# svip-lab/impersonator

Measured on AMD Instinct MI355X. Metric: frames/sec (256x256 motion-imitation, batch=8), higher is better.
Workload: dtype bf16x3; 1 GPU; Imitator inference 256x256 batch=8, random-init ImpersonatorGenerator + synthetic SMPL, 1 source; frames=1024, batch_per_gpu=8, image_size=256, parallelism=frame-sharded replicas x1, grid_sample_align_corners=False, lanes=2, batches_per_launch_sequence=4, frames_per_launch=32, precision=bf16x3, precision_policy=auto

## Files before the change

impersonator_amd/csrc/conv.h:

```cpp
#pragma once
#include <vector>

#include "common.h"

namespace lwg {

constexpr int kConvBM = 128;
constexpr int kConvBK = 32;

struct ConvPhase {
    int KH, KW;
    int ntaps;
    int Kpad;
    long w_off;
    int oy0, ox0;
    int iy0, ix0;
};

inline void split_bf16_groups(const float *src, size_t n, float *dst_opaque)
{
    __bf16 *d = reinterpret_cast<__bf16 *>(dst_opaque);
    for (size_t g = 0; g < n; g += 32)
        for (int e = 0; e < 32; ++e) {
            const float v = src[g + e];
            const __bf16 hi = (__bf16)v;
            d[2 * g + e] = hi;
            d[2 * g + 32 + e] = (__bf16)(v - (float)hi);
        }
}

struct ConvArgs {
    const float *x; int ldx;
    int N, H, W, Cin, cin_log2;
    const float *w;
    const float *w_split;
    int precision;
    const float *zeros;
    float *y; int ldy;
    int Ho, Wo, Cout;
    int Hm, Wm, stride, pad, os;
    int dil;
    float2 *partials;
    int mtiles;
    int nphase;
    int fuse_phases;
    int natural_order;
    int tap_inner;
    int raw_in, raw_from;
    const float2 *in_ss; int in_ss_ld;
    unsigned long long *trace;
    int general;
    const float *bias;
    int ksplit;
    float *kpart;
    size_t kpart_stride;
    ConvPhase ph[4];
};

int conv_trace_set(void *device_buffer, size_t bytes);
int conv_trace_launch(int idx, long long *v10);

enum { kIgemmReg64 = 0, kIgemmReg128 = 1, kIgemmSmallCin = 2, kIgemmDma64 = 3, kIgemmDma128 = 4, kIgemmBf16x3_64 = 5,
       kIgemmBf16x3_128 = 6, kDirectStemBf16x3 = 7, kHaloBf16x3_128 = 8, kHaloBf16x3_64 = 9, kIgemmDma32 = 10, kIgemmVariants = 11 };
extern const char *const kIgemmVariantNames[kIgemmVariants];
int launch_conv_igemm(const ConvArgs &a, int bn, hipStream_t st, int *variant = nullptr);
int check_conv_igemm(const ConvArgs &a, int bn);
bool conv_raw_input_supported(const ConvArgs &a, int bn);

constexpr int kStemKRow = 48;
constexpr int kStemWPitch = 7 * kStemKRow * 2 + 16;
constexpr int kStemWBytes = 2 * 64 * kStemWPitch;
struct StemArgs {
    const float *x; int N, H, W;
    const void *w;
    float *y;
    float2 *partials;
    int dbg;
};
bool stem_bf16x3_supported(int H, int W, int cin, int cin_pad, int cout, int k, int stride, int pad);
void stem_pack_weights(const float *w_oihw, int cin, std::vector<unsigned char> &out);
int launch_stem_bf16x3(const StemArgs &a, hipStream_t st, int max_workgroups = 0);

int launch_in_finalize(const float2 *partials, int nphase, int mtiles, int N, int C, const float *gamma,
                       const float *beta, float eps, float2 *scale_shift, hipStream_t st);

struct ApplyArgs {
    const float *raw; int C;
    int N, H, W;
    const float2 *scale_shift;
    int relu;
    float *dst; int ld_dst;
    const float *res; int ld_res;
    int split;
    int nwarp;
    const float *warp_src[2];
    int warp_n[2];
    const float *warp_T[2];
    int align_corners;
};
int launch_apply(const ApplyArgs &a, hipStream_t st, int lanes = 0);

int launch_unsplit(float *buf, size_t n, hipStream_t st);

struct HeadsArgs {
    const float *x; int N, H, W;
    const float2 *scale_shift;
    const float *wh;
    float *color, *mask;
    const float *bg; int bg_bs;
    float *pred;
};
int launch_heads(const HeadsArgs &a, hipStream_t st);
size_t heads_bf16x3_frag_bytes();
int launch_heads_pack(const float *wh, void *wfrag, hipStream_t st);
int launch_heads_bf16x3(const HeadsArgs &a, const void *wfrag, hipStream_t st, int bands = 0);

}
```

impersonator_amd/csrc/conv.hip:

```cpp
#include <type_traits>

#include "conv.h"
#include "split.h"
#include "sample.h"

namespace lwg {
namespace {

typedef float f32x16 __attribute__((ext_vector_type(16)));
typedef float f32x4 __attribute__((ext_vector_type(4)));
#pragma clang diagnostic ignored "-Winline-asm"

constexpr int BM = kConvBM;
constexpr int BK = kConvBK;
constexpr int LDK = BK + 4;

template <int BN, int WM, int WN, bool WIDE = false, int NWAVES = 4, int BMT = BM, int TC2 = 0>
__device__ __forceinline__ void igemm_epilogue(const ConvArgs &a, const ConvPhase &ph, int phase, f32x16 (&acc)[WM][WN],
                                               float *smem, int tid, int lane, int wave_m, int wave_n, int img, int rem0, int n0,
                                               int mtile, int sub_stride = 0)
{
    unsigned ones = ~0u;
    asm volatile("" : "+s"(ones));
    lane = (int)__builtin_amdgcn_mbcnt_hi(ones, __builtin_amdgcn_mbcnt_lo(ones, 0u));
// ... 398 lines not shown
        }
        amask[j] = m;
    }
    const float *xin = a.x + (size_t)img * a.H * a.W * a.ldx;
    const float *wsrc[B_ROWS];
#pragma unroll
    for (int j = 0; j < B_ROWS; ++j) {
        const int row = (wave * B_ROWS + j) * 8 + lr;
        wsrc[j] = a.w + ph.w_off + (size_t)(n0 + row) * ph.Kpad + (ls ^ ((row >> 1) & 7)) * 4;
    }

    const unsigned lds_base = (unsigned)(uintptr_t)(__attribute__((address_space(3))) float *)smem;
    auto dma16 = [&](const float *gsrc, unsigned lds_byte) {
        asm volatile("s_mov_b32 m0, %1\n\t"
                     "s_nop 0\n\t"
                     "global_load_lds_dwordx4 %0, off"
                     :
                     : "v"(gsrc), "s"(lds_byte)
                     : "memory", "m0");
    };
    const unsigned wave_a = __builtin_amdgcn_readfirstlane(lds_base + (unsigned)(wave * 4 * 8 * BK * 4));
    const unsigned wave_b = __builtin_amdgcn_readfirstlane(lds_base + (unsigned)((BM * BK + wave * B_ROWS * 8 * BK) * 4));
    int s_tap = 0, s_kh = 0, s_kw = 0, s_ci0 = 0;
    auto dma_piece = [&](int p, int kt, int slot) {
        const unsigned slot_byte = (unsigned)(slot * STAGE * 4);
        if (p < 4) {
            const unsigned sa = wave_a + slot_byte + (unsigned)(p * 8 * BK * 4);
            const int toff = (s_kh * a.W + s_kw) * a.dil * a.ldx + s_ci0;
            const float *src = ((amask[p] >> s_tap) & 1u) ? xin + (aoff[p] + toff) : a.zeros;
            dma16(src, sa);
        } else {
            const unsigned sb = wave_b + slot_byte + (unsigned)((p - 4) * 8 * BK * 4);
            dma16(wsrc[p - 4] + kt * BK, sb);
        }
        if (p == LPS - 1) {
            s_ci0 += BK;
            if (s_ci0 == a.Cin) {
                s_ci0 = 0;
                ++s_tap;
                if (++s_kw == ph.KW) { s_kw = 0; ++s_kh; }
            }
        }
    };

    f32x16 acc[WM][WN];
#pragma unroll
    for (int i = 0; i < WM; ++i)
#pragma unroll
        for (int j = 0; j < WN; ++j)
#pragma unroll
            for (int r = 0; r < 16; ++r) acc[i][j][r] = 0.f;

    const int frow = lane & 31;
    const int fsw = (frow >> 1) & 7;
    const int a_row = (wave_m * 32 * WM + frow) * BK;
    const int b_row = BM * BK + (wave_n * 32 * WN + frow) * BK;
    int fcol[BK / 8];
#pragma unroll
    for (int k8 = 0; k8 < BK / 8; ++k8) fcol[k8] = (((2 * k8 + (lane >> 5)) ^ fsw) * 4);

    auto stage_body = [&](int kt, int slot, auto do_dma) {
        const float *As = smem + slot * STAGE + a_row;
        const float *Bs = smem + slot * STAGE + b_row;
        int slot2 = slot + (NS - 1);
        if (slot2 >= NS) slot2 -= NS;
        float4 af[WM], bf[WN];
#pragma unroll
        for (int i = 0; i < WM; ++i) af[i] = *reinterpret_cast<const float4 *>(As + i * 32 * BK + fcol[0]);
#pragma unroll
        for (int j = 0; j < WN; ++j) bf[j] = *reinterpret_cast<const float4 *>(Bs + j * 32 * BK + fcol[0]);
#pragma unroll
        for (int k8 = 0; k8 < BK / 8; ++k8) {
            float4 an[WM], bn4[WN];
            if (k8 + 1 < BK / 8 && !(DBG & 8)) {
#pragma unroll
                for (int i = 0; i < WM; ++i) an[i] = *reinterpret_cast<const float4 *>(As + i * 32 * BK + fcol[k8 + 1]);
#pragma unroll
                for (int j = 0; j < WN; ++j) bn4[j] = *reinterpret_cast<const float4 *>(Bs + j * 32 * BK + fcol[k8 + 1]);
            }
#pragma unroll
            for (int i = 0; i < WM; ++i)
#pragma unroll
                for (int j = 0; j < WN; ++j) {
                    acc[i][j] = __builtin_amdgcn_mfma_f32_32x32x2f32(af[i].x, bf[j].x, acc[i][j], 0, 0, 0);
                    acc[i][j] = __builtin_amdgcn_mfma_f32_32x32x2f32(af[i].y, bf[j].y, acc[i][j], 0, 0, 0);
                    acc[i][j] = __builtin_amdgcn_mfma_f32_32x32x2f32(af[i].z, bf[j].z, acc[i][j], 0, 0, 0);
                    acc[i][j] = __builtin_amdgcn_mfma_f32_32x32x2f32(af[i].w, bf[j].w, acc[i][j], 0, 0, 0);
                    constexpr int CHAINS = (BK / 8) * WM * WN;
                    const int piece = k8 * (WM * WN) + i * WN + j;
                    if (decltype(do_dma)::value && !(DBG & 1)) {
#pragma unroll
                        for (int pp = piece; pp < LPS; ++pp) {
                            if (pp != piece && piece != CHAINS - 1) break;
                            __builtin_amdgcn_sched_barrier(0);
                            dma_piece(pp, kt + (NS - 1), slot2);
                            __builtin_amdgcn_sched_barrier(0);
                        }
                    }
                }
            if (k8 + 1 < BK / 8 && !(DBG & 8)) {
#pragma unroll
                for (int i = 0; i < WM; ++i) af[i] = an[i];
#pragma unroll
                for (int j = 0; j < WN; ++j) bf[j] = bn4[j];
            }
        }
        if (decltype(do_dma)::value) {
            asm volatile("s_waitcnt vmcnt(%0)" ::"n"((NS - 2) * LPS) : "memory");
        } else {
            asm volatile("s_waitcnt vmcnt(0)" ::: "memory");
        }
        if (!(DBG & 4)) __builtin_amdgcn_s_barrier();
        asm volatile("" ::: "memory");
    };
    using yes = std::integral_constant<bool, true>;
    using no = std::integral_constant<bool, false>;
    static_assert(LPS <= 2 * (BK / 8) * WM * WN, "not enough MFMA chains to hide the DMA pieces of a stage");

    const int nk = ph.Kpad / BK;
#pragma unroll
    for (int st = 0; st < NS - 1; ++st)
        if (st < nk) {
#pragma unroll
            for (int p = 0; p < LPS; ++p) dma_piece(p, st, st);
        }
    if (nk >= NS - 1) {
        asm volatile("s_waitcnt vmcnt(%0)" ::"n"((NS - 2) * LPS) : "memory");
    } else {
        asm volatile("s_waitcnt vmcnt(0)" ::: "memory");
    }
    __builtin_amdgcn_s_barrier();
    asm volatile("" ::: "memory");

    int slot = 0, kt = 0;
    for (; kt + (NS - 1) < nk; ++kt) {
        stage_body(kt, slot, yes{});
        if (++slot == NS) slot = 0;
    }
    for (; kt < nk; ++kt) {
        stage_body(kt, slot, no{});
        if (++slot == NS) slot = 0;
    }
    igemm_epilogue<BN, WM, WN, true>(a, ph, pz, acc, smem, tid, lane, wave_m, wave_n, img, rem0, n0, blockIdx.x);
    __syncthreads();
    }
}

template <int BN, int WM, int WN, int DBG = 0, int NS = 3>
__global__ __launch_bounds__(256) void conv_igemm_dma_f32(const ConvArgs a)
{
    igemm_dma_body<BN, WM, WN, DBG, NS>(a);
}

template <int BN, int WM, int WN, int NS = 3, int DBG = 0, int BMT = BM>
__global__ __launch_bounds__(64 * (BMT / (32 * WM)) * (BN / (32 * WN))) void conv_igemm_bf16x3(const ConvArgs a)
{
    constexpr int WAVES_N = BN / (32 * WN), WAVES_M = BMT / (32 * WM), NW = WAVES_M * WAVES_N;
    static_assert((NW == 4 || NW == 8) && NS >= 3, "wave layout");
    constexpr int A_CH = (DBG & 1024) ? 1 : BMT / 8 / NW, B_CH = BN / 8 / NW;
    constexpr int LPS = A_CH + B_CH;
    constexpr int STAGE = (BMT + BN) * BK;
    constexpr int TILES = WM * WN;
    constexpr int Q = 6 * TILES;
    static_assert(Q >= LPS, "at most one DMA piece per MFMA");
    constexpr int QB = Q * 3 / 4;
    constexpr int ISSUED = (QB * LPS) / Q;

    extern __shared__ __attribute__((aligned(16))) float smem[];
    const int tid = threadIdx.x, lane = tid & 63;
    const int wave = __builtin_amdgcn_readfirstlane(tid >> 6);
    const int wave_m = wave / WAVES_N, wave_n = wave % WAVES_N;
    int bx = blockIdx.x;
    const int by = blockIdx.y;
    if (!(DBG & 64) && !a.natural_order && (gridDim.x & 7) == 0) bx = (blockIdx.x & 7) * (gridDim.x >> 3) + (blockIdx.x >> 3);
    const int m0 = bx * BMT, n0 = by * BN;
    const int hw_m = a.Hm * a.Wm, img = __builtin_amdgcn_readfirstlane(m0 / hw_m), rem0 = m0 - img * hw_m;
    const unsigned lds_base = (unsigned)(uintptr_t)(__attribute__((address_space(3))) float *)smem;
    auto uniform_ptr = [](const void *p) {
        const unsigned long long v = (unsigned long long)p;
        const unsigned lo = __builtin_amdgcn_readfirstlane((unsigned)v);
        const unsigned hi = __builtin_amdgcn_readfirstlane((unsigned)(v >> 32));
        return reinterpret_cast<const char *>(((unsigned long long)hi << 32) | lo);
    };
    auto dma16 = [&](unsigned voff, const char *sbase, unsigned lds_byte) {
        asm volatile("s_mov_b32 m0, %2\n\t"
                     "s_nop 0\n\t"
                     "global_load_lds_dwordx4 %0, %1"
                     :
                     : "v"(voff), "s"(sbase), "s"(lds_byte)
                     : "memory", "m0");
    };
    using yes = std::integral_constant<bool, true>;
    using no = std::integral_constant<bool, false>;
    unsigned long long tr_a = 0, tr_b = 0, tr_c = 0, tr_wait = 0, tr_bar = 0, tr_t0 = 0, tr_loop0 = 0, tr_loop1 = 0;
    unsigned long long tr_d0 = 0, tr_d1 = 0, tr_d2 = 0, tr_d3 = 0, tr_dma = 0, tr_rt0 = 0;
    unsigned tr_stages = 0;
    if (DBG & 512) {
        tr_t0 = __builtin_amdgcn_s_memtime();
        tr_rt0 = __builtin_amdgcn_s_memrealtime();
    }

    const int pz0 = a.fuse_phases ? 0 : a.nphase - 1 - (int)blockIdx.z;
    const int pz1 = a.fuse_phases ? a.nphase : pz0 + 1;
    for (int pz = pz0; pz < pz1; ++pz) {
    const ConvPhase ph = a.ph[pz];

    const int lr = lane >> 3, ls = lane & 7;
    int aoff[A_CH];
    unsigned amask[A_CH];
#pragma unroll
    for (int j = 0; j < A_CH; ++j) {
        const int row = (wave * A_CH + j) * 8 + lr;
        const int rem = rem0 + row;
        const int hm = rem / a.Wm, wm = rem - hm * a.Wm;
        const int hi0 = hm * a.stride - a.pad, wi0 = wm * a.stride - a.pad;
        aoff[j] = (hi0 * a.W + wi0) * a.ldx + (ls ^ ((row >> 1) & 7)) * 4;
        unsigned m = 0;
        for (int t = 0, kh = 0, kw = 0; t < ph.ntaps; ++t) {
            const bool ok = (unsigned)(hi0 + kh * a.dil) < (unsigned)a.H && (unsigned)(wi0 + kw * a.dil) < (unsigned)a.W;
            m |= (unsigned)ok << t;
            if (++kw == ph.KW) { kw = 0; ++kh; }
        }
        amask[j] = m;
    }
    const float *xin = a.x + (size_t)img * a.H * a.W * a.ldx;
    const char *x_base = uniform_ptr(xin);
    const char *w_base = uniform_ptr(a.w_split + ph.w_off);
    const unsigned zoff_b = (unsigned)((const char *)a.zeros - (const char *)xin);
    unsigned wvoff[B_CH], cur[A_CH];
#pragma unroll
    for (int j = 0; j < B_CH; ++j) {
        const int row = (wave * B_CH + j) * 8 + lr;
        wvoff[j] = (unsigned)(((n0 + row) * ph.Kpad + (ls ^ ((row >> 1) & 7)) * 4) * 4);
    }
    int s_tap = 0, s_kh = 0, s_kw = 0;
    unsigned s_ci_b = 0, s_w_b = 0;
    auto retap = [&]() {
        const int tapoff = (s_kh * a.W + s_kw) * a.dil * a.ldx;
#pragma unroll
        for (int p = 0; p < A_CH; ++p) cur[p] = ((amask[p] >> s_tap) & 1u) ? (unsigned)((aoff[p] + tapoff) * 4) : zoff_b;
    };
    retap();
    const unsigned wave_a = __builtin_amdgcn_readfirstlane(lds_base + (unsigned)(wave * A_CH * 8 * BK * 4));
    const unsigned wave_b = __builtin_amdgcn_readfirstlane(lds_base + (unsigned)((BMT * BK + wave * B_CH * 8 * BK) * 4));
    auto dma_piece = [&](int p, int kt, int slot) {
        const unsigned slot_byte = (unsigned)(slot * STAGE * 4);
        if (p < A_CH) {
            dma16(cur[p], x_base + s_ci_b, wave_a + slot_byte + (unsigned)(p * 8 * BK * 4));
        } else {
            dma16(wvoff[p - A_CH], w_base + __builtin_amdgcn_readfirstlane(s_w_b), wave_b + slot_byte + (unsigned)((p - A_CH) * 8 * BK * 4));
        }
        if (p == LPS - 1) {
            if (a.tap_inner) {
                ++s_tap;
                if (++s_kw == ph.KW) { s_kw = 0; ++s_kh; }
                if (s_tap == ph.ntaps) { s_tap = 0; s_kh = 0; s_kw = 0; s_ci_b += BK * 4; }
                s_w_b = (unsigned)(s_tap * a.Cin) * 4u + s_ci_b;
                retap();
            } else {
                s_w_b += BK * 4;
                s_ci_b += BK * 4;
                if (s_ci_b == (unsigned)a.Cin * 4) {
                    asm volatile("; next tap" ::: "memory");
                    s_ci_b = 0;
                    ++s_tap;
                    if (++s_kw == ph.KW) { s_kw = 0; ++s_kh; }
                    retap();
                }
            }
        }
    };

    f32x16 acc[WM][WN];
#pragma unroll
    for (int i = 0; i < WM; ++i)
#pragma unroll
        for (int j = 0; j < WN; ++j)
#pragma unroll
            for (int r = 0; r < 16; ++r) acc[i][j][r] = 0.f;

    const int frow = lane & 31, fsw = (frow >> 1) & 7;
    const int a_row = (wave_m * 32 * WM + frow) * BK;
    const int b_row = BMT * BK + (wave_n * 32 * WN + frow) * BK;
    int fcol[4];
#pragma unroll
    for (int c = 0; c < 4; ++c) fcol[c] = (((2 * c + (lane >> 5)) ^ fsw) * 4);
    struct Frags { float4 ah[WM], al[WM], bh[WN], bl[WN]; };
    auto load_frags = [&](int slot, int kb, Frags &f) {
        const float *As = smem + slot * STAGE + a_row;
        const float *Bs = smem + slot * STAGE + b_row;
        const int ch = fcol[kb], cl = fcol[2 + kb];
#pragma unroll
        for (int i = 0; i < WM; ++i) {
            f.ah[i] = *reinterpret_cast<const float4 *>(As + i * 32 * BK + ch);
            f.al[i] = *reinterpret_cast<const float4 *>(As + i * 32 * BK + cl);
        }
#pragma unroll
        for (int j = 0; j < WN; ++j) {
            f.bh[j] = *reinterpret_cast<const float4 *>(Bs + j * 32 * BK + ch);
            f.bl[j] = *reinterpret_cast<const float4 *>(Bs + j * 32 * BK + cl);
        }
    };
    auto load_one = [&](int slot, int kb, Frags &f, int idx) {
        const float *As = smem + slot * STAGE + a_row;
        const float *Bs = smem + slot * STAGE + b_row;
        const int ch = fcol[kb], cl = fcol[2 + kb];
        if (idx < WM) f.al[idx] = *reinterpret_cast<const float4 *>(As + idx * 32 * BK + cl);
        else if (idx < WM + WN) f.bh[idx - WM] = *reinterpret_cast<const float4 *>(Bs + (idx - WM) * 32 * BK + ch);
        else if (idx < 2 * WM + WN) f.ah[idx - WM - WN] = *reinterpret_cast<const float4 *>(As + (idx - WM - WN) * 32 * BK + ch);
        else f.bl[idx - 2 * WM - WN] = *reinterpret_cast<const float4 *>(Bs + (idx - 2 * WM - WN) * 32 * BK + cl);
    };
    constexpr int NL = 2 * (WM + WN);
    constexpr int RPM = (NL + (Q - QB) - 1) / (Q - QB);
    Frags fr;

    auto stage_body = [&](int kt, auto slot_c, auto do_dma) {
        constexpr int slot = decltype(slot_c)::value;
        constexpr int slot1 = (slot + 1) % NS, slot2 = (slot + NS - 1) % NS;
        Frags f1, nx;
        if (DBG & 256) load_frags(slot, 1, f1);
#pragma unroll
        for (int q = 0; q < Q; ++q) {
            const int kb = q / (3 * TILES), r = q % (3 * TILES);
            const int t = r / TILES, i = (r / WN) % WM, j = r % WN;
            if (q == QB) {
                __builtin_amdgcn_sched_barrier(0);
                if (DBG & 512) {
                    if (tr_stages) {
                        tr_wait += tr_b - tr_a; tr_bar += tr_c - tr_b;
                        tr_dma += (tr_d1 - tr_d0) + (tr_d3 - tr_d2);
                    }
                    ++tr_stages;
                    tr_a = __builtin_amdgcn_s_memtime();
                }
                if (decltype(do_dma)::value) {
                    asm volatile("s_waitcnt vmcnt(%0) lgkmcnt(0)" ::"n"((NS - 3) * LPS + ISSUED) : "memory");
                } else {
                    asm volatile("s_waitcnt vmcnt(0) lgkmcnt(0)" ::: "memory");
                }
                if (DBG & 512) tr_b = __builtin_amdgcn_s_memtime();
                if (!(DBG & 4)) __builtin_amdgcn_s_barrier();
                if (DBG & 512) tr_c = __builtin_amdgcn_s_memtime();
                asm volatile("" ::: "memory");
                if (DBG & 256) {
                    load_frags(slot1, 0, nx);
                    __builtin_amdgcn_sched_barrier(0);
                }
            }
            const Frags &f = kb == 0 ? fr : f1;
            const float4 a4 = t == 0 ? f.al[i] : f.ah[i];
            const float4 b4 = t == 1 ? f.bl[j] : f.bh[j];
            acc[i][j] = __builtin_amdgcn_mfma_f32_32x32x16_bf16(__builtin_bit_cast(bf16x8_t, a4),
                                                                __builtin_bit_cast(bf16x8_t, b4), acc[i][j], 0, 0, 0);
            if (!(DBG & 8) && !(DBG & 256)) {
                if (q < NL) {
                    load_one(slot, 1, f1, q);
                    __builtin_amdgcn_sched_group_barrier(0x008, 1, 0);
                    __builtin_amdgcn_sched_group_barrier(0x100, 1, 0);
                } else if (q >= QB && RPM * (q - QB) < NL) {
#pragma unroll
                    for (int r2 = 0; r2 < RPM; ++r2)
                        if (RPM * (q - QB) + r2 < NL) load_one(slot1, 0, nx, RPM * (q - QB) + r2);
                    __builtin_amdgcn_sched_group_barrier(0x008, 1, 0);
                    __builtin_amdgcn_sched_group_barrier(0x100, RPM, 0);
                }
            }
            if (decltype(do_dma)::value && !(DBG & 1)) {
                const int pc = ((q + 1) * LPS) / Q;
                const int pb = (q * LPS) / Q;
                if (pc != pb) {
                    __builtin_amdgcn_sched_barrier(0);
                    if ((DBG & 512) && pb == 0) tr_d0 = __builtin_amdgcn_s_memtime();
                    if ((DBG & 512) && pb == A_CH) tr_d2 = __builtin_amdgcn_s_memtime();
                    dma_piece(pb, kt + (NS - 1), slot2);
                    if ((DBG & 512) && pb == 0) tr_d1 = __builtin_amdgcn_s_memtime();
                    if ((DBG & 512) && pb == A_CH) tr_d3 = __builtin_amdgcn_s_memtime();
                    __builtin_amdgcn_sched_barrier(0);
                }
            }
        }
        if (!(DBG & 8)) fr = nx;
    };

    const int nk = ph.Kpad / BK;
#pragma unroll
    for (int st = 0; st < NS - 1; ++st)
        if (st < nk) {
#pragma unroll
            for (int p = 0; p < LPS; ++p) dma_piece(p, st, st);
        }
    if (nk >= NS - 1) {
        asm volatile("s_waitcnt vmcnt(%0)" ::"n"((NS - 2) * LPS) : "memory");
    } else {
        asm volatile("s_waitcnt vmcnt(0)" ::: "memory");
    }
    __builtin_amdgcn_s_barrier();
    asm volatile("" ::: "memory");
    load_frags(0, 0, fr);

    if (DBG & 512) tr_loop0 = __builtin_amdgcn_s_memtime();
    int kt = 0, slot = 0;
    static_assert(NS >= 3 && NS <= 5, "ring depth");
    for (; kt + 2 * (NS - 1) < nk; kt += NS) {
        stage_body(kt, std::integral_constant<int, 0>{}, yes{});
        stage_body(kt + 1, std::integral_constant<int, 1>{}, yes{});
        stage_body(kt + 2, std::integral_constant<int, 2>{}, yes{});
        if constexpr (NS >= 4) stage_body(kt + 3, std::integral_constant<int, 3>{}, yes{});
        if constexpr (NS >= 5) stage_body(kt + 4, std::integral_constant<int, 4>{}, yes{});
    }
    auto run_stage = [&](int k, int sl, auto do_dma) {
        if (sl == 0) stage_body(k, std::integral_constant<int, 0>{}, do_dma);
        else if (sl == 1) stage_body(k, std::integral_constant<int, 1>{}, do_dma);
        else if (NS == 3 || sl == 2) stage_body(k, std::integral_constant<int, 2>{}, do_dma);
        else if (NS == 4 || sl == 3) stage_body(k, std::integral_constant<int, (NS > 3 ? 3 : 2)>{}, do_dma);
        else stage_body(k, std::integral_constant<int, NS - 1>{}, do_dma);
    };
    for (; kt + (NS - 1) < nk; ++kt) {
        run_stage(kt, slot, yes{});
        if (++slot == NS) slot = 0;
    }
    for (; kt < nk; ++kt) {
        run_stage(kt, slot, no{});
        if (++slot == NS) slot = 0;
    }

    if (DBG & 512) {
        asm volatile("s_waitcnt lgkmcnt(0)" ::: "memory");
        tr_wait += tr_b - tr_a;
        tr_bar += tr_c - tr_b;
        tr_loop1 = __builtin_amdgcn_s_memtime();
    }
    if (!(DBG & 32)) igemm_epilogue<BN, WM, WN, !(DBG & 128), NW, BMT>(a, ph, pz, acc, smem, tid, lane, wave_m, wave_n, img, rem0, n0, bx);
    if ((DBG & 512) && a.trace && lane == 0) {
        const unsigned long long tr_end = __builtin_amdgcn_s_memtime();
        unsigned long long *o = a.trace + ((((size_t)blockIdx.z * gridDim.y + blockIdx.y) * gridDim.x + blockIdx.x) * NW + wave) * 8;
        const unsigned long long tr_rt1 = __builtin_amdgcn_s_memrealtime();
        unsigned hwid, xcc;
        asm volatile("s_getreg_b32 %0, hwreg(HW_REG_HW_ID)" : "=s"(hwid));
        asm volatile("s_getreg_b32 %0, hwreg(HW_REG_XCC_ID)" : "=s"(xcc));
        o[0] = tr_t0; o[1] = tr_loop0; o[2] = tr_loop1; o[3] = tr_end; o[4] = tr_wait; o[5] = tr_bar;
        o[6] = (unsigned long long)tr_stages | (tr_dma << 16) | ((tr_rt1 - tr_rt0) << 44);
        o[7] = ((unsigned long long)xcc << 32) | hwid;
    }
    if (DBG & 32) {
        float keep = 0.f;
#pragma unroll
        for (int i = 0; i < WM; ++i)
#pragma unroll
            for (int j = 0; j < WN; ++j)
#pragma unroll
                for (int r = 0; r < 16; ++r) keep += acc[i][j][r];
        if (keep == 123.456f) a.y[0] = 1.f;
    }
    __syncthreads();
    }
}

template <int NHW, int B_CH, int Q, int QB, int NS, int HT = 7>
struct HaloSched {
    static constexpr int nh(int t) { return t < HT ? NHW / HT + (t < NHW % HT ? 1 : 0) : 0; }
    static constexpr int tap_of(int k) { int t = 0; while (hstart(t + 1) <= k) ++t; return t; }
    static constexpr bool dma_at(int t, int q) { for (int p = 0; p < lps(t); ++p) if (pos(t, p) == q) return true; return false; }
    static constexpr int nfree(int t, int q0) { int n = 0; for (int q = q0; q < QB; ++q) n += dma_at(t, q) ? 0 : 1; return n; }
    static constexpr int conv_first(int nconv, int nslot, int slot, int piece) { return conv_range(nconv, nslot, slot, piece) / 16; }
    static constexpr int conv_last(int nconv, int nslot, int slot, int piece) { return conv_range(nconv, nslot, slot, piece) % 16; }
    static constexpr int conv_range(int nconv, int nslot, int slot, int piece) {
        if (nconv == 1) {
            if (piece != 0) return 0;
            if (nslot >= 7)
                return slot == 0 ? 0 * 16 + 1 : slot == 3 ? 1 * 16 + 3 : slot == 4 ? 3 * 16 + 5 : slot == 5 ? 5 * 16 + 7 : slot == 6 ? 7 * 16 + 8 : 0;
            return slot == 0 ? 0 * 16 + 1 : slot == 2 ? 1 * 16 + 4 : slot == 3 ? 4 * 16 + 6 : slot == 4 ? 6 * 16 + 8 : 0;
        }
        if (nslot >= 8) {
            if (slot >= 8 || (slot & 1) != piece) return 0;
            return (slot >> 1) == 0 ? 0 * 16 + 1 : (slot >> 1) == 1 ? 1 * 16 + 3 : (slot >> 1) == 2 ? 3 * 16 + 5 : 5 * 16 + 8;
        }
        if (slot == 0) return 0 * 16 + 1;
        if (slot < 2 || slot >= 6 || (slot & 1) != piece) return 0;
        return slot < 4 ? 1 * 16 + 4 : 4 * 16 + 8;
    }
    static constexpr int free_index(int t, int q0, int q) {
        if (q < q0 || q >= QB || dma_at(t, q)) return -1;
        int n = 0;
        for (int u = q0; u < q; ++u) n += dma_at(t, u) ? 0 : 1;
        return n;
    }
    static constexpr int hstart(int t) { int n = 0; for (int u = 0; u < t; ++u) n += nh(u); return n; }
    static constexpr int lps(int t) { return nh(t) + B_CH; }
    static constexpr int pos(int t, int p) { return (p + 1) * Q / lps(t) - 1; }
    static constexpr int issued(int t) { int n = 0; for (int p = 0; p < lps(t); ++p) n += pos(t, p) < QB ? 1 : 0; return n; }
    static constexpr int nwait(int t) { int n = issued(t); for (int d = 1; d <= NS - 3; ++d) n += lps((t + 9 - d) % 9); return n; }
};

struct HaloCT {
    static constexpr int phase(int t) { return t == 0 ? 0 : t < 3 ? 1 : t < 5 ? 2 : 3; }
    static constexpr int tap(int t) { return t == 0 ? 0 : t < 3 ? t - 1 : t < 5 ? t - 3 : t - 5; }
    static constexpr int dy(int t) { return (t == 4 || t == 7 || t == 8) ? 1 : 0; }
    static constexpr int dx(int t) { return (t == 2 || t == 6 || t == 8) ? 1 : 0; }
};

template <int BN, int WM, int WN, int NWAVES, int BMT, int TC>
__device__ __forceinline__ void halo_epilogue(const ConvArgs &a, const ConvPhase &ph, int phase, f32x4 (&acc)[2 * WM][2 * WN], float *smem,
                                              int wave_m, int wave_n, int img, int h0, int w0, int n0, int part0, int sub_stride)
{
    unsigned ones = ~0u;
    asm volatile("" : "+s"(ones));
    const int lane = (int)__builtin_amdgcn_mbcnt_hi(ones, __builtin_amdgcn_mbcnt_lo(ones, 0u));
    const int tid = (wave_m * (BN / (32 * WN)) + wave_n) * 64 + lane;
    const int col = lane & 15, rsel = 4 * (lane >> 4);
    constexpr int TP = 36;
    float *stage = smem + (tid >> 6) * 32 * TP;
    const int rrow = lane >> 3, rcol = (lane & 7) * 4;
#pragma unroll
    for (int i = 0; i < WM; ++i)
#pragma unroll
        for (int j = 0; j < WN; ++j) {
#pragma unroll
            for (int h = 0; h < 2; ++h)
#pragma unroll
                for (int g = 0; g < 2; ++g)
#pragma unroll
                    for (int r = 0; r < 4; ++r) stage[(16 * h + rsel + r) * TP + 16 * g + col] = acc[2 * i + h][2 * j + g][r];
#pragma unroll
            for (int q = 0; q < 4; ++q) {
                const int row = q * 8 + rrow;
                const float4 v = *reinterpret_cast<const float4 *>(stage + row * TP + rcol);
                const int trow = wave_m * 32 * WM + i * 32 + row;
                const int hm = h0 + trow / TC, wm = w0 + trow % TC;
                const size_t opix = ((size_t)img * a.Ho + hm * a.os + ph.oy0) * a.Wo + wm * a.os + ph.ox0;
                *reinterpret_cast<float4 *>(a.y + opix * a.ldy + n0 + wave_n * 32 * WN + j * 32 + rcol) = v;
            }
        }
    if (!a.partials) return;
    float2 *red = reinterpret_cast<float2 *>(smem + NWAVES * 32 * TP);
    auto lane_xor = [&](float v, int m) {
        return __builtin_bit_cast(float, __builtin_amdgcn_ds_bpermute((lane ^ m) << 2, __builtin_bit_cast(int, v)));
    };
#pragma unroll
    for (int i = 0; i < WM; ++i)
#pragma unroll
        for (int j = 0; j < WN; ++j)
#pragma unroll
            for (int g = 0; g < 2; ++g) {
                float s = 0.f;
#pragma unroll
                for (int h = 0; h < 2; ++h)
#pragma unroll
                    for (int r = 0; r < 4; ++r) s += acc[2 * i + h][2 * j + g][r];
                s += lane_xor(s, 16);
                s += lane_xor(s, 32);
                const float mu = s * (1.f / 32.f);
                float q = 0.f;
#pragma unroll
                for (int h = 0; h < 2; ++h)
#pragma unroll
                    for (int r = 0; r < 4; ++r) {
                        const float d = acc[2 * i + h][2 * j + g][r] - mu;
                        q += d * d;
                    }
                q += lane_xor(q, 16);
                q += lane_xor(q, 32);
                if (lane < 16) red[(wave_m * WM + i) * BN + wave_n * 32 * WN + j * 32 + 16 * g + col] = make_float2(mu, q);
            }
    __syncthreads();
    if (tid < BN * (BMT / BM)) {
        constexpr int RT = BM / 32;
        const int sub = tid / BN, ch = tid - sub * BN;
        float mean = 0.f;
#pragma unroll
        for (int w = 0; w < RT; ++w) mean += red[(sub * RT + w) * BN + ch].x;
        mean *= 1.f / RT;
        float m2 = 0.f;
#pragma unroll
        for (int w = 0; w < RT; ++w) {
            const float2 p = red[(sub * RT + w) * BN + ch];
            const float d = p.x - mean;
            m2 += p.y + 32.f * d * d;
        }
        a.partials[((size_t)phase * a.mtiles + (size_t)part0 + (size_t)sub * sub_stride) * a.Cout + n0 + ch] = make_float2(mean, m2);
    }
}

constexpr int halo_min_waves(int bn, int ct) { return ct ? (bn == 128 ? 1 : 2) : bn == 128 ? 2 : 3; }

template <int BN, int WM, int WN, int NS, int TC, int BMT = BM, int CT = 0, bool RAW = false>
__global__ __launch_bounds__(64 * (BMT / (32 * WM)) * (BN / (32 * WN))) __attribute__((amdgpu_waves_per_eu(halo_min_waves(BN, CT))))
void conv3x3_halo_bf16x3(const ConvArgs a)
{
    constexpr int NPH = CT ? 4 : 1, PADL = CT ? 0 : 1;
    constexpr int WAVES_N = BN / (32 * WN), WAVES_M = BMT / (32 * WM), NW = WAVES_M * WAVES_N;
    static_assert((NW == 4 || NW == 8) && (NS == 3 || NS == 4) && BMT % TC == 0 && TC % 32 == 0, "layout");
    constexpr int TR = BMT / TC, HC = TC + 2 - (CT ? 1 : 0), HR = TR + 2 - (CT ? 1 : 0), HP = HR * HC;
    constexpr int NCH = (HP + 7) / 8;
    constexpr int NHW = (NCH + NW - 1) / NW;
    constexpr int HALO = NCH * 8 * BK;
    constexpr int B_CH = BN / 8 / NW, BSTAGE = BN * BK, BOFF = 2 * HALO;
    static_assert(B_CH >= 1, "a weight chunk per wave");
    constexpr int TILES = WM * WN, Q = 6 * TILES, QB = Q * 3 / 4, NL = 2 * (WM + WN);
    constexpr int RPM = (NL + 2 * (Q - QB) - 1) / (2 * (Q - QB));
    constexpr int HT = RAW ? 6 : 7;
    using S = HaloSched<NHW, B_CH, Q, QB, NS, HT>;
    static_assert(S::hstart(9) == NHW && Q >= NHW / HT + 1 + B_CH, "halo pieces fit their taps, one piece per MFMA at most");
    static_assert(!RAW || (NW % 2 == 0 && S::tap_of(NHW - 1) + 3 <= 8), "RAW: chunk parity per wave, conversions end ahead of the barrier of tap 8");
    constexpr int DUMMY = BOFF + NS * BSTAGE;
    constexpr int SSOFF = DUMMY + 8 * BK;

    extern __shared__ __attribute__((aligned(16))) float smem[];
    const int tid = threadIdx.x, lane = tid & 63;
// ... 165 lines not shown
        int nxt_a[WM];
        [[maybe_unused]] const bool raw_next = RAW && sl + 1 < nslices && (sl + 1) * BK >= a.raw_from;
        [[maybe_unused]] const unsigned live_bits = raw_next ? inside : 0u;
        if constexpr (RAW) {
            if (T == S::tap_of(0) + 3) load_ss(sl + 1 < nslices ? sl + 1 : 0);
        }
#pragma unroll
        for (int q = 0; q < Q; ++q) {
            const int t = q / (2 * TILES), r = q % (2 * TILES);
            if (q == QB) {
                __builtin_amdgcn_sched_barrier(0);
                if (ISSUE) {
                    asm volatile("s_waitcnt vmcnt(%0) lgkmcnt(0)" ::"n"(S::nwait(T)) : "memory");
                } else {
                    asm volatile("s_waitcnt vmcnt(0) lgkmcnt(0)" ::: "memory");
                }
                __builtin_amdgcn_s_barrier();
                asm volatile("" ::: "memory");
#pragma unroll
                for (int ii = 0; ii < WM; ++ii) nxt_a[ii] = a_addr(ii, TN, hs_next);
            }
            constexpr int PP = CT ? HaloCT::phase(T) : 0;
            auto mfma_and_read = [&](int e) {
                const int u = 2 * r + e, i = u / WN2, j = u % WN2, g = 2 * q + e;
                const float4 a4 = t == 0 ? fr.a[i] : f1.a[i];
                const float4 b4 = t == 1 ? f1.b[j] : fr.b[j];
                acc[PP][i][j] = __builtin_amdgcn_mfma_f32_16x16x32_bf16(__builtin_bit_cast(bf16x8_t, a4),
                                                                        __builtin_bit_cast(bf16x8_t, b4), acc[PP][i][j], 0, 0, 0);
                if (g < NL) {
                    load_one(cur_a, slot, false, f1, g);
                    __builtin_amdgcn_sched_group_barrier(0x008, 1, 0);
                    __builtin_amdgcn_sched_group_barrier(0x100, 1, 0);
                } else if (g >= 2 * QB && RPM * (g - 2 * QB) < NL) {
#pragma unroll
                    for (int r2 = 0; r2 < RPM; ++r2)
                        if (RPM * (g - 2 * QB) + r2 < NL) load_one(nxt_a, slot1, true, nx, RPM * (g - 2 * QB) + r2);
                    __builtin_amdgcn_sched_group_barrier(0x008, 1, 0);
                    __builtin_amdgcn_sched_group_barrier(0x100, RPM, 0);
                }
            };
            mfma_and_read(0);
            if constexpr (!RAW) mfma_and_read(1);
            if constexpr (RAW) {
                constexpr int NCONV = T >= 3 ? S::nh(T - 3) : 0, K0 = T >= 3 ? S::hstart(T - 3) : 0;
                constexpr int Q0 = QB - NL >= 10 ? NL : 0;
                constexpr int NF = S::nfree(T, Q0);
                static_assert(NCONV <= 2 && NF >= (NCONV == 2 ? 6 : 5), "conversion steps fit ahead of the barrier");
                const int fi = S::free_index(T, Q0, q);
                if (NCONV > 0 && fi >= 0) {
                    const int a0 = S::conv_first(NCONV, NF, fi, 0), a1 = S::conv_last(NCONV, NF, fi, 0);
                    const int b0 = S::conv_first(NCONV, NF, fi, 1), b1 = S::conv_last(NCONV, NF, fi, 1);
                    if (a1 > a0 || b1 > b0) {
                        __builtin_amdgcn_sched_barrier(0);
#pragma unroll
                        for (int m = 0; m < 8; ++m)
                            if (m >= a0 && m < a1) convert_step(K0, cvA, hs ^ 1, m, (live_bits >> K0) & 1u);
#pragma unroll
                        for (int m = 0; m < 8; ++m)
                            if (m >= b0 && m < b1) convert_step(K0 + 1, cvB, hs ^ 1, m, (live_bits >> (K0 + 1)) & 1u);
                        __builtin_amdgcn_sched_barrier(0);
                    }
                }
                mfma_and_read(1);
            }
            if (ISSUE) {
#pragma unroll
                for (int p = 0; p < S::lps(T); ++p)
                    if (q == S::pos(T, p)) {
                        __builtin_amdgcn_sched_barrier(0);
                        if (p < S::nh(T)) halo_piece(S::hstart(T) + p, sl_halo, hs ^ 1);
                        else weight_piece(p - S::nh(T), IT, is, slot2);
                        __builtin_amdgcn_sched_barrier(0);
                    }
            }
        }
        fr = nx;
#pragma unroll
        for (int ii = 0; ii < WM; ++ii) cur_a[ii] = nxt_a[ii];
    };

    if constexpr (RAW) {
        const float2 *ss = a.in_ss + (size_t)img * a.in_ss_ld;
        const int nraw = a.Cin - a.raw_from;
        for (int i2 = tid; i2 < nraw; i2 += NW * 64) reinterpret_cast<float2 *>(smem + SSOFF)[i2] = ss[i2];
        asm volatile("s_waitcnt vmcnt(0)" ::: "memory");
    }
#pragma unroll
    for (int j = 0; j < NHW; ++j) halo_piece(j, 0, 0);
#pragma unroll
    for (int st = 0; st < NS - 1; ++st)
#pragma unroll
        for (int jb = 0; jb < B_CH; ++jb) weight_piece(jb, st, 0, st);
    asm volatile("s_waitcnt vmcnt(%0)" ::"n"((NS - 2) * B_CH) : "memory");
    if constexpr (RAW) {
        if (a.raw_from == 0) {
            asm volatile("s_waitcnt lgkmcnt(0)" ::: "memory");
            __builtin_amdgcn_s_barrier();
            asm volatile("" ::: "memory");
            load_ss(0);
#pragma unroll
            for (int j = 0; j < NHW; ++j)
#pragma unroll
                for (int step = 0; step < 8; ++step) convert_step(j, cvA, 0, step, (inside >> j) & 1u);
            asm volatile("s_waitcnt lgkmcnt(0)" ::: "memory");
        }
    }
    __builtin_amdgcn_s_barrier();
    asm volatile("" ::: "memory");
#pragma unroll
    for (int ii = 0; ii < WM; ++ii) cur_a[ii] = a_addr(ii, 0, 0);
#pragma unroll
    for (int idx = 0; idx < NL; ++idx) load_one(cur_a, 0, true, fr, idx);

    using yes = std::integral_constant<bool, true>;
    using no = std::integral_constant<bool, false>;
    if (a.trace) tr_loop0 = __builtin_amdgcn_s_memtime();
    int slot = 0;
    auto bump = [&]() { slot = slot + 1 == NS ? 0 : slot + 1; };
#define LWG_HALO_STAGE(T, ISS) stage_body(std::integral_constant<int, T>{}, ISS{}, sl, slot); bump();
    for (int sl = 0; sl + 1 < nslices; ++sl) {
        LWG_HALO_STAGE(0, yes) LWG_HALO_STAGE(1, yes) LWG_HALO_STAGE(2, yes) LWG_HALO_STAGE(3, yes) LWG_HALO_STAGE(4, yes)
        LWG_HALO_STAGE(5, yes) LWG_HALO_STAGE(6, yes) LWG_HALO_STAGE(7, yes) LWG_HALO_STAGE(8, yes)
    }
    {
        const int sl = nslices - 1;
        LWG_HALO_STAGE(0, yes) LWG_HALO_STAGE(1, yes) LWG_HALO_STAGE(2, yes) LWG_HALO_STAGE(3, yes) LWG_HALO_STAGE(4, yes)
        LWG_HALO_STAGE(5, yes)
        if constexpr (NS == 3) { LWG_HALO_STAGE(6, yes) } else { LWG_HALO_STAGE(6, no) }
        LWG_HALO_STAGE(7, no) LWG_HALO_STAGE(8, no)
    }
#undef LWG_HALO_STAGE

    if (a.trace) tr_loop1 = __builtin_amdgcn_s_memtime();
    __syncthreads();
    const int part0 = img * (tiles_x * (a.Hm / 4)) + (h0 / 4) * tiles_x + (w0 / TC);
#pragma unroll
    for (int pp = 0; pp < NPH; ++pp) {
        if (pp) __syncthreads();
        halo_epilogue<BN, WM, WN, NW, BMT, TC>(a, a.ph[pp], pp, acc[pp], smem, wave_m, wave_n, img, h0, w0, n0, part0, tiles_x);
    }
    if (a.trace && lane == 0) {
        const unsigned long long tr_end = __builtin_amdgcn_s_memtime(), tr_rt1 = __builtin_amdgcn_s_memrealtime();
        unsigned long long *o = a.trace + (((size_t)blockIdx.y * gridDim.x + blockIdx.x) * NW + wave) * 8;
        o[0] = tr_t0; o[1] = tr_loop0; o[2] = tr_loop1; o[3] = tr_end; o[4] = 0; o[5] = 0;
        o[6] = (unsigned long long)(9 * nslices) | ((tr_rt1 - tr_rt0) << 44);
        o[7] = 0;
    }
}

constexpr int FIN_CH = 16, FIN_SL = 16;
__global__ __launch_bounds__(256) void in_finalize_kernel(const float2 *__restrict__ partials, int nphase, int mtiles,
                                                          int tiles_per_img, int C, const float *__restrict__ gamma,
                                                          const float *__restrict__ beta, float eps,
                                                          float2 *__restrict__ scale_shift)
{
    __shared__ double sh[3][FIN_SL][FIN_CH];
    const int cl = threadIdx.x & (FIN_CH - 1);
    const int c = blockIdx.x * FIN_CH + cl;
    const int slice = threadIdx.x / FIN_CH;
    const int n = blockIdx.y;
    double sm = 0., sq = 0., m2 = 0.;
    if (c < C) {
        for (int p = 0; p < nphase; ++p) {
            const float2 *base = partials + ((size_t)p * mtiles + (size_t)n * tiles_per_img) * C + c;
#pragma unroll 4
            for (int t = slice; t < tiles_per_img; t += FIN_SL) {
                const float2 v = base[(size_t)t * C];
                sm += v.x;
                sq += (double)v.x * v.x;
                m2 += v.y;
            }
        }
    }
    sh[0][slice][cl] = sm;
    sh[1][slice][cl] = sq;
    sh[2][slice][cl] = m2;
    __syncthreads();
    if (slice == 0 && c < C) {
        sm = sq = m2 = 0.;
#pragma unroll
        for (int k = 0; k < FIN_SL; ++k) {
            sm += sh[0][k][cl];
            sq += sh[1][k][cl];
            m2 += sh[2][k][cl];
        }
        const double cnt = (double)nphase * tiles_per_img;
        const double mean = sm / cnt;
        double between = sq - cnt * mean * mean;
        if (between < 0.) between = 0.;
        const double var = (m2 + BM * between) / (cnt * BM);
        const double inv = 1.0 / sqrt(var + (double)eps);
        const float sc = (float)(gamma[c] * inv);
        scale_shift[(size_t)n * C + c] = make_float2(sc, (float)(beta[c] - mean * gamma[c] * inv));
    }
}

__device__ __forceinline__ float4 ld4(const float *p) { return *reinterpret_cast<const float4 *>(p); }
__device__ __forceinline__ void fma4(float4 &acc, const float4 v, float w)
{
    acc.x += v.x * w; acc.y += v.y * w; acc.z += v.z * w; acc.w += v.w * w;
}

__global__ __launch_bounds__(256) void apply_kernel(const ApplyArgs a)
{
    const int c4n = a.C >> 2;
    const long i = (long)blockIdx.x * blockDim.x + threadIdx.x;
    const long total = (long)a.N * a.H * a.W * c4n;
    if (i >= total) return;
    const long pix = i / c4n;
    const int c = (int)(i - pix * c4n) * 4;
    const int hw = a.H * a.W;
    const int n = (int)(pix / hw);
    const int pn = (int)(pix - (long)n * hw);

    const float4 v = ld4(a.raw + pix * a.C + c);
    const float4 s01 = ld4(reinterpret_cast<const float *>(a.scale_shift + (size_t)n * a.C + c));
    const float4 s23 = ld4(reinterpret_cast<const float *>(a.scale_shift + (size_t)n * a.C + c + 2));
    float4 y;
    y.x = v.x * s01.x + s01.y;
    y.y = v.y * s01.z + s01.w;
    y.z = v.z * s23.x + s23.y;
    y.w = v.w * s23.z + s23.w;
    if (a.relu) {
        y.x = fmaxf(y.x, 0.f); y.y = fmaxf(y.y, 0.f); y.z = fmaxf(y.z, 0.f); y.w = fmaxf(y.w, 0.f);
    }
    const int soff = (c >> 5) * 32 + ((c & 31) >> 1);
    if (a.res) {
        float4 r;
        if (a.split) {
            const bf16x4_t h = *reinterpret_cast<const bf16x4_t *>(a.res + pix * a.ld_res + soff);
            const bf16x4_t l = *reinterpret_cast<const bf16x4_t *>(a.res + pix * a.ld_res + soff + 16);
            r = make_float4((float)h[0] + (float)l[0], (float)h[1] + (float)l[1], (float)h[2] + (float)l[2],
                            (float)h[3] + (float)l[3]);
        } else {
            r = ld4(a.res + pix * a.ld_res + c);
        }
        y.x += r.x; y.y += r.y; y.z += r.z; y.w += r.w;
    }
    for (int k = 0; k < a.nwarp; ++k) {
        const float2 g = *reinterpret_cast<const float2 *>(a.warp_T[k] + pix * 2);
        const GridTaps t = grid_taps(g.x, g.y, a.W, a.H, a.align_corners);
        const float *src = a.warp_src[k] + (size_t)(a.warp_n[k] > 1 ? n : 0) * hw * a.C + c;
        float4 wsum = make_float4(0.f, 0.f, 0.f, 0.f);
        if (t.vnw) fma4(wsum, ld4(src + (size_t)(t.y0 * a.W + t.x0) * a.C), t.wnw);
        if (t.vne) fma4(wsum, ld4(src + (size_t)(t.y0 * a.W + t.x0 + 1) * a.C), t.wne);
        if (t.vsw) fma4(wsum, ld4(src + (size_t)((t.y0 + 1) * a.W + t.x0) * a.C), t.wsw);
        if (t.vse) fma4(wsum, ld4(src + (size_t)((t.y0 + 1) * a.W + t.x0 + 1) * a.C), t.wse);
        y.x += wsum.x; y.y += wsum.y; y.z += wsum.z; y.w += wsum.w;
    }
    (void)pn;
    if (a.split) {
        bf16x4_t h, l;
        h[0] = (__bf16)y.x; h[1] = (__bf16)y.y; h[2] = (__bf16)y.z; h[3] = (__bf16)y.w;
        l[0] = (__bf16)(y.x - (float)h[0]); l[1] = (__bf16)(y.y - (float)h[1]);
        l[2] = (__bf16)(y.z - (float)h[2]); l[3] = (__bf16)(y.w - (float)h[3]);
        *reinterpret_cast<bf16x4_t *>(a.dst + pix * a.ld_dst + soff) = h;
        *reinterpret_cast<bf16x4_t *>(a.dst + pix * a.ld_dst + soff + 16) = l;
    } else {
        *reinterpret_cast<float4 *>(a.dst + pix * a.ld_dst + c) = y;
    }
}

__global__ __launch_bounds__(256) void apply8_kernel(const ApplyArgs a)
{
    const int c8n = a.C >> 3;
    const long i = (long)blockIdx.x * blockDim.x + threadIdx.x;
    const long total = (long)a.N * a.H * a.W * c8n;
    if (i >= total) return;
    const long pix = i / c8n;
    const int c = (int)(i - pix * c8n) * 8;
    const int hw = a.H * a.W;
    const int n = (int)(pix / hw);

    const float4 v0 = ld4(a.raw + pix * a.C + c), v1 = ld4(a.raw + pix * a.C + c + 4);
    const float *ssp = reinterpret_cast<const float *>(a.scale_shift + (size_t)n * a.C + c);
    const float4 s0 = ld4(ssp), s1 = ld4(ssp + 4), s2 = ld4(ssp + 8), s3 = ld4(ssp + 12);
    float y[8];
    y[0] = v0.x * s0.x + s0.y; y[1] = v0.y * s0.z + s0.w; y[2] = v0.z * s1.x + s1.y; y[3] = v0.w * s1.z + s1.w;
    y[4] = v1.x * s2.x + s2.y; y[5] = v1.y * s2.z + s2.w; y[6] = v1.z * s3.x + s3.y; y[7] = v1.w * s3.z + s3.w;
    if (a.relu) {
#pragma unroll
        for (int k = 0; k < 8; ++k) y[k] = fmaxf(y[k], 0.f);
    }
    const int soff = (c >> 5) * 32 + ((c & 31) >> 1);
    if (a.res) {
        const bf16x8_t h = *reinterpret_cast<const bf16x8_t *>(a.res + pix * a.ld_res + soff);
        const bf16x8_t l = *reinterpret_cast<const bf16x8_t *>(a.res + pix * a.ld_res + soff + 16);
#pragma unroll
        for (int k = 0; k < 8; ++k) y[k] += (float)h[k] + (float)l[k];
    }
    for (int k = 0; k < a.nwarp; ++k) {
        const float2 g = *reinterpret_cast<const float2 *>(a.warp_T[k] + pix * 2);
        const GridTaps t = grid_taps(g.x, g.y, a.W, a.H, a.align_corners);
        const float *src = a.warp_src[k] + (size_t)(a.warp_n[k] > 1 ? n : 0) * hw * a.C + c;
        float4 w0 = make_float4(0.f, 0.f, 0.f, 0.f), w1 = w0;
        if (t.vnw) { const float *q = src + (size_t)(t.y0 * a.W + t.x0) * a.C; fma4(w0, ld4(q), t.wnw); fma4(w1, ld4(q + 4), t.wnw); }
        if (t.vne) { const float *q = src + (size_t)(t.y0 * a.W + t.x0 + 1) * a.C; fma4(w0, ld4(q), t.wne); fma4(w1, ld4(q + 4), t.wne); }
        if (t.vsw) { const float *q = src + (size_t)((t.y0 + 1) * a.W + t.x0) * a.C; fma4(w0, ld4(q), t.wsw); fma4(w1, ld4(q + 4), t.wsw); }
        if (t.vse) { const float *q = src + (size_t)((t.y0 + 1) * a.W + t.x0 + 1) * a.C; fma4(w0, ld4(q), t.wse); fma4(w1, ld4(q + 4), t.wse); }
        y[0] += w0.x; y[1] += w0.y; y[2] += w0.z; y[3] += w0.w; y[4] += w1.x; y[5] += w1.y; y[6] += w1.z; y[7] += w1.w;
    }
    bf16x8_t h, l;
#pragma unroll
    for (int k = 0; k < 8; ++k) {
        h[k] = (__bf16)y[k];
        l[k] = (__bf16)(y[k] - (float)h[k]);
    }
    *reinterpret_cast<bf16x8_t *>(a.dst + pix * a.ld_dst + soff) = h;
    *reinterpret_cast<bf16x8_t *>(a.dst + pix * a.ld_dst + soff + 16) = l;
}

__global__ __launch_bounds__(256) void unsplit_kernel(float *buf, size_t ngroups)
{
    const size_t g = (size_t)blockIdx.x * blockDim.x + threadIdx.x;
    if (g >= ngroups) return;
    float4 raw[8];
#pragma unroll
    for (int i = 0; i < 8; ++i) raw[i] = ld4(buf + g * 32 + i * 4);
#pragma unroll
    for (int i = 0; i < 4; ++i) {
        const bf16x8_t h = __builtin_bit_cast(bf16x8_t, raw[i]);
        const bf16x8_t l = __builtin_bit_cast(bf16x8_t, raw[4 + i]);
        float4 o0 = make_float4((float)h[0] + (float)l[0], (float)h[1] + (float)l[1], (float)h[2] + (float)l[2],
                                (float)h[3] + (float)l[3]);
        float4 o1 = make_float4((float)h[4] + (float)l[4], (float)h[5] + (float)l[5], (float)h[6] + (float)l[6],
                                (float)h[7] + (float)l[7]);
        *reinterpret_cast<float4 *>(buf + g * 32 + i * 8) = o0;
        *reinterpret_cast<float4 *>(buf + g * 32 + i * 8 + 4) = o1;
    }
}

constexpr int HT = 32, HH = HT + 6;
constexpr int HCH = 8;
constexpr int HPITCH = HCH + 4;
constexpr int HEADS_W = 49 * HCH * 4;
constexpr int HEADS_LDS = (HH * HH * HPITCH + HEADS_W) * (int)sizeof(float);

__global__ __launch_bounds__(256) void heads_kernel(const HeadsArgs a)
{
    extern __shared__ __attribute__((aligned(16))) float halo[];
    const int tid = threadIdx.x;
    const int tx = tid & 31, tg = tid >> 5;
    const int n = blockIdx.z;
    const int y0 = blockIdx.y * HT, x0 = blockIdx.x * HT;
    const float *xin = a.x + (size_t)n * a.H * a.W * 64;
    const float2 *ss = a.scale_shift + (size_t)n * 64;

    float acc[4][4];
#pragma unroll
    for (int r = 0; r < 4; ++r)
#pragma unroll
        for (int o = 0; o < 4; ++o) acc[r][o] = 0.f;

    for (int chunk = 0; chunk < 64 / HCH; ++chunk) {
        __syncthreads();
        for (int i = tid; i < HH * HH * (HCH / 4); i += 256) {
            const int pix = i / (HCH / 4), half = i % (HCH / 4);
            const int hy = pix / HH, hx = pix - hy * HH;
            const int gy = y0 - 3 + hy, gx = x0 - 3 + hx;
            float4 v = make_float4(0.f, 0.f, 0.f, 0.f);
            if ((unsigned)gy < (unsigned)a.H && (unsigned)gx < (unsigned)a.W) {
                const int c = chunk * HCH + half * 4;
                v = ld4(xin + ((size_t)gy * a.W + gx) * 64 + c);
                const float4 s01 = ld4(reinterpret_cast<const float *>(ss + c));
                const float4 s23 = ld4(reinterpret_cast<const float *>(ss + c + 2));
                v.x = fmaxf(v.x * s01.x + s01.y, 0.f);
                v.y = fmaxf(v.y * s01.z + s01.w, 0.f);
                v.z = fmaxf(v.z * s23.x + s23.y, 0.f);
                v.w = fmaxf(v.w * s23.z + s23.w, 0.f);
            }
            *reinterpret_cast<float4 *>(halo + pix * HPITCH + half * 4) = v;
        }
        float *wl = halo + HH * HH * HPITCH;
        for (int i = tid; i < 49 * HCH; i += 256) {
            const int t = i / HCH, c = i % HCH;
            *reinterpret_cast<float4 *>(wl + i * 4) = ld4(a.wh + ((size_t)t * 64 + chunk * HCH + c) * 4);
        }
        __syncthreads();
        for (int kx = 0; kx < 7; ++kx)
            for (int q = 0; q < HCH / 4; ++q) {
                float4 hv[10], wq[7][4];
#pragma unroll
                for (int hr = 0; hr < 10; ++hr) hv[hr] = ld4(halo + ((tg * 4 + hr) * HH + tx + kx) * HPITCH + q * 4);
#pragma unroll
                for (int ky = 0; ky < 7; ++ky) {
                    const float *wp = wl + ((ky * 7 + kx) * HCH + q * 4) * 4;
#pragma unroll
                    for (int ci = 0; ci < 4; ++ci) wq[ky][ci] = ld4(wp + ci * 4);
                }
                __builtin_amdgcn_sched_barrier(0);
#pragma unroll
                for (int ky = 0; ky < 7; ++ky)
#pragma unroll
                    for (int r = 0; r < 4; ++r) {
                        const float4 v = hv[r + ky];
                        const float vv[4] = {v.x, v.y, v.z, v.w};
#pragma unroll
                        for (int ci = 0; ci < 4; ++ci) {
                            const float4 w = wq[ky][ci];
                            acc[r][0] = fmaf(vv[ci], w.x, acc[r][0]);
                            acc[r][1] = fmaf(vv[ci], w.y, acc[r][1]);
                            acc[r][2] = fmaf(vv[ci], w.z, acc[r][2]);
                            acc[r][3] = fmaf(vv[ci], w.w, acc[r][3]);
                        }
                    }
            }
    }
    const int ox = x0 + tx;
    if (ox >= a.W) return;
    const size_t hw = (size_t)a.H * a.W;
#pragma unroll
    for (int r = 0; r < 4; ++r) {
        const int oy = y0 + tg * 4 + r;
        if (oy >= a.H) break;
        const size_t p = (size_t)oy * a.W + ox;
        const float col[3] = {tanhf(acc[r][0]), tanhf(acc[r][1]), tanhf(acc[r][2])};
        const float m = 1.f / (1.f + expf(-acc[r][3]));
#pragma unroll
        for (int c = 0; c < 3; ++c) {
            if (a.color) a.color[((size_t)n * 3 + c) * hw + p] = col[c];
            if (a.pred) {
                const float b = a.bg[((size_t)(a.bg_bs > 1 ? n : 0) * 3 + c) * hw + p];
                a.pred[((size_t)n * 3 + c) * hw + p] = m * b + (1.f - m) * col[c];
            }
        }
        if (a.mask) a.mask[(size_t)n * hw + p] = m;
    }
}

}

const char *const kIgemmVariantNames[kIgemmVariants] = {
    "conv_igemm_f32<64, 1, 2, false, 0>", "conv_igemm_f32<128, 2, 2, false, 0>", "conv_igemm_f32<64, 1, 2, true, 0>",
    "conv_igemm_dma_f32<64, 1, 2, 0, 3>", "conv_igemm_dma_f32<128, 2, 2, 0, 3>",
    "conv_igemm_bf16x3<64, 1, 2, 3, 0>", "conv_igemm_bf16x3<128, 2, 2", "stem_bf16x3_kernel",
    "conv3x3_halo_bf16x3<128, 2, 2", "conv3x3_halo_bf16x3<64, 1, 2", "conv_igemm_dma_f32<32, 1, 1, 0, 3>"};

constexpr int kTraceMaxLaunches = 4096;
struct TraceLaunch { size_t offset; int gx, gy, gz, waves, stages, cin, cout, hm, n; };
struct TraceState {
    void *buf = nullptr; size_t bytes = 0, used = 0; int n = 0;
    TraceLaunch launch[kTraceMaxLaunches];
};
static TraceState g_trace;

int conv_trace_set(void *device_buffer, size_t bytes)
{
    g_trace.buf = device_buffer; g_trace.bytes = device_buffer ? bytes : 0; g_trace.used = 0; g_trace.n = 0;
    return LWG_OK;
}
int conv_trace_launch(int idx, long long *v)
{
    if (idx < 0 || idx >= g_trace.n) return LWG_ERR_INVALID_ARG;
    const TraceLaunch &L = g_trace.launch[idx];
    v[0] = (long long)L.offset; v[1] = L.gx; v[2] = L.gy; v[3] = L.gz; v[4] = L.waves; v[5] = L.stages; v[6] = L.cin; v[7] = L.cout;
    v[8] = L.hm; v[9] = L.n;
    return LWG_OK;
}

static unsigned long long *trace_block(const ConvArgs &a, dim3 grid, int waves, int stages)
{
    if (!g_trace.buf) return nullptr;
    const size_t need = (size_t)grid.x * grid.y * grid.z * waves * 8 * sizeof(unsigned long long);
    if (g_trace.used + need > g_trace.bytes || g_trace.n >= kTraceMaxLaunches) return nullptr;
    unsigned long long *p = reinterpret_cast<unsigned long long *>(static_cast<char *>(g_trace.buf) + g_trace.used);
    TraceLaunch &L = g_trace.launch[g_trace.n++];
    L.offset = g_trace.used; L.gx = grid.x; L.gy = grid.y; L.gz = grid.z; L.waves = waves; L.stages = stages; L.cin = a.Cin;
    L.cout = a.Cout; L.hm = a.Hm; L.n = a.N;
    g_trace.used += need;
    return p;
}

struct ConvKernel { void (*fn)(ConvArgs); int block; size_t lds_cap; int variant; const char *label; };

constexpr int kRawMaxChannels = 512;
constexpr size_t reg_lds(int bn) { return (size_t)2 * (BM + bn) * LDK * sizeof(float); }
constexpr size_t ring_lds(int ns, int bn, int bmt = BM) { return (size_t)ns * (bmt + bn) * BK * sizeof(float); }
constexpr size_t halo_lds(int hp, int ns, int bn) { return ((size_t)2 * ((hp + 7) / 8) * 8 * BK + (size_t)ns * bn * BK) * sizeof(float); }
constexpr int halo3x3_px(int bmt) { return (bmt / 32 + 2) * (32 + 2); }
constexpr int kHaloCTPx = (4 + 1) * (32 + 1);
constexpr size_t raw_lds(int channels) { return (size_t)8 * BK * sizeof(float) + (size_t)channels * sizeof(float2); }

enum ConvKernelId {
    kF32_64, kF32_128, kF32_Small, kGen_64, kGen_128, kGen_Small, kGenX3_64, kGenX3_128, kGenX3_Small,
    kDma_32, kDma_64, kDma_128,
    kRing_64, kRing_128_3, kRing_128_4, kRing_128_Traced, kRing_128_Tall,
    kHalo_64, kHalo_128, kHalo_Tall, kHaloRaw_64, kHaloRaw_128, kHaloRaw_Tall,
    kHaloCT_64, kHaloCT_128, kHaloCTRaw_64, kHaloCTRaw_128,
#ifdef LWG_EXPERIMENTS
    kRing_128_X, kRing_128_5,
#endif
    kConvKernels
};
static const ConvKernel kConvKernelTable[kConvKernels] = {
    {&conv_igemm_f32<64, 1, 2, false>, 256, reg_lds(64), kIgemmReg64, "conv_igemm_f32"},
    {&conv_igemm_f32<128, 2, 2, false>, 256, reg_lds(128), kIgemmReg128, "conv_igemm_f32"},
    {&conv_igemm_f32<64, 1, 2, true>, 256, reg_lds(64), kIgemmSmallCin, "conv_igemm_f32"},
    {&conv_igemm_f32<64, 1, 2, false, 0, true>, 256, reg_lds(64), kIgemmReg64, "conv_igemm_f32 (general)"},
    {&conv_igemm_f32<128, 2, 2, false, 0, true>, 256, reg_lds(128), kIgemmReg128, "conv_igemm_f32 (general)"},
    {&conv_igemm_f32<64, 1, 2, true, 0, true>, 256, reg_lds(64), kIgemmSmallCin, "conv_igemm_f32 (general)"},
    {&conv_igemm_f32<64, 1, 2, false, 0, true, true>, 256, reg_lds(64), kIgemmReg64, "conv_igemm_f32 (general)"},
    {&conv_igemm_f32<128, 2, 2, false, 0, true, true>, 256, reg_lds(128), kIgemmReg128, "conv_igemm_f32 (general)"},
    {&conv_igemm_f32<64, 1, 2, true, 0, true, true>, 256, reg_lds(64), kIgemmSmallCin, "conv_igemm_f32 (general)"},
    {&conv_igemm_dma_f32<32, 1, 1>, 256, ring_lds(3, 32), kIgemmDma32, "conv_igemm_dma_f32"},
    {&conv_igemm_dma_f32<64, 1, 2>, 256, ring_lds(3, 64), kIgemmDma64, "conv_igemm_dma_f32"},
    {&conv_igemm_dma_f32<128, 2, 2>, 256, ring_lds(3, 128), kIgemmDma128, "conv_igemm_dma_f32"},
    {&conv_igemm_bf16x3<64, 1, 2>, 256, ring_lds(3, 64), kIgemmBf16x3_64, "conv_igemm_bf16x3"},
    {&conv_igemm_bf16x3<128, 2, 2>, 256, ring_lds(3, 128), kIgemmBf16x3_128, "conv_igemm_bf16x3"},
    {&conv_igemm_bf16x3<128, 2, 2, 4>, 256, ring_lds(4, 128), kIgemmBf16x3_128, "conv_igemm_bf16x3"},
    {&conv_igemm_bf16x3<128, 2, 2, 4, 512>, 256, ring_lds(4, 128), kIgemmBf16x3_128, "conv_igemm_bf16x3 (traced)"},
    {&conv_igemm_bf16x3<128, 2, 2, 3, 0, 256>, 512, ring_lds(3, 128, 256), kIgemmBf16x3_128, "conv_igemm_bf16x3 (256-row tiles)"},
    {&conv3x3_halo_bf16x3<64, 1, 2, 3, 32>, 256, halo_lds(halo3x3_px(128), 3, 64), kHaloBf16x3_64, "conv3x3_halo_bf16x3"},
    {&conv3x3_halo_bf16x3<128, 2, 2, 4, 32>, 256, halo_lds(halo3x3_px(128), 4, 128), kHaloBf16x3_128, "conv3x3_halo_bf16x3"},
    {&conv3x3_halo_bf16x3<128, 2, 2, 4, 32, 256>, 512, halo_lds(halo3x3_px(256), 4, 128), kHaloBf16x3_128, "conv3x3_halo_bf16x3"},
    {&conv3x3_halo_bf16x3<64, 1, 2, 3, 32, 128, 0, true>, 256, halo_lds(halo3x3_px(128), 3, 64) + raw_lds(kRawMaxChannels),
     kHaloBf16x3_64, "conv3x3_halo_bf16x3"},
    {&conv3x3_halo_bf16x3<128, 2, 2, 4, 32, 128, 0, true>, 256, halo_lds(halo3x3_px(128), 4, 128) + raw_lds(kRawMaxChannels),
     kHaloBf16x3_128, "conv3x3_halo_bf16x3"},
    {&conv3x3_halo_bf16x3<128, 2, 2, 4, 32, 256, 0, true>, 512, halo_lds(halo3x3_px(256), 4, 128) + raw_lds(kRawMaxChannels),
     kHaloBf16x3_128, "conv3x3_halo_bf16x3"},
    {&conv3x3_halo_bf16x3<64, 1, 2, 3, 32, 128, 1>, 256, halo_lds(kHaloCTPx, 3, 64), kHaloBf16x3_64, "conv3x3_halo_bf16x3 (transposed)"},
    {&conv3x3_halo_bf16x3<128, 2, 2, 4, 32, 128, 1>, 256, halo_lds(kHaloCTPx, 4, 128), kHaloBf16x3_128, "conv3x3_halo_bf16x3 (transposed)"},
    {&conv3x3_halo_bf16x3<64, 1, 2, 3, 32, 128, 1, true>, 256, kLdsPerCu, kHaloBf16x3_64, "conv3x3_halo_bf16x3 (transposed)"},
    {&conv3x3_halo_bf16x3<128, 2, 2, 4, 32, 128, 1, true>, 256, kLdsPerCu, kHaloBf16x3_128, "conv3x3_halo_bf16x3 (transposed)"},
#ifdef LWG_EXPERIMENTS
    {&conv_igemm_bf16x3<128, 2, 2, 4, 1024>, 256, ring_lds(4, 128), kIgemmBf16x3_128, "conv_igemm_bf16x3"},
    {&conv_igemm_bf16x3<128, 2, 2, 5>, 256, ring_lds(5, 128), kIgemmBf16x3_128, "conv_igemm_bf16x3"},
#endif
};

static bool halo3x3_shape(const ConvArgs &a)
{
    const ConvPhase &p0 = a.ph[0];
    return a.nphase == 1 && p0.KH == 3 && p0.KW == 3 && a.stride == 1 && a.pad == 1 && a.dil == 1 && a.os == 1 && a.H == a.Hm &&
           a.W == a.Wm && p0.Kpad == 9 * a.Cin && a.Wm % 32 == 0 && a.Hm % 4 == 0;
}
static bool haloCT_shape(const ConvArgs &a)
{
    return a.nphase == 4 && a.os == 2 && a.stride == 1 && a.pad == 0 && a.dil == 1 && a.H == a.Hm && a.W == a.Wm && a.Wm % 32 == 0 &&
           a.Hm % 4 == 0 && a.Cout % 64 == 0 && a.ph[0].KH == 1 && a.ph[0].KW == 1 && a.ph[1].KH == 1 && a.ph[1].KW == 2 &&
           a.ph[2].KH == 2 && a.ph[2].KW == 1 && a.ph[3].KH == 2 && a.ph[3].KW == 2 && a.ph[0].Kpad == a.Cin &&
           a.ph[1].Kpad == 2 * a.Cin && a.ph[2].Kpad == 2 * a.Cin && a.ph[3].Kpad == 4 * a.Cin;
}

struct ConvSwitches {
    bool halo, halo_tall, ct_wide, ring3, ring_tall, fused_apply;
    char ring_exp;
};
static const ConvSwitches &conv_switches()
{
    static const ConvSwitches sw = [] {
        auto first = [](const char *name) { const char *v = getenv(name); return v ? v[0] : '\0'; };
        return ConvSwitches{first("LWG_HALO") != '0',
                            first("LWG_HALO_TALL") != '0',
                            first("LWG_CT_WIDE") != '0',
                            first("LWG_RING") == '3',
                            first("LWG_RING_TALL") != '0',
                            first("LWG_FUSED_APPLY") != '0',
                            first("LWG_RING")};
    }();
    return sw;
}

static bool raw_input_route(const ConvArgs &a, int bn, const ConvSwitches &sw)
{
    if (!sw.halo || !sw.fused_apply) return false;
    if (a.precision != 1 || a.general || !a.w_split || (a.ldx & 31) || (a.Cin & 31) || a.Cin < 32 || (bn != 64 && bn != 128)) return false;
    if (a.raw_from < 0 || (a.raw_from & 31) || a.raw_from >= a.Cin || a.Cin - a.raw_from > kRawMaxChannels) return false;
    return halo3x3_shape(a) || haloCT_shape(a);
}
bool conv_raw_input_supported(const ConvArgs &a, int bn) { return raw_input_route(a, bn, conv_switches()); }

struct ConvLaunch { const ConvKernel *k; dim3 grid; size_t lds; int trace_waves, trace_stages; };

static int plan_conv_igemm(const ConvArgs &a, int bn, int ncu, const ConvSwitches &sw, bool tracing, size_t trace_free, ConvLaunch *out)
{
    const bool bn32_ok = bn == 32 && a.precision == 0 && !a.general && a.Cin >= BK && a.zeros;
    if (a.Cout % bn != 0 || (bn != 64 && bn != 128 && !bn32_ok))
        LWG_FAIL(LWG_ERR_UNSUPPORTED, "conv: Cout=%d not a multiple of the %d-channel tile", a.Cout, bn);
    if (!a.general && ((a.Hm * a.Wm) % BM != 0 || a.mtiles * BM != a.N * a.Hm * a.Wm))
        LWG_FAIL(LWG_ERR_UNSUPPORTED, "conv: %dx%d output grid per image is not a multiple of %d pixels", a.Hm, a.Wm, BM);
    if (a.general && (a.partials || a.fuse_phases || (a.precision != 0 && a.precision != 1) ||
                      a.mtiles != ceil_div((long)a.N * a.Hm * a.Wm, BM)))
        LWG_FAIL(LWG_ERR_INVALID_ARG, "conv: general mode is unfused, without statistics, mtiles = ceil(M/128)");
    if (a.ksplit > 1 && (!a.general || !a.kpart || a.kpart_stride < (size_t)a.N * a.Ho * a.Wo * a.ldy))
        LWG_FAIL(LWG_ERR_INVALID_ARG, "conv: a reduction split needs the general mode and a partial buffer of ksplit outputs");
    if (a.dil < 1) LWG_FAIL(LWG_ERR_INVALID_ARG, "conv: dilation must be >= 1");
    if ((1 << a.cin_log2) != a.Cin || a.Cin < 4 || (a.ldx & 3))
        LWG_FAIL(LWG_ERR_UNSUPPORTED, "conv: Cin=%d must be a power of two >= 4 with a 16-byte aligned pixel stride", a.Cin);
    int max_taps = 0;
    for (int p = 0; p < a.nphase; ++p) {
        if (a.ph[p].Kpad % BK != 0 || a.ph[p].Kpad < a.ph[p].ntaps * a.Cin)
            LWG_FAIL(LWG_ERR_UNSUPPORTED, "conv: bad padded K=%d for %d taps x %d channels", a.ph[p].Kpad, a.ph[p].ntaps, a.Cin);
        if (a.ph[p].ntaps > max_taps) max_taps = a.ph[p].ntaps;
    }
    if (a.precision == 1 && a.tap_inner)
        for (int p = 0; p < a.nphase; ++p)
            if (a.ph[p].Kpad != a.ph[p].ntaps * a.Cin)
                LWG_FAIL(LWG_ERR_UNSUPPORTED, "conv: taps-innermost walk needs K=%d == %d taps x %d channels", a.ph[p].Kpad,
                         a.ph[p].ntaps, a.Cin);
    if (a.raw_in && (!a.in_ss || !raw_input_route(a, bn, sw)))
        LWG_FAIL(LWG_ERR_UNSUPPORTED, "conv: raw (un-normalised) input is only taken by the halo-resident bf16x3 kernels");

    const bool small_cin = a.Cin < BK;
    const dim3 grid(a.mtiles, a.Cout / bn, a.fuse_phases ? 1 : a.nphase * (a.ksplit > 1 ? a.ksplit : 1));
    const int tile = small_cin ? 2 : (bn == 128 ? 1 : 0);
    auto choose = [&](int id, dim3 g, size_t lds, int trace_waves = 0, int trace_stages = 0) -> int {
        *out = ConvLaunch{&kConvKernelTable[id], g, lds, trace_waves, trace_stages};
        if (lds > out->k->lds_cap) LWG_FAIL(LWG_ERR_STATE, "conv: %s asks for %zu bytes of LDS, opted in to %zu", out->k->label, lds, out->k->lds_cap);
        return LWG_OK;
    };
    if (a.general) {
        if (small_cin && bn != 64) LWG_FAIL(LWG_ERR_UNSUPPORTED, "conv: Cin=%d < %d is only built for the 64-channel tile", a.Cin, BK);
        if (max_taps > 64) LWG_FAIL(LWG_ERR_UNSUPPORTED, "conv: more than 64 taps");
        return choose((a.precision == 1 ? kGenX3_64 : kGen_64) + tile, grid, reg_lds(bn));
    }
    if (a.precision == 1) {
        if (small_cin || !a.w_split || !a.zeros || (a.ldx & 31) || (a.Cin & 31))
            LWG_FAIL(LWG_ERR_UNSUPPORTED, "conv: the bf16x3 path needs split weights and Cin, pixel stride multiples of 32");
        const char *x_end = reinterpret_cast<const char *>(a.x + (size_t)a.N * a.H * a.W * a.ldx);
        const char *z = reinterpret_cast<const char *>(a.zeros);
        if (z < x_end || (size_t)(z - reinterpret_cast<const char *>(a.x)) + (size_t)a.Cin * 4 > 0xffffffffull)
            LWG_FAIL(LWG_ERR_UNSUPPORTED, "conv: the bf16x3 path needs its zero run behind the input tensor, within 4 GiB");
        for (int p = 0; p < a.nphase; ++p)
            if ((size_t)a.Cout * a.ph[p].Kpad * 4 > 0xffffffffull)
                LWG_FAIL(LWG_ERR_UNSUPPORTED, "conv: weight matrix too large for 32-bit lane offsets");
        if (max_taps > 32) LWG_FAIL(LWG_ERR_UNSUPPORTED, "conv: more than 32 taps on the bf16x3 path");
        const size_t raw_bytes = a.raw_in ? raw_lds(a.Cin - a.raw_from) : 0;
        if (sw.halo && halo3x3_shape(a)) {
            const bool tall = bn == 128 && a.Hm % 8 == 0 && (long)(a.mtiles / 2) * (a.Cout / 128) >= ncu && sw.halo_tall;
            const int bmt = tall ? 256 : BM;
            return choose((a.raw_in ? kHaloRaw_64 : kHalo_64) + (tall ? 2 : bn == 128 ? 1 : 0), dim3(grid.x / (bmt / BM), grid.y, 1),
                          halo_lds(halo3x3_px(bmt), bn == 128 ? 4 : 3, bn) + raw_bytes, bmt / 32, 9 * a.Cin / BK);
        }
        if (sw.halo && haloCT_shape(a)) {
            const bool wide = a.Cout % 128 == 0 && (long)a.mtiles * (a.Cout / 128) >= ncu && sw.ct_wide;
            const int cbn = wide ? 128 : 64;
            return choose((a.raw_in ? kHaloCTRaw_64 : kHaloCT_64) + wide, dim3(a.mtiles, a.Cout / cbn, 1),
                          halo_lds(kHaloCTPx, wide ? 4 : 3, cbn) + raw_bytes, 4, -(int)(9 * a.Cin / BK));
        }
        if (bn == 64) return choose(kRing_64, grid, ring_lds(3, 64));
        if (tracing && !sw.ring3 && (size_t)grid.x * grid.y * grid.z * 4 * 8 * sizeof(unsigned long long) <= trace_free)
            return choose(kRing_128_Traced, grid, ring_lds(4, 128), 4, a.ph[0].Kpad / BK);
        if (!a.fuse_phases && a.nphase == 1 && (a.mtiles & 1) == 0 && (a.Hm * a.Wm) % 256 == 0 && !tracing &&
            (long)(a.mtiles / 2) * (a.Cout / 128) >= ncu && sw.ring_tall)
            return choose(kRing_128_Tall, dim3(grid.x / 2, grid.y, 1), ring_lds(3, 128, 256));
#ifdef LWG_EXPERIMENTS
        if (sw.ring_exp == 'x') return choose(kRing_128_X, grid, ring_lds(4, 128));
        if (sw.ring_exp == '5') return choose(kRing_128_5, grid, ring_lds(5, 128));
#endif
        return sw.ring3 ? choose(kRing_128_3, grid, ring_lds(3, 128)) : choose(kRing_128_4, grid, ring_lds(4, 128));
    }
    if (small_cin && bn != 64) LWG_FAIL(LWG_ERR_UNSUPPORTED, "conv: Cin=%d < %d is only built for the 64-channel tile", a.Cin, BK);
    const bool use_dma = !small_cin && a.zeros && max_taps <= 32 && (bn <= 64 || (long)grid.x * grid.y * grid.z <= ncu);
    if (a.fuse_phases && !use_dma) LWG_FAIL(LWG_ERR_UNSUPPORTED, "conv: fused phases need the DMA-fed kernel (Cin >= 32, 64-channel tile)");
    if (use_dma) return choose(bn == 32 ? kDma_32 : bn == 64 ? kDma_64 : kDma_128, grid, ring_lds(3, bn));
    if (bn != 64 && bn != 128) LWG_FAIL(LWG_ERR_UNSUPPORTED, "conv: the register-staged fp32 kernel has 64- and 128-channel tiles, not %d", bn);
    return choose(kF32_64 + tile, grid, reg_lds(bn));
}

int check_conv_igemm(const ConvArgs &a, int bn)
{
    ConvLaunch L;
    return plan_conv_igemm(a, bn, device_cu_count(), conv_switches(), false, 0, &L);
}

int launch_conv_igemm(const ConvArgs &a_in, int bn, hipStream_t st, int *variant)
{
    ConvArgs a = a_in;
    a.trace = nullptr;
    ConvLaunch L;
    const size_t trace_free = g_trace.n < kTraceMaxLaunches ? g_trace.bytes - g_trace.used : 0;
    const int rc = plan_conv_igemm(a, bn, device_cu_count(), conv_switches(), g_trace.buf != nullptr, trace_free, &L);
    if (rc != LWG_OK) return rc;
    static DeviceOnce opted_in;
    if (!opted_in.done()) {
        for (const ConvKernel &k : kConvKernelTable)
            LWG_HIP(hipFuncSetAttribute(reinterpret_cast<const void *>(k.fn), hipFuncAttributeMaxDynamicSharedMemorySize, (int)k.lds_cap));
        opted_in.mark();
    }
    if (L.trace_waves) a.trace = trace_block(a, L.grid, L.trace_waves, L.trace_stages);
    L.k->fn<<<L.grid, L.k->block, L.lds, st>>>(a);
    if (variant) *variant = L.k->variant;
    LWG_LAUNCH_CHECK(L.k->label);
    return LWG_OK;
}

#ifdef LWG_IGEMM_BENCH
static void launch_capped(void (*kern)(ConvArgs), const ConvArgs &a, int bn, int block, size_t lds, hipStream_t st, int bmt = BM)
{
    (void)hipFuncSetAttribute(reinterpret_cast<const void *>(kern), hipFuncAttributeMaxDynamicSharedMemorySize, (int)lds);
    kern<<<dim3(a.mtiles / (bmt / BM), a.Cout / bn, a.nphase), block, lds, st>>>(a);
}
template <int DBG>
static void launch_dbg(const ConvArgs &a, int bn, hipStream_t st)
{
    launch_capped(bn == 64 ? &conv_igemm_f32<64, 1, 2, false, DBG> : &conv_igemm_f32<128, 2, 2, false, DBG>, a, bn, 256, reg_lds(bn), st);
}
template <int DBG, int NS = 3>
static void launch_dma_dbg(const ConvArgs &a, int bn, hipStream_t st)
{
    launch_capped(bn == 64 ? &conv_igemm_dma_f32<64, 1, 2, DBG, NS> : &conv_igemm_dma_f32<128, 2, 2, DBG, NS>, a, bn, 256, ring_lds(NS, bn), st);
}
template <int NS, int DBG>
static void launch_k_dbg(const ConvArgs &a, int bn, hipStream_t st)
{
    launch_capped(bn == 64 ? &conv_igemm_bf16x3<64, 1, 2, NS, DBG> : &conv_igemm_bf16x3<128, 2, 2, NS, DBG>, a, bn, 256, ring_lds(NS, bn), st);
}
template <int BN, int WM, int WN, int DBG>
static void launch_w_dbg(const ConvArgs &a, hipStream_t st)
{
    launch_capped(&conv_igemm_bf16x3<BN, WM, WN, 3, DBG>, a, BN, 64 * (BM / (32 * WM)) * (BN / (32 * WN)), ring_lds(3, BN), st);
}
int launch_conv_igemm_dbg(const ConvArgs &a, int bn, int dbg, hipStream_t st)
{
    switch (dbg) {
        case 821: if (bn == 128) launch_w_dbg<128, 2, 1, 0>(a, st); else launch_w_dbg<64, 1, 1, 0>(a, st); break;
        case 812: if (bn == 128) launch_w_dbg<128, 1, 2, 0>(a, st); else launch_w_dbg<64, 1, 1, 0>(a, st); break;
        case 831: if (bn == 128) launch_w_dbg<128, 2, 1, 1>(a, st); else launch_w_dbg<64, 1, 1, 1>(a, st); break;
        case 856:
            if (bn != 64 || (a.mtiles & 1) || (a.Hm * a.Wm) % 256 != 0) return LWG_ERR_INVALID_ARG;
            launch_capped(&conv_igemm_bf16x3<64, 2, 2, 3, 0, 256>, a, 64, 256, ring_lds(3, 64, 256), st, 256);
            break;
        case 300: {
            ConvArgs b = a;
            b.precision = 1;
            return launch_conv_igemm(b, bn, st, nullptr);
        }
        case 200: launch_k_dbg<3, 0>(a, bn, st); break;
        case 201: launch_k_dbg<3, 1>(a, bn, st); break;
        case 204: launch_k_dbg<3, 4>(a, bn, st); break;
        case 213: launch_k_dbg<3, 13>(a, bn, st); break;
        case 240: launch_k_dbg<4, 0>(a, bn, st); break;
        case 241: launch_k_dbg<4, 1>(a, bn, st); break;
        case 245: launch_k_dbg<4, 13>(a, bn, st); break;
        case 1240: launch_k_dbg<4, 1024>(a, bn, st); break;
        case 232: launch_k_dbg<3, 32>(a, bn, st); break;
        case 264: launch_k_dbg<3, 64>(a, bn, st); break;
        case 328: launch_k_dbg<3, 128>(a, bn, st); break;
        case 456: launch_k_dbg<3, 256>(a, bn, st); break;
        case 0: launch_dbg<0>(a, bn, st); break;
        case 1: launch_dbg<1>(a, bn, st); break;
        case 3: launch_dbg<3>(a, bn, st); break;
        case 7: launch_dbg<7>(a, bn, st); break;
        case 15: launch_dbg<15>(a, bn, st); break;
        case 16: launch_dbg<16>(a, bn, st); break;
        case 4: launch_dbg<4>(a, bn, st); break;
        case 100: launch_dma_dbg<0>(a, bn, st); break;
        case 116: launch_dma_dbg<16>(a, bn, st); break;
        case 101: launch_dma_dbg<1>(a, bn, st); break;
        case 104: launch_dma_dbg<4>(a, bn, st); break;
        case 140: launch_dma_dbg<0, 4>(a, bn, st); break;
        default: return LWG_ERR_INVALID_ARG;
    }
    return LWG_OK;
}
#endif

int launch_in_finalize(const float2 *partials, int nphase, int mtiles, int N, int C, const float *gamma,
                       const float *beta, float eps, float2 *scale_shift, hipStream_t st)
{
    if (mtiles % N != 0) LWG_FAIL(LWG_ERR_UNSUPPORTED, "in_finalize: %d tiles do not split over %d images", mtiles, N);
    const dim3 grid(ceil_div(C, FIN_CH), N);
    in_finalize_kernel<<<grid, 256, 0, st>>>(partials, nphase, mtiles, mtiles / N, C, gamma, beta, eps, scale_shift);
    LWG_LAUNCH_CHECK("in_finalize_kernel");
    return LWG_OK;
}

int launch_apply(const ApplyArgs &a, hipStream_t st, int lanes)
{
    if (lanes != 0 && lanes != 4 && lanes != 8) LWG_FAIL(LWG_ERR_INVALID_ARG, "apply: lanes=%d (0: the launcher's choice, 4, 8)", lanes);
    if (lanes == 8 && !a.split) LWG_FAIL(LWG_ERR_UNSUPPORTED, "apply: eight channels per thread is the split-bf16 kernel");
    if ((a.C & 3) || (a.ld_dst & 3) || (a.res && (a.ld_res & 3)))
        LWG_FAIL(LWG_ERR_UNSUPPORTED, "apply: channel counts/strides must be multiples of 4 (C=%d)", a.C);
    if (a.split && ((a.C & 31) || (a.ld_dst & 31) || ((uintptr_t)a.dst & 127) ||
                    (a.res && ((a.ld_res & 31) || ((uintptr_t)a.res & 127)))))
        LWG_FAIL(LWG_ERR_UNSUPPORTED, "apply: split-bf16 buffers need 32-channel granularity (C=%d)", a.C);
    static const char *a8_env = getenv("LWG_APPLY8");
    if (lanes == 8 || (lanes == 0 && a.split && !(a8_env && a8_env[0] == '0'))) {
        const long total8 = (long)a.N * a.H * a.W * (a.C >> 3);
        apply8_kernel<<<ceil_div(total8, 256), 256, 0, st>>>(a);
        LWG_LAUNCH_CHECK("apply8_kernel");
        return LWG_OK;
    }
    const long total = (long)a.N * a.H * a.W * (a.C >> 2);
    apply_kernel<<<ceil_div(total, 256), 256, 0, st>>>(a);
    LWG_LAUNCH_CHECK("apply_kernel");
    return LWG_OK;
}

int launch_unsplit(float *buf, size_t n, hipStream_t st)
{
    if (n % 32) LWG_FAIL(LWG_ERR_INVALID_ARG, "unsplit: %zu floats is not a whole number of 32-value groups", n);
    if (!n) return LWG_OK;
    unsplit_kernel<<<(unsigned)ceil_div((long)(n / 32), 256), 256, 0, st>>>(buf, n / 32);
    LWG_LAUNCH_CHECK("unsplit_kernel");
    return LWG_OK;
}

int launch_heads(const HeadsArgs &a, hipStream_t st)
{
    if (a.pred && !a.bg) LWG_FAIL(LWG_ERR_INVALID_ARG, "heads: pred requested without a background image");
    static DeviceOnce opt_in;
    const int rc = opt_in_lds(reinterpret_cast<const void *>(&heads_kernel), HEADS_LDS, opt_in);
    if (rc != LWG_OK) return rc;
    const dim3 grid(ceil_div(a.W, HT), ceil_div(a.H, HT), a.N);
    heads_kernel<<<grid, 256, HEADS_LDS, st>>>(a);
    LWG_LAUNCH_CHECK("heads_kernel");
    return LWG_OK;
}

}
```

impersonator_amd/csrc/direct.hip:

```cpp
#include <type_traits>

#include "conv.h"

namespace lwg {
namespace {

typedef float f32x16 __attribute__((ext_vector_type(16)));
typedef __bf16 bf16x8_t __attribute__((ext_vector_type(8)));
typedef float f32x4 __attribute__((ext_vector_type(4)));
typedef float f32x4u __attribute__((ext_vector_type(4), aligned(4)));

constexpr int ST_COLS = 128, ST_ROWS = 2;
constexpr int ST_HW = ST_COLS + 8, ST_HH = ST_ROWS + 6;
constexpr int ST_PIX = 12;
constexpr int ST_HPLANE = ST_HH * ST_HW * ST_PIX;
constexpr int ST_WROW = kStemKRow * 2;
constexpr int ST_WPITCH = kStemWPitch;
constexpr int ST_WPLANE = 64 * ST_WPITCH;
constexpr int ST_RED = 2 * 4 * 64 * 8;
constexpr int ST_GROUPS = 2;
constexpr int ST_GLDS = 2 * ST_HPLANE + ST_RED;
constexpr int ST_LDS = 2 * ST_WPLANE + ST_GROUPS * ST_GLDS + 16;
static_assert(2 * ST_WPLANE == kStemWBytes, "host and device agree on the staged filter bank");
static_assert(ST_HPLANE % 16 == 0 && ST_LDS <= 160 * 1024, "stem tile must fit one CU's LDS");
static_assert((ST_WPITCH / 16) % 2 == 1, "odd 16-byte pitch: conflict-free weight fragment reads");

__device__ __forceinline__ void stem_group_barrier(unsigned *ctr, unsigned &target, int lane)
{
    target += 4;
    asm volatile("s_waitcnt lgkmcnt(0)" ::: "memory");
    if (lane == 0) __hip_atomic_fetch_add(ctr, 1u, __ATOMIC_RELAXED, __HIP_MEMORY_SCOPE_WORKGROUP);
    while (__hip_atomic_load(ctr, __ATOMIC_RELAXED, __HIP_MEMORY_SCOPE_WORKGROUP) < target) __builtin_amdgcn_s_sleep(1);
    asm volatile("" ::: "memory");
}

__global__ __launch_bounds__(256 * ST_GROUPS) void stem_bf16x3_kernel(const StemArgs a)
{
    extern __shared__ __attribute__((aligned(16))) unsigned char lds[];
    unsigned char *wts = lds;
    const int group = __builtin_amdgcn_readfirstlane(threadIdx.x >> 8);
    unsigned char *halo = lds + 2 * ST_WPLANE + group * ST_GLDS;
    float2 *red = reinterpret_cast<float2 *>(halo + 2 * ST_HPLANE);
    unsigned *gctr_all = reinterpret_cast<unsigned *>(lds + 2 * ST_WPLANE + ST_GROUPS * ST_GLDS);
    unsigned *gctr = gctr_all + group;
    unsigned gtarget = 0;

    const int tid = threadIdx.x & 255, lane = tid & 63;
    const int wave = __builtin_amdgcn_readfirstlane(tid >> 6);
#ifdef LWG_EXPERIMENTS
    const int dbg = a.dbg;
#else
    constexpr int dbg = 0;
#endif
    const int wrow = wave >> 1, whalf = wave & 1;

    for (int i = threadIdx.x; i < 2 * ST_WPLANE / 16; i += 256 * ST_GROUPS)
        reinterpret_cast<float4 *>(wts)[i] = reinterpret_cast<const float4 *>(a.w)[i];
    if (threadIdx.x < ST_GROUPS) gctr_all[threadIdx.x] = 0;

    const int a_base = ((wrow * ST_HW) + whalf * 64 + (lane & 31)) * ST_PIX + (lane >> 5) * 16;
    const int b_base = (lane & 31) * ST_WPITCH + (lane >> 5) * 16;

    const int tiles_x = a.W / ST_COLS, tiles_y = a.H / ST_ROWS;
    const int ntiles = a.N * tiles_y * tiles_x;
    constexpr int HE = (ST_HH * ST_HW + 255) / 256;
    float4 pre4[HE];
    float2 pre2[HE];
    auto fetch_halo = [&](int tile) {
        const int img = tile / (tiles_y * tiles_x);
        const int trem = tile - img * (tiles_y * tiles_x);
        const int ty = trem / tiles_x, tx = trem - ty * tiles_x;
        const int h0 = ty * ST_ROWS, c0 = tx * ST_COLS;
        const float *xin = a.x + (size_t)img * a.H * a.W * 8;
#pragma unroll
        for (int k = 0; k < HE; ++k) {
            const int e = tid + k * 256;
            const int hy = e / ST_HW, hx = e - hy * ST_HW;
            const int gy = h0 - 3 + hy, gx = c0 - 3 + hx;
            pre4[k] = make_float4(0.f, 0.f, 0.f, 0.f);
            pre2[k] = make_float2(0.f, 0.f);
            if (e < ST_HH * ST_HW && (unsigned)gy < (unsigned)a.H && (unsigned)gx < (unsigned)a.W) {
                const float *p = xin + ((size_t)gy * a.W + gx) * 8;
                pre4[k] = *reinterpret_cast<const float4 *>(p);
                pre2[k] = *reinterpret_cast<const float2 *>(p + 4);
            }
        }
    };
    auto store_halo = [&]() {
#pragma unroll
        for (int k = 0; k < HE; ++k) {
            const int e = tid + k * 256;
            if (e >= ST_HH * ST_HW) break;
            const float f[6] = {pre4[k].x, pre4[k].y, pre4[k].z, pre4[k].w, pre2[k].x, pre2[k].y};
            unsigned hw[3], lw[3];
#pragma unroll
            for (int c = 0; c < 3; ++c) {
                const __bf16 h0 = (__bf16)f[2 * c], h1 = (__bf16)f[2 * c + 1];
                const __bf16 l0 = (__bf16)(f[2 * c] - (float)h0), l1 = (__bf16)(f[2 * c + 1] - (float)h1);
                hw[c] = (unsigned)__builtin_bit_cast(unsigned short, h0) | ((unsigned)__builtin_bit_cast(unsigned short, h1) << 16);
                lw[c] = (unsigned)__builtin_bit_cast(unsigned short, l0) | ((unsigned)__builtin_bit_cast(unsigned short, l1) << 16);
            }
            unsigned *ph = reinterpret_cast<unsigned *>(halo + e * ST_PIX);
            unsigned *pl = reinterpret_cast<unsigned *>(halo + ST_HPLANE + e * ST_PIX);
            ph[0] = hw[0]; ph[1] = hw[1]; ph[2] = hw[2];
            pl[0] = lw[0]; pl[1] = lw[1]; pl[2] = lw[2];
        }
    };
    const int tile0 = blockIdx.x * ST_GROUPS + group, tstride = gridDim.x * ST_GROUPS;
    if (tile0 < ntiles) fetch_halo(tile0);
    __syncthreads();
    for (int tile = tile0; tile < ntiles; tile += tstride) {
        const int img = tile / (tiles_y * tiles_x);
        const int trem = tile - img * (tiles_y * tiles_x);
        const int ty = trem / tiles_x, tx = trem - ty * tiles_x;
        const int h0 = ty * ST_ROWS, c0 = tx * ST_COLS;

        if (!(dbg & 8) || tile == tile0) store_halo();
        stem_group_barrier(gctr, gtarget, lane);
        if (!(dbg & 8) && tile + tstride < ntiles) fetch_halo(tile + tstride);

        f32x16 acc[2][2];
#pragma unroll
        for (int i = 0; i < 2; ++i)
#pragma unroll
            for (int j = 0; j < 2; ++j)
#pragma unroll
                for (int r = 0; r < 16; ++r) acc[i][j][r] = 0.f;
        struct Frags { f32x4 ah[2], al[2], bh[2], bl[2]; };
        auto load_frags = [&](int n, Frags &f) {
            const int kh = n / 3, s3 = n - 3 * kh;
            const int ao = a_base + kh * ST_HW * ST_PIX + s3 * 32, bo = b_base + kh * ST_WROW + s3 * 32;
            f.al[0] = *reinterpret_cast<const f32x4u *>(halo + ST_HPLANE + ao);
            f.bh[0] = *reinterpret_cast<const f32x4 *>(wts + bo);
            f.bh[1] = *reinterpret_cast<const f32x4 *>(wts + bo + 32 * ST_WPITCH);
            f.al[1] = *reinterpret_cast<const f32x4u *>(halo + ST_HPLANE + ao + 32 * ST_PIX);
            f.ah[0] = *reinterpret_cast<const f32x4u *>(halo + ao);
            f.bl[0] = *reinterpret_cast<const f32x4 *>(wts + ST_WPLANE + bo);
            f.bl[1] = *reinterpret_cast<const f32x4 *>(wts + ST_WPLANE + bo + 32 * ST_WPITCH);
            f.ah[1] = *reinterpret_cast<const f32x4u *>(halo + ao + 32 * ST_PIX);
        };
        Frags fr[2];
        load_frags(0, fr[0]);
        if (!(dbg & 4))
#pragma unroll
        for (int n = 0; n < 21; ++n) {
            const Frags &f = fr[n & 1];
            if (n + 1 < 21) load_frags(n + 1, fr[(n + 1) & 1]);
#pragma unroll
            for (int t = 0; t < 3; ++t)
#pragma unroll
                for (int i = 0; i < 2; ++i)
#pragma unroll
                    for (int j = 0; j < 2; ++j) {
                        const f32x4 a4 = t == 0 ? f.al[i] : f.ah[i];
                        const f32x4 b4 = t == 1 ? f.bl[j] : f.bh[j];
                        acc[i][j] = __builtin_amdgcn_mfma_f32_32x32x16_bf16(
                            __builtin_bit_cast(bf16x8_t, a4), __builtin_bit_cast(bf16x8_t, b4), acc[i][j], 0, 0, 0);
                    }
            if (n + 1 < 21) {
#pragma unroll
                for (int g2 = 0; g2 < 12; ++g2) {
                    __builtin_amdgcn_sched_group_barrier(0x008, 1, 0);
                    __builtin_amdgcn_sched_group_barrier(0x100, 1, 0);
                }
            }
            __builtin_amdgcn_sched_barrier(0);
        }

        const int col = lane & 31, rsel = 4 * (lane >> 5);
        const size_t prow = ((size_t)img * a.H + h0 + wrow) * a.W + c0 + whalf * 64;
        if (!(dbg & 1)) {
#pragma unroll
            for (int i = 0; i < 2; ++i)
#pragma unroll
                for (int r = 0; r < 16; ++r) {
                    const int px = i * 32 + (r & 3) + 8 * (r >> 2) + rsel;
                    float *yo = a.y + (prow + px) * 64 + col;
                    yo[0] = acc[i][0][r];
                    yo[32] = acc[i][1][r];
                }
        }
        if (a.partials && !(dbg & 2)) {
#pragma unroll
            for (int i = 0; i < 2; ++i)
#pragma unroll
                for (int j = 0; j < 2; ++j) {
                    float s = 0.f;
#pragma unroll
                    for (int r = 0; r < 16; ++r) s += acc[i][j][r];
                    s += __shfl_xor(s, 32);
                    const float mu = s * (1.f / 32.f);
                    float q = 0.f;
#pragma unroll
                    for (int r = 0; r < 16; ++r) {
                        const float d = acc[i][j][r] - mu;
                        q += d * d;
                    }
                    q += __shfl_xor(q, 32);
                    if (lane < 32) red[(wrow * 4 + whalf * 2 + i) * 64 + j * 32 + col] = make_float2(mu, q);
                }
        }
        stem_group_barrier(gctr, gtarget, lane);
        if (a.partials && tid < 128) {
            const int row = tid >> 6, c = tid & 63;
            float mean = 0.f;
#pragma unroll
            for (int w = 0; w < 4; ++w) mean += red[(row * 4 + w) * 64 + c].x;
            mean *= 0.25f;
            float m2 = 0.f;
#pragma unroll
            for (int w = 0; w < 4; ++w) {
                const float2 pr = red[(row * 4 + w) * 64 + c];
                const float d = pr.x - mean;
                m2 += pr.y + 32.f * d * d;
            }
            const size_t mtile = (((size_t)img * a.H + h0 + row) * a.W + c0) / kConvBM;
            a.partials[mtile * 64 + c] = make_float2(mean, m2);
        }
    }
}

}

bool stem_bf16x3_supported(int H, int W, int cin, int cin_pad, int cout, int k, int stride, int pad)
{
    return cin <= 6 && cin_pad == 8 && cout == 64 && k == 7 && stride == 1 && pad == 3 && W % ST_COLS == 0 && H % ST_ROWS == 0 &&
           kConvBM == 128;
}

void stem_pack_weights(const float *w, int cin, std::vector<unsigned char> &out)
{
    out.assign(kStemWBytes, 0);
    __bf16 *hi = reinterpret_cast<__bf16 *>(out.data());
    __bf16 *lo = reinterpret_cast<__bf16 *>(out.data() + kStemWBytes / 2);
    for (int co = 0; co < 64; ++co)
        for (int kh = 0; kh < 7; ++kh)
            for (int kw = 0; kw < 7; ++kw)
                for (int ci = 0; ci < cin && ci < 6; ++ci) {
                    const float v = w[(((size_t)co * cin + ci) * 7 + kh) * 7 + kw];
                    const size_t idx = (size_t)co * (kStemWPitch / 2) + (size_t)kh * kStemKRow + (size_t)kw * 6 + ci;
                    const __bf16 h = (__bf16)v;
                    hi[idx] = h;
                    lo[idx] = (__bf16)(v - (float)h);
                }
}

int launch_stem_bf16x3(const StemArgs &a, hipStream_t st, int max_workgroups)
{
    if (!a.x || !a.w || !a.y) LWG_FAIL(LWG_ERR_INVALID_ARG, "stem: NULL argument");
    if (a.N < 1 || a.H < 1 || a.W < 1 || max_workgroups < 0) LWG_FAIL(LWG_ERR_INVALID_ARG, "stem: empty tensor or negative grid cap");
    if (a.W % ST_COLS || a.H % ST_ROWS) LWG_FAIL(LWG_ERR_UNSUPPORTED, "stem: %dx%d is not a multiple of the 2x128 tile", a.H, a.W);
    static DeviceOnce opt_in;
    const int rc = opt_in_lds(reinterpret_cast<const void *>(&stem_bf16x3_kernel), ST_LDS, opt_in);
    if (rc != LWG_OK) return rc;
    const int ncu = device_cu_count();
    const int ntiles = a.N * (a.H / ST_ROWS) * (a.W / ST_COLS);
    const int want = ceil_div(ntiles, ST_GROUPS);
    int nwg = want < ncu ? want : ncu;
    if (max_workgroups > 0 && nwg > max_workgroups) nwg = max_workgroups;
#ifdef LWG_EXPERIMENTS
    static const int dbg = getenv("LWG_STEM_DBG") ? atoi(getenv("LWG_STEM_DBG")) : 0;
    StemArgs b = a;
    b.dbg = dbg;
    stem_bf16x3_kernel<<<nwg, 256 * ST_GROUPS, ST_LDS, st>>>(b);
#else
    stem_bf16x3_kernel<<<nwg, 256 * ST_GROUPS, ST_LDS, st>>>(a);
#endif
    LWG_LAUNCH_CHECK("stem_bf16x3_kernel");
    return LWG_OK;
}

}

using namespace lwg;

int lwg_stem_forward(const float *x, int N, int H, int W, const float *w_host, int cin, int precision, float *y, float *partials,
                     int max_workgroups, lwg_stream_t stream)
{
    LWG_REQUIRE(x && w_host && y, "stem_forward: NULL argument");
    LWG_REQUIRE(N >= 1 && H >= 1 && W >= 1, "stem_forward: empty tensor (N=%d, H=%d, W=%d)", N, H, W);
    LWG_REQUIRE(cin >= 1, "stem_forward: cin=%d", cin);
    LWG_REQUIRE(precision == 0 || precision == 1, "stem_forward: precision=%d (0: fp32, 1: bf16x3)", precision);
    LWG_REQUIRE(max_workgroups >= 0, "stem_forward: max_workgroups=%d", max_workgroups);
    LWG_REQUIRE((uintptr_t)x % 16 == 0 && (uintptr_t)y % 4 == 0 && (uintptr_t)partials % 8 == 0,
                "stem_forward: x must be 16-byte aligned (y 4, partials 8)");
    if (cin > 6) LWG_FAIL(LWG_ERR_UNSUPPORTED, "stem_forward: cin=%d, the NHWC8 stem carries at most 6 channels", cin);
    if (W % ST_COLS || H % ST_ROWS)
        LWG_FAIL(LWG_ERR_UNSUPPORTED, "stem_forward: %dx%d is not a multiple of the %dx%d tile", H, W, ST_ROWS, ST_COLS);
    if ((long)N * H * W > (1l << 24)) LWG_FAIL(LWG_ERR_UNSUPPORTED, "stem_forward: more than 2^24 pixels");
    hipStream_t st = as_stream(stream);

    ConvPhase ph = {};
    ph.KH = ph.KW = 7;
    ph.ntaps = 49;
    ph.Kpad = (int)align_up((size_t)49 * 8, kConvBK);
    std::vector<unsigned char> packed;
    if (precision == 1) {
        stem_pack_weights(w_host, cin, packed);
    } else {
        packed.assign((size_t)64 * ph.Kpad * sizeof(float), 0);
        float *h = reinterpret_cast<float *>(packed.data());
        for (int co = 0; co < 64; ++co)
            for (int ci = 0; ci < cin; ++ci)
                for (int t = 0; t < 49; ++t) h[(size_t)co * ph.Kpad + (size_t)t * 8 + ci] = w_host[((size_t)co * cin + ci) * 49 + t];
    }
    void *wdev = nullptr;
    LWG_HIP(hipMalloc(&wdev, packed.size()));
    int rc = LWG_OK;
    if (hipMemcpy(wdev, packed.data(), packed.size(), hipMemcpyHostToDevice) != hipSuccess) {
        set_error("stem_forward: weight upload failed");
        rc = LWG_ERR_HIP;
    } else if (precision == 1) {
        StemArgs s = {};
        s.x = x; s.N = N; s.H = H; s.W = W;
        s.w = wdev;
        s.y = y;
        s.partials = reinterpret_cast<float2 *>(partials);
        rc = launch_stem_bf16x3(s, st, max_workgroups);
    } else {
        ConvArgs a = {};
        a.x = x; a.ldx = 8;
        a.N = N; a.H = H; a.W = W; a.Cin = 8; a.cin_log2 = 3;
        a.w = static_cast<const float *>(wdev);
        a.y = y; a.ldy = 64;
        a.Ho = a.Hm = H; a.Wo = a.Wm = W; a.Cout = 64;
        a.stride = 1; a.pad = 3; a.os = 1; a.dil = 1;
        a.partials = reinterpret_cast<float2 *>(partials);
        a.mtiles = N * H * W / kConvBM;
        a.nphase = 1;
        a.ph[0] = ph;
        rc = launch_conv_igemm(a, 64, st);
    }
    if (hipStreamSynchronize(st) != hipSuccess && rc == LWG_OK) {
        set_error("stem_forward: the stem kernel failed");
        rc = LWG_ERR_HIP;
    }
    (void)hipFree(wdev);
    return rc;
}
```

impersonator_amd/csrc/generator.hip:

```cpp
#include <cmath>
#include <cstring>
#include <string>
#include <vector>

#include <cstdlib>

#include "conv.h"

namespace lwg {
namespace {

constexpr int kNDown = 3;
constexpr float kInEps = 1e-5f;

int ilog2(int v)
{
    int l = 0;
    while ((1 << l) < v) ++l;
    return l;
}

struct Layer {
    int cin = 0, cin_pad = 0, cout = 0, k = 0, stride = 1, pad = 0;
    bool transposed = false, has_norm = true;
    float *w = nullptr;
    float *w_split = nullptr;
    void *w_stem = nullptr;
    ConvPhase ph[4];
    int nphase = 1;
    float *gamma = nullptr, *beta = nullptr;
    bool got_w = false, got_g = false, got_b = false;
    size_t w_floats = 0;
};

struct StreamNet {
    Layer enc[kNDown + 1];
    std::vector<Layer> res;
    Layer dec[kNDown], skip[kNDown];
    float *heads_w = nullptr;
    void *heads_frag = nullptr;
    bool heads_frag_stale = true;
    bool got_img = false, got_att = false;
    bool has_skip = true;
};

}
}

using namespace lwg;

struct lwg_generator {
    int src_dim, tsf_dim, cd, repeat, is, max_batch;
    StreamNet src, tsf, bg;
    int bg_dim = 0;
    int ignored_keys = 0;

    float *x0 = nullptr;
    int x0_c = 8;
    float *raw = nullptr;
    float *cat[kNDown] = {};
    float *trunk[3] = {};
    float *sk[kNDown] = {};
    float *tscale[2][kNDown] = {};
    float2 *partials = nullptr;
    float2 *ss = nullptr;
    float *zeros = nullptr;
    size_t cat_floats[kNDown] = {}, trunk_floats = 0, sk_floats[kNDown] = {};
    int trunk_out = 0;
    int precision = 1;
    bool split = false;
    bool last_split = false;

    bool profile = false;
    std::vector<hipEvent_t> ev_pool;
    size_t ev_used = 0;
    std::vector<int> ev_variant;
    double prof_flops[kIgemmVariants] = {};
    int prof_launches[kIgemmVariants] = {};
};

namespace lwg {
namespace {

int dev_alloc(float **p, size_t floats)
{
    LWG_HIP(hipMalloc(reinterpret_cast<void **>(p), floats * sizeof(float)));
    return LWG_OK;
}

constexpr size_t kZeroTail = 1024;
int act_alloc(float **p, size_t floats)
{
    LWG_HIP(hipMalloc(reinterpret_cast<void **>(p), (floats + kZeroTail) * sizeof(float)));
    LWG_HIP(hipMemset(*p + floats, 0, kZeroTail * sizeof(float)));
    return LWG_OK;
}

void init_conv(Layer &L, int cin, int cout, int k, int stride, int pad)
{
    L.cin = cin;
    L.cin_pad = cin <= 8 ? 8 : cin <= 16 ? 16 : cin <= 32 ? 32 : cin;
    L.cout = cout;
    L.k = k;
    L.stride = stride;
    L.pad = pad;
    L.transposed = false;
    L.nphase = 1;
    ConvPhase &p = L.ph[0];
    p.KH = p.KW = k;
    p.ntaps = k * k;
    p.Kpad = (int)align_up((size_t)p.ntaps * L.cin_pad, kConvBK);
    p.w_off = 0;
    p.oy0 = p.ox0 = 0;
    L.w_floats = (size_t)cout * p.Kpad;
}

void init_convT(Layer &L, int cin, int cout)
{
    L.cin = L.cin_pad = cin;
    L.cout = cout;
    L.k = 3;
    L.stride = 1;
    L.pad = 0;
    L.transposed = true;
    L.nphase = 4;
    long off = 0;
    for (int py = 0; py < 2; ++py)
        for (int px = 0; px < 2; ++px) {
            ConvPhase &p = L.ph[py * 2 + px];
            p.KH = 1 + py;
            p.KW = 1 + px;
            p.ntaps = p.KH * p.KW;
            p.Kpad = (int)align_up((size_t)p.ntaps * cin, kConvBK);
            p.w_off = off;
            p.oy0 = py;
            p.ox0 = px;
            off += (long)cout * p.Kpad;
        }
    L.w_floats = (size_t)off;
}

int alloc_layer(Layer &L)
{
    int rc = dev_alloc(&L.w, L.w_floats);
    if (rc != LWG_OK) return rc;
    LWG_HIP(hipMemset(L.w, 0, L.w_floats * sizeof(float)));
    if (L.cin_pad >= kConvBK && L.k * L.k <= 32) {
        LWG_HIP(hipMalloc(reinterpret_cast<void **>(&L.w_split), L.w_floats * sizeof(float)));
        LWG_HIP(hipMemset(L.w_split, 0, L.w_floats * sizeof(float)));
    } else if (!L.transposed && stem_bf16x3_supported(kConvBM, kConvBM, L.cin, L.cin_pad, L.cout, L.k, L.stride, L.pad)) {
        LWG_HIP(hipMalloc(&L.w_stem, kStemWBytes));
        LWG_HIP(hipMemset(L.w_stem, 0, kStemWBytes));
    }
    if (L.has_norm) {
        if ((rc = dev_alloc(&L.gamma, L.cout)) != LWG_OK) return rc;
        if ((rc = dev_alloc(&L.beta, L.cout)) != LWG_OK) return rc;
    }
    return LWG_OK;
}

void free_layer(Layer &L)
{
    if (L.w) (void)hipFree(L.w);
    if (L.w_split) (void)hipFree(L.w_split);
    if (L.w_stem) (void)hipFree(L.w_stem);
    L.w_split = nullptr;
    L.w_stem = nullptr;
    if (L.gamma) (void)hipFree(L.gamma);
    if (L.beta) (void)hipFree(L.beta);
    L.w = L.gamma = L.beta = nullptr;
}

int build_stream(StreamNet &s, int in_dim, int cd, int repeat, bool with_decoder, bool with_skip = true)
{
    s.has_skip = with_skip;
    init_conv(s.enc[0], in_dim, cd, 7, 1, 3);
    for (int i = 1; i <= kNDown; ++i) init_conv(s.enc[i], cd << (i - 1), cd << i, 3, 2, 1);
    const int ct = cd << kNDown;
    s.res.resize(2 * repeat);
    for (auto &L : s.res) init_conv(L, ct, ct, 3, 1, 1);
    int rc;
    for (int i = 0; i <= kNDown; ++i)
        if ((rc = alloc_layer(s.enc[i])) != LWG_OK) return rc;
    for (auto &L : s.res)
        if ((rc = alloc_layer(L)) != LWG_OK) return rc;
    if (with_decoder) {
        int cur = ct;
        for (int i = 0; i < kNDown; ++i) {
            init_convT(s.dec[i], cur, cur / 2);
            if ((rc = alloc_layer(s.dec[i])) != LWG_OK) return rc;
            if (with_skip) {
                init_conv(s.skip[i], cur, cur / 2, 3, 1, 1);
                if ((rc = alloc_layer(s.skip[i])) != LWG_OK) return rc;
            }
            cur /= 2;
        }
        if ((rc = dev_alloc(&s.heads_w, 49 * 64 * 4)) != LWG_OK) return rc;
        LWG_HIP(hipMemset(s.heads_w, 0, 49 * 64 * 4 * sizeof(float)));
        LWG_HIP(hipMalloc(&s.heads_frag, heads_bf16x3_frag_bytes()));
        s.heads_frag_stale = true;
    }
    return LWG_OK;
}

void free_stream(StreamNet &s)
{
    for (auto &L : s.enc) free_layer(L);
    for (auto &L : s.res) free_layer(L);
    for (auto &L : s.dec) free_layer(L);
    for (auto &L : s.skip) free_layer(L);
    if (s.heads_w) (void)hipFree(s.heads_w);
    s.heads_w = nullptr;
    if (s.heads_frag) (void)hipFree(s.heads_frag);
    s.heads_frag = nullptr;
}

int upload_matrix(Layer &L, const std::vector<float> &h)
{
    LWG_HIP(hipMemcpy(L.w, h.data(), h.size() * sizeof(float), hipMemcpyHostToDevice));
    if (L.w_split) {
        std::vector<float> sp(h.size());
        split_bf16_groups(h.data(), h.size(), sp.data());
        LWG_HIP(hipMemcpy(L.w_split, sp.data(), sp.size() * sizeof(float), hipMemcpyHostToDevice));
    }
    L.got_w = true;
    return LWG_OK;
}

int upload_conv(Layer &L, const float *w, const int64_t *shape, int ndim, const char *key)
{
    if (ndim != 4 || shape[0] != L.cout || shape[1] != L.cin || shape[2] != L.k || shape[3] != L.k)
        LWG_FAIL(LWG_ERR_INVALID_ARG, "%s: expected shape (%d,%d,%d,%d)", key, L.cout, L.cin, L.k, L.k);
    const ConvPhase &p = L.ph[0];
    std::vector<float> h((size_t)L.cout * p.Kpad, 0.f);
    for (int co = 0; co < L.cout; ++co)
        for (int ci = 0; ci < L.cin; ++ci)
            for (int t = 0; t < L.k * L.k; ++t)
                h[(size_t)co * p.Kpad + (size_t)t * L.cin_pad + ci] = w[((size_t)co * L.cin + ci) * L.k * L.k + t];
    if (L.w_stem) {
        std::vector<unsigned char> packed;
        stem_pack_weights(w, L.cin, packed);
        LWG_HIP(hipMemcpy(L.w_stem, packed.data(), packed.size(), hipMemcpyHostToDevice));
    }
    return upload_matrix(L, h);
}

int upload_convT(Layer &L, const float *w, const int64_t *shape, int ndim, const char *key)
{
    if (ndim != 4 || shape[0] != L.cin || shape[1] != L.cout || shape[2] != 3 || shape[3] != 3)
        LWG_FAIL(LWG_ERR_INVALID_ARG, "%s: expected shape (%d,%d,3,3)", key, L.cin, L.cout);
    std::vector<float> h(L.w_floats, 0.f);
    for (int py = 0; py < 2; ++py)
        for (int px = 0; px < 2; ++px) {
            const ConvPhase &p = L.ph[py * 2 + px];
            for (int ty = 0; ty < p.KH; ++ty)
                for (int tx = 0; tx < p.KW; ++tx) {
                    const int ky = py == 0 ? 1 : (ty == 0 ? 2 : 0);
                    const int kx = px == 0 ? 1 : (tx == 0 ? 2 : 0);
                    const int t = ty * p.KW + tx;
                    for (int co = 0; co < L.cout; ++co)
                        for (int ci = 0; ci < L.cin; ++ci)
                            h[(size_t)p.w_off + (size_t)co * p.Kpad + (size_t)t * L.cin + ci] =
                                w[(((size_t)ci * L.cout + co) * 3 + ky) * 3 + kx];
                }
        }
    return upload_matrix(L, h);
}

int upload_vec(float *dst, int n, bool *flag, const float *src, const int64_t *shape, int ndim, const char *key)
{
    if (ndim != 1 || shape[0] != n) LWG_FAIL(LWG_ERR_INVALID_ARG, "%s: expected shape (%d,)", key, n);
    LWG_HIP(hipMemcpy(dst, src, (size_t)n * sizeof(float), hipMemcpyHostToDevice));
    *flag = true;
    return LWG_OK;
}

int upload_head(StreamNet &s, const float *w, const int64_t *shape, int ndim, int c0, int nc, int cd, const char *key)
{
    if (ndim != 4 || shape[0] != nc || shape[1] != cd || shape[2] != 7 || shape[3] != 7)
        LWG_FAIL(LWG_ERR_INVALID_ARG, "%s: expected shape (%d,%d,7,7)", key, nc, cd);
    std::vector<float> h(49 * 64 * 4);
    LWG_HIP(hipMemcpy(h.data(), s.heads_w, h.size() * sizeof(float), hipMemcpyDeviceToHost));
    for (int c = 0; c < nc; ++c)
        for (int ci = 0; ci < cd; ++ci)
            for (int t = 0; t < 49; ++t) h[((size_t)t * 64 + ci) * 4 + c0 + c] = w[((size_t)c * cd + ci) * 49 + t];
    LWG_HIP(hipMemcpy(s.heads_w, h.data(), h.size() * sizeof(float), hipMemcpyHostToDevice));
    s.heads_frag_stale = true;
    return LWG_OK;
}

int missing_in(const StreamNet &s, bool with_decoder)
{
    int m = 0;
    auto need = [&](const Layer &L) { m += !L.got_w + (L.has_norm ? (!L.got_g + !L.got_b) : 0); };
    for (auto &L : s.enc) need(L);
    for (auto &L : s.res) need(L);
    if (with_decoder) {
        for (auto &L : s.dec) need(L);
        if (s.has_skip) {
            for (auto &L : s.skip) need(L);
            m += !s.got_att;
        }
        m += !s.got_img;
    }
    return m;
}

#ifdef LWG_EXPERIMENTS
static int g_ko_passes = 0;
static bool ko(int bit)
{
    static const int mask = getenv("LWG_KO") ? atoi(getenv("LWG_KO")) : 0;
    return (mask & bit) && g_ko_passes >= 6;
}
#else
static constexpr bool ko(int) { return false; }
#endif

int prof_begin(lwg_generator *g, hipStream_t st, hipEvent_t *e1)
{
    if (g->ev_used + 2 > g->ev_pool.size()) {
        for (int i = 0; i < 64; ++i) {
            hipEvent_t e;
            LWG_HIP(hipEventCreate(&e));
            g->ev_pool.push_back(e);
        }
    }
    LWG_HIP(hipEventRecord(g->ev_pool[g->ev_used], st));
    *e1 = g->ev_pool[g->ev_used + 1];
    g->ev_used += 2;
    return LWG_OK;
}

const float *zero_tail_of(const lwg_generator *g, const float *x)
{
    for (int l = 0; l < kNDown; ++l) {
        if (g->cat[l] && x >= g->cat[l] && x < g->cat[l] + g->cat_floats[l]) return g->cat[l] + g->cat_floats[l];
        if (g->sk[l] && x >= g->sk[l] && x < g->sk[l] + g->sk_floats[l]) return g->sk[l] + g->sk_floats[l];
    }
    for (int i = 0; i < 3; ++i)
        if (g->trunk[i] && x >= g->trunk[i] && x < g->trunk[i] + g->trunk_floats) return g->trunk[i] + g->trunk_floats;
    return nullptr;
}

int conv_args(lwg_generator *g, const Layer &L, const float *x, int ldx, int N, int H, int W, float *raw, int ld_raw, int raw_from,
              ConvArgs &a, int &bn)
{
    a = ConvArgs{};
    a.x = x;
    a.ldx = ldx;
    a.N = N;
    a.H = H;
    a.W = W;
    a.Cin = L.cin_pad;
    a.cin_log2 = ilog2(L.cin_pad);
    a.w = L.w;
    a.w_split = L.w_split;
    a.precision = (g->split && L.w_split) ? 1 : 0;
    static const bool natural = getenv("LWG_NATURAL_TILE_ORDER") != nullptr;
    a.natural_order = natural ? 1 : 0;
    static const char *k_order = getenv("LWG_K_ORDER");
    a.tap_inner = (k_order && k_order[0] == 'c') ? 0 : 1;
    a.zeros = g->zeros;
    if (a.precision == 1) {
        a.zeros = zero_tail_of(g, x);
        if (!a.zeros) LWG_FAIL(LWG_ERR_STATE, "bf16x3 conv input is not one of the handle's activation buffers");
    }
    a.y = raw;
    a.ldy = ld_raw > 0 ? ld_raw : L.cout;
    a.Cout = L.cout;
    if (raw_from >= 0) {
        a.raw_in = 1;
        a.raw_from = raw_from;
        a.in_ss = g->ss;
        a.in_ss_ld = L.cin_pad - raw_from;
    }
    a.nphase = L.nphase;
    a.dil = 1;
    for (int p = 0; p < L.nphase; ++p) a.ph[p] = L.ph[p];
    if (L.transposed) {
        a.Hm = H; a.Wm = W; a.stride = 1; a.pad = 0; a.os = 2; a.Ho = 2 * H; a.Wo = 2 * W;
    } else {
        a.Hm = (H + 2 * L.pad - L.k) / L.stride + 1;
        a.Wm = (W + 2 * L.pad - L.k) / L.stride + 1;
        a.stride = L.stride; a.pad = L.pad; a.os = 1; a.Ho = a.Hm; a.Wo = a.Wm;
    }
    a.mtiles = N * a.Hm * a.Wm / kConvBM;
    a.partials = L.has_norm ? g->partials : nullptr;
    const long tiles128 = (long)a.mtiles * (L.cout / 128) * L.nphase;
    bn = (L.cout % 128 == 0 && tiles128 >= 256) ? 128 : 64;
    static const char *bn32_env = getenv("LWG_F32_BN32");
    if (bn == 64 && a.precision == 0 && !L.transposed && L.cin_pad >= kConvBK && L.k * L.k <= 32 && L.cout % 32 == 0 &&
        (long)a.mtiles * (L.cout / 64) * L.nphase * 2 <= 256 && !(bn32_env && bn32_env[0] == '0'))
        bn = 32;
    if (L.transposed) {
        if (a.precision == 1 && L.cout % 128 == 0) {
            bn = 128;
            a.fuse_phases = 0;
        } else {
            bn = 64;
            a.fuse_phases = 1;
        }
    }
    return LWG_OK;
}

bool takes_raw_input(lwg_generator *g, const Layer &L, const float *x, int ldx, int N, int H, int W, int raw_from)
{
    if (!g->split || !L.w_split) return false;
    ConvArgs a;
    int bn = 0;
    if (conv_args(g, L, x, ldx, N, H, W, g->raw, 0, raw_from, a, bn) != LWG_OK) return false;
    return conv_raw_input_supported(a, bn);
}

int run_conv(lwg_generator *g, const Layer &L, const float *x, int ldx, int N, int H, int W, float *raw, hipStream_t st,
             int ld_raw = 0, int raw_from = -1)
{
    ConvArgs a;
    int bn = 0;
    {
        const int rc0 = conv_args(g, L, x, ldx, N, H, W, raw, ld_raw, raw_from, a, bn);
        if (rc0 != LWG_OK) return rc0;
    }

    hipEvent_t e1 = nullptr;
    if (g->profile) {
        const int rc = prof_begin(g, st, &e1);
        if (rc != LWG_OK) return rc;
    }
    int variant = 0;
    int rc;
    if (g->split && L.w_stem && ldx == 8 && stem_bf16x3_supported(H, W, L.cin, L.cin_pad, L.cout, L.k, L.stride, L.pad)) {
        StemArgs s = {};
        s.x = x; s.N = N; s.H = H; s.W = W;
        s.w = L.w_stem;
        s.y = raw;
        s.partials = a.partials;
        rc = launch_stem_bf16x3(s, st);
        variant = kDirectStemBf16x3;
    } else {
        rc = launch_conv_igemm(a, bn, st, &variant);
    }
    if (rc != LWG_OK) return rc;
    if (g->profile) {
        LWG_HIP(hipEventRecord(e1, st));
        double k_alg = 0;
        for (int p = 0; p < L.nphase; ++p) k_alg += (double)L.ph[p].ntaps * L.cin;
        g->prof_flops[variant] += 2.0 * N * a.Hm * a.Wm * (double)L.cout * k_alg;
        g->prof_launches[variant] += 1;
        g->ev_variant.push_back(variant);
    }
    if (L.has_norm && !ko(1)) {
        rc = launch_in_finalize(g->partials, L.nphase, a.mtiles, N, L.cout, L.gamma, L.beta, kInEps, g->ss, st);
        if (rc != LWG_OK) return rc;
    }
    return LWG_OK;
}

struct Warp {
    const float *src = nullptr;
    const float *T = nullptr;
    int n = 1;
};

int run_apply(lwg_generator *g, int N, int H, int W, int C, bool relu, float *dst, int ld_dst, const float *res,
              int ld_res, const Warp *warps, int nwarp, int align, hipStream_t st)
{
    ApplyArgs a = {};
    a.raw = g->raw;
    a.C = C;
    a.N = N;
    a.H = H;
    a.W = W;
    a.scale_shift = g->ss;
    a.relu = relu;
    a.dst = dst;
    a.ld_dst = ld_dst;
    a.res = res;
    a.ld_res = ld_res;
    a.nwarp = nwarp;
    for (int k = 0; k < nwarp; ++k) {
        a.warp_src[k] = warps[k].src;
        a.warp_n[k] = warps[k].n;
        a.warp_T[k] = warps[k].T;
    }
    a.align_corners = align;
    a.split = g->split ? 1 : 0;
    return launch_apply(a, st);
}

int pack_input(lwg_generator *g, const float *x, int layout, int N, int C, int cpad, hipStream_t st, const float **out)
{
    if (layout == 1) {
        if (cpad != 8) LWG_FAIL(LWG_ERR_INVALID_ARG, "layout 1 (NHWC8) needs an input of at most 8 channels, this stream has %d", C);
        *out = x;
        return LWG_OK;
    }
    if (layout != 0) LWG_FAIL(LWG_ERR_INVALID_ARG, "layout must be 0 (NCHW) or 1 (NHWC8)");
    if (cpad > g->x0_c) LWG_FAIL(LWG_ERR_STATE, "packed-input buffer holds %d channels, %d needed", g->x0_c, cpad);
    const int rc = lwg_pack_nhwc(x, N, C, g->is, g->is, cpad, g->x0, st);
    *out = g->x0;
    return rc;
}

int run_encoder(lwg_generator *g, const StreamNet &s, int lvl, const float *x, int ldx, int N, float *dst, int ld_dst,
                const Warp *warps, int nwarp, int align, hipStream_t st)
{
    const Layer &L = s.enc[lvl];
    const int Hin = lvl == 0 ? g->is : g->is >> (lvl - 1);
    int rc = (lvl == 0 && &s == &g->tsf && ko(32)) ? LWG_OK : run_conv(g, L, x, ldx, N, Hin, Hin, g->raw, st);
    if (rc != LWG_OK) return rc;
    const int Ho = g->is >> lvl;
    if (&s == &g->tsf && ko(lvl == 0 ? 2 : 4)) return LWG_OK;
    return run_apply(g, N, Ho, Ho, L.cout, true, dst, ld_dst, nullptr, 0, warps, nwarp, align, st);
}

int run_resblock(lwg_generator *g, const StreamNet &s, int i, const float *xin, float *xout, int N,
                 const Warp *warps, int nwarp, int align, hipStream_t st)
{
    const int h = g->is >> kNDown, C = g->cd << kNDown;
    int rc;
    if (takes_raw_input(g, s.res[2 * i + 1], g->trunk[2], C, N, h, h, 0)) {
        if ((rc = run_conv(g, s.res[2 * i], xin, C, N, h, h, g->trunk[2], st, C)) != LWG_OK) return rc;
        if ((rc = run_conv(g, s.res[2 * i + 1], g->trunk[2], C, N, h, h, g->raw, st, 0, 0)) != LWG_OK) return rc;
    } else {
        if ((rc = run_conv(g, s.res[2 * i], xin, C, N, h, h, g->raw, st)) != LWG_OK) return rc;
        if ((rc = run_apply(g, N, h, h, C, true, g->trunk[2], C, nullptr, 0, nullptr, 0, align, st)) != LWG_OK) return rc;
        if ((rc = run_conv(g, s.res[2 * i + 1], g->trunk[2], C, N, h, h, g->raw, st)) != LWG_OK) return rc;
    }
    if (&s == &g->tsf && ko(8)) return LWG_OK;
    return run_apply(g, N, h, h, C, false, xout, C, xin, C, warps, nwarp, align, st);
}

int check_ready(const lwg_generator *g, int bs)
{
    if (!g) LWG_FAIL(LWG_ERR_INVALID_ARG, "NULL generator handle");
    if (bs <= 0 || bs > g->max_batch) LWG_FAIL(LWG_ERR_STATE, "batch %d outside 1..max_batch=%d", bs, g->max_batch);
    const int m = missing_in(g->src, false) + missing_in(g->tsf, true);
    if (m) LWG_FAIL(LWG_ERR_STATE, "%d weight tensors have not been loaded", m);
    return LWG_OK;
}

int run_tsf(lwg_generator *g, const float *tsf_inputs, int layout, const float *const T[2],
            const float *const *feats[2], int nsets, int bs, int align, float *color, float *mask, const float *bg,
            int bg_bs, float *pred, hipStream_t st, int feats_bs = 1)
{
    const StreamNet &s = g->tsf;
    const int is = g->is, cd = g->cd;
    int rc;
    g->split = g->last_split = g->precision == 1;
    for (int k = 0; k < nsets; ++k)
        for (int l = 1; l <= kNDown; ++l)
            if ((rc = lwg_resize_flow(T[k], bs, is, is, is >> l, is >> l, g->tscale[k][l - 1], st)) != LWG_OK) return rc;

    const float *x0 = nullptr;
    if ((rc = pack_input(g, tsf_inputs, layout, bs, g->tsf_dim, s.enc[0].cin_pad, st, &x0)) != LWG_OK) return rc;

    if ((rc = run_encoder(g, s, 0, x0, s.enc[0].cin_pad, bs, g->cat[0], 2 * cd, nullptr, 0, align, st)) != LWG_OK) return rc;
    for (int l = 1; l <= kNDown; ++l) {
        Warp w[2];
        for (int k = 0; k < nsets; ++k) {
            w[k].src = feats[k][l];
            w[k].T = g->tscale[k][l - 1];
            w[k].n = feats_bs;
        }
        const float *xin = g->cat[l - 1];
        const int ldx = 2 * (cd << (l - 1));
        float *dst = l < kNDown ? g->cat[l] : g->trunk[0];
        const int ld_dst = l < kNDown ? 2 * (cd << l) : (cd << l);
        if ((rc = run_encoder(g, s, l, xin, ldx, bs, dst, ld_dst, w, nsets, align, st)) != LWG_OK) return rc;
    }
    int cur = 0;
    for (int i = 0; i < g->repeat; ++i) {
        Warp w[2];
        for (int k = 0; k < nsets; ++k) {
            w[k].src = feats[k][kNDown + 1 + i];
            w[k].T = g->tscale[k][kNDown - 1];
            w[k].n = feats_bs;
        }
        if ((rc = run_resblock(g, s, i, g->trunk[cur], g->trunk[cur ^ 1], bs, w, nsets, align, st)) != LWG_OK) return rc;
        cur ^= 1;
    }
    g->trunk_out = cur;
    const float *d = g->trunk[cur];
    int dC = cd << kNDown, dH = is >> kNDown;
    bool d_raw = false;
    for (int i = 0; i < kNDown; ++i) {
        const int lvl = kNDown - 1 - i, oC = dC / 2, oH = dH * 2;
        const bool last = i + 1 == kNDown;
        const bool skip_takes_raw = takes_raw_input(g, s.skip[i], g->cat[lvl], 2 * oC, bs, oH, oH, oC);
        if (!(last && ko(128)) &&
            (rc = run_conv(g, s.dec[i], d, dC, bs, dH, dH, skip_takes_raw ? g->cat[lvl] + oC : g->raw, st, skip_takes_raw ? 2 * oC : 0,
                           d_raw ? 0 : -1)) != LWG_OK)
            return rc;
        if (!skip_takes_raw &&
            (rc = run_apply(g, bs, oH, oH, oC, true, g->cat[lvl] + oC, 2 * oC, nullptr, 0, nullptr, 0, align, st)) != LWG_OK)
            return rc;
        const bool next_takes_raw = !last && takes_raw_input(g, s.dec[i + 1], g->sk[i], oC, bs, oH, oH, 0);
        if (!(last && ko(64)) &&
            (rc = run_conv(g, s.skip[i], g->cat[lvl], 2 * oC, bs, oH, oH, next_takes_raw ? g->sk[i] : g->raw, st, 0,
                           skip_takes_raw ? oC : -1)) != LWG_OK)
            return rc;
        if (!last) {
            if (!next_takes_raw &&
                (rc = run_apply(g, bs, oH, oH, oC, true, g->sk[i], oC, nullptr, 0, nullptr, 0, align, st)) != LWG_OK)
                return rc;
            d = g->sk[i];
            d_raw = next_takes_raw;
        }
        dC = oC;
        dH = oH;
    }
    HeadsArgs h = {};
    h.x = g->raw;
    h.N = bs;
    h.H = is;
    h.W = is;
    h.scale_shift = g->ss;
    h.wh = s.heads_w;
    h.color = color;
    h.mask = mask;
    h.bg = bg;
    h.bg_bs = bg_bs;
    h.pred = pred;
#ifdef LWG_EXPERIMENTS
    ++g_ko_passes;
#endif
    if (ko(16)) return LWG_OK;
    if (!g->split) return launch_heads(h, st);
    if (g->tsf.heads_frag_stale) {
        if ((rc = launch_heads_pack(s.heads_w, s.heads_frag, st)) != LWG_OK) return rc;
        g->tsf.heads_frag_stale = false;
    }
    return launch_heads_bf16x3(h, s.heads_frag, st);
}

}
}

extern "C" {

int lwg_generator_create(lwg_generator **out, int src_dim, int tsf_dim, int conv_dim, int repeat_num, int image_size,
                         int max_batch)
{
    LWG_REQUIRE(out, "generator_create: NULL out");
    *out = nullptr;
    LWG_REQUIRE(src_dim > 0 && src_dim <= 32 && tsf_dim > 0 && tsf_dim <= 32, "generator_create: input dims must be 1..32");
    LWG_REQUIRE(repeat_num > 0 && max_batch > 0, "generator_create: repeat_num/max_batch must be positive");
    if (conv_dim != 64)
        LWG_FAIL(LWG_ERR_UNSUPPORTED, "generator_create: conv_dim=%d (the kernels are built for the reference's 64)", conv_dim);
    const int hb = image_size >> kNDown;
    if (image_size <= 0 || (image_size & 7) || (hb * hb) % kConvBM != 0)
        LWG_FAIL(LWG_ERR_UNSUPPORTED, "generator_create: image_size=%d; (image_size/8)^2 must be a multiple of %d",
                 image_size, kConvBM);
    int ndev = 0;
    LWG_HIP(hipGetDeviceCount(&ndev));

    lwg_generator *g = new lwg_generator();
    g->src_dim = src_dim;
    g->tsf_dim = tsf_dim;
    g->cd = conv_dim;
    g->repeat = repeat_num;
    g->is = image_size;
    g->max_batch = max_batch;
    int rc = build_stream(g->src, src_dim, conv_dim, repeat_num, true);
    if (rc == LWG_OK) rc = build_stream(g->tsf, tsf_dim, conv_dim, repeat_num, true);

    const size_t B = (size_t)max_batch, P = (size_t)image_size * image_size;
    const int cd = conv_dim;
    if (rc == LWG_OK) {
        g->x0_c = g->src.enc[0].cin_pad > g->tsf.enc[0].cin_pad ? g->src.enc[0].cin_pad : g->tsf.enc[0].cin_pad;
        rc = dev_alloc(&g->x0, B * P * g->x0_c);
    }
    if (rc == LWG_OK) rc = dev_alloc(&g->raw, B * P * cd);
    for (int l = 0; l < kNDown && rc == LWG_OK; ++l) rc = act_alloc(&g->cat[l], g->cat_floats[l] = B * (P >> (2 * l)) * (size_t)(2 * (cd << l)));
    for (int i = 0; i < 3 && rc == LWG_OK; ++i) rc = act_alloc(&g->trunk[i], g->trunk_floats = B * (P >> (2 * kNDown)) * (size_t)(cd << kNDown));
    for (int i = 0; i + 1 < kNDown && rc == LWG_OK; ++i) {
        const int lvl = kNDown - 1 - i;
        rc = act_alloc(&g->sk[i], g->sk_floats[i] = B * (P >> (2 * lvl)) * (size_t)(cd << lvl));
    }
    for (int k = 0; k < 2; ++k)
        for (int l = 1; l <= kNDown && rc == LWG_OK; ++l) rc = dev_alloc(&g->tscale[k][l - 1], B * (P >> (2 * l)) * 2);
    if (rc == LWG_OK) {
        size_t need = 0;
        for (int l = 0; l <= kNDown; ++l) {
            const size_t tiles = B * (P >> (2 * l)) / kConvBM;
            const size_t c = (size_t)(cd << l);
            need = need > tiles * c ? need : tiles * c;
        }
        float *p = nullptr;
        rc = dev_alloc(&p, need * 2);
        g->partials = reinterpret_cast<float2 *>(p);
    }
    if (rc == LWG_OK) {
        float *p = nullptr;
        rc = dev_alloc(&p, B * (size_t)(cd << kNDown) * 2);
        g->ss = reinterpret_cast<float2 *>(p);
    }
    if (rc == LWG_OK) rc = dev_alloc(&g->zeros, 64);
    if (rc == LWG_OK && hipMemset(g->zeros, 0, 64 * sizeof(float)) != hipSuccess) {
        set_error("hipMemset of the zero page failed");
        rc = LWG_ERR_HIP;
    }
    if (rc != LWG_OK) {
        lwg_generator_destroy(g);
        return rc;
    }
    *out = g;
    return LWG_OK;
}

void lwg_generator_destroy(lwg_generator *g)
{
    if (!g) return;
    free_stream(g->src);
    free_stream(g->tsf);
    free_stream(g->bg);
    auto fr = [](void *p) { if (p) (void)hipFree(p); };
    fr(g->x0);
    fr(g->raw);
    for (auto p : g->cat) fr(p);
    for (auto p : g->trunk) fr(p);
    for (auto p : g->sk) fr(p);
    for (auto &k : g->tscale)
        for (auto p : k) fr(p);
    fr(g->partials);
    fr(g->ss);
    fr(g->zeros);
    for (auto e : g->ev_pool) (void)hipEventDestroy(e);
    delete g;
}

int lwg_generator_load_weight(lwg_generator *g, const char *key, const float *data_host, const int64_t *shape, int ndim)
{
    LWG_REQUIRE(g && key && data_host && shape, "load_weight: NULL argument");
    std::string k(key);
    if (k.rfind("module.", 0) == 0) k = k.substr(7);
    if (k.rfind("bg_model.", 0) == 0) {
        if (!g->bg_dim) {
            g->ignored_keys++;
            return LWG_OK;
        }
        StreamNet &b = g->bg;
        int idx = -1, sub = -1;
        char tail[32] = {0};
        const int res0 = 3 + 3 * kNDown, up0 = res0 + g->repeat, fin = up0 + 3 * kNDown;
        auto put = [&](Layer &L, bool norm, const char *what) -> int {
            if (!norm && !strcmp(what, "weight"))
                return L.transposed ? upload_convT(L, data_host, shape, ndim, key) : upload_conv(L, data_host, shape, ndim, key);
            if (norm && !strcmp(what, "weight")) return upload_vec(L.gamma, L.cout, &L.got_g, data_host, shape, ndim, key);
            if (norm && !strcmp(what, "bias")) return upload_vec(L.beta, L.cout, &L.got_b, data_host, shape, ndim, key);
            LWG_FAIL(LWG_ERR_INVALID_ARG, "load_weight: unknown key '%s'", key);
        };
        if (sscanf(k.c_str(), "bg_model.model.%d.main.%d.%31s", &idx, &sub, tail) == 3 && idx >= res0 && idx < up0) {
            const int i = idx - res0;
            if (sub == 0 || sub == 1) return put(b.res[2 * i], sub == 1, tail);
            if (sub == 3 || sub == 4) return put(b.res[2 * i + 1], sub == 4, tail);
            LWG_FAIL(LWG_ERR_INVALID_ARG, "load_weight: unknown key '%s'", key);
        }
        if (sscanf(k.c_str(), "bg_model.model.%d.%31s", &idx, tail) == 2) {
            if (idx == fin && !strcmp(tail, "weight")) {
                const int rc = upload_head(b, data_host, shape, ndim, 0, 3, g->cd, key);
                if (rc == LWG_OK) b.got_img = true;
                return rc;
            }
            if (idx >= 0 && idx < res0) return put(b.enc[idx / 3], idx % 3 == 1, tail);
            if (idx >= up0 && idx < fin) return put(b.dec[(idx - up0) / 3], (idx - up0) % 3 == 1, tail);
        }
        LWG_FAIL(LWG_ERR_INVALID_ARG, "load_weight: unknown key '%s'", key);
    }
    StreamNet *s = nullptr;
    bool is_tsf = false;
    if (k.rfind("src_model.", 0) == 0) s = &g->src;
    else if (k.rfind("tsf_model.", 0) == 0) { s = &g->tsf; is_tsf = true; }
    else LWG_FAIL(LWG_ERR_INVALID_ARG, "load_weight: unknown key '%s'", key);
    k = k.substr(10);

    int i = -1, j = -1;
    char tail[32] = {0};
    auto norm_or_conv = [&](Layer &L, int sub, const char *what) -> int {
        if (sub == 0 && !strcmp(what, "weight"))
            return L.transposed ? upload_convT(L, data_host, shape, ndim, key) : upload_conv(L, data_host, shape, ndim, key);
        if (sub == 1 && !strcmp(what, "weight")) return upload_vec(L.gamma, L.cout, &L.got_g, data_host, shape, ndim, key);
        if (sub == 1 && !strcmp(what, "bias")) return upload_vec(L.beta, L.cout, &L.got_b, data_host, shape, ndim, key);
        LWG_FAIL(LWG_ERR_INVALID_ARG, "load_weight: unknown key '%s'", key);
    };
    if (sscanf(k.c_str(), "encoders.%d.%d.%31s", &i, &j, tail) == 3 && i >= 0 && i <= kNDown)
        return norm_or_conv(s->enc[i], j, tail);
    if (sscanf(k.c_str(), "resnets.%d.main.%d.%31s", &i, &j, tail) == 3 && i >= 0 && i < g->repeat) {
        if (j == 0 || j == 1) return norm_or_conv(s->res[2 * i], j, tail);
        if (j == 3 || j == 4) return norm_or_conv(s->res[2 * i + 1], j - 3, tail);
        LWG_FAIL(LWG_ERR_INVALID_ARG, "load_weight: unknown key '%s'", key);
    }
    const bool dec = sscanf(k.c_str(), "decoders.%d.%d.%31s", &i, &j, tail) == 3;
    const bool skp = !dec && sscanf(k.c_str(), "skippers.%d.%d.%31s", &i, &j, tail) == 3;
    if ((dec || skp) && i >= 0 && i < kNDown) {
        return norm_or_conv(dec ? s->dec[i] : s->skip[i], j, tail);
    }
    if (k == "img_reg.0.weight" || k == "attetion_reg.0.weight") {
        const bool img = k[0] == 'i';
        const int rc = upload_head(*s, data_host, shape, ndim, img ? 0 : 3, img ? 3 : 1, g->cd, key);
        if (rc == LWG_OK) (img ? s->got_img : s->got_att) = true;
        return rc;
    }
    LWG_FAIL(LWG_ERR_INVALID_ARG, "load_weight: unknown key '%s'", key);
}

int lwg_generator_missing_weights(const lwg_generator *g)
{
    if (!g) return -1;
    return missing_in(g->src, false) + missing_in(g->tsf, true);
}

int lwg_generator_num_src_features(const lwg_generator *g) { return g ? kNDown + 1 + g->repeat : 0; }

int lwg_generator_src_feature_shape(const lwg_generator *g, int index, int *C, int *H, int *W)
{
    LWG_REQUIRE(g && C && H && W, "src_feature_shape: NULL argument");
    LWG_REQUIRE(index >= 0 && index < kNDown + 1 + g->repeat, "src_feature_shape: index %d out of range", index);
    const int lvl = index <= kNDown ? index : kNDown;
    *C = g->cd << lvl;
    *H = *W = g->is >> lvl;
    return LWG_OK;
}

int lwg_generator_encode_src(lwg_generator *g, const float *src_inputs_nchw, float *const *feats_nhwc,
                             lwg_stream_t stream)
{
    return lwg_generator_encode_src_n(g, src_inputs_nchw, 1, feats_nhwc, stream);
}

int lwg_generator_encode_src_n(lwg_generator *g, const float *src_inputs_nchw, int bs, float *const *feats_nhwc,
                               lwg_stream_t stream)
{
    int rc = check_ready(g, bs);
    if (rc != LWG_OK) return rc;
    LWG_REQUIRE(src_inputs_nchw && feats_nhwc, "encode_src: NULL argument");
    for (int i = 0; i < kNDown + 1 + g->repeat; ++i) LWG_REQUIRE(feats_nhwc[i], "encode_src: feats_nhwc[%d] is NULL", i);
    hipStream_t st = as_stream(stream);
    g->split = false;
    const float *x0 = nullptr;
    if ((rc = pack_input(g, src_inputs_nchw, 0, bs, g->src_dim, g->src.enc[0].cin_pad, st, &x0)) != LWG_OK) return rc;
    const float *x = x0;
    int ldx = g->src.enc[0].cin_pad;
    for (int l = 0; l <= kNDown; ++l) {
        const int C = g->cd << l;
        if ((rc = run_encoder(g, g->src, l, x, ldx, bs, feats_nhwc[l], C, nullptr, 0, 0, st)) != LWG_OK) return rc;
        x = feats_nhwc[l];
        ldx = C;
    }
    for (int i = 0; i < g->repeat; ++i) {
        float *o = feats_nhwc[kNDown + 1 + i];
        if ((rc = run_resblock(g, g->src, i, x, o, bs, nullptr, 0, 0, st)) != LWG_OK) return rc;
        x = o;
    }
    return LWG_OK;
}

int lwg_generator_decode_src(lwg_generator *g, const float *const *feats_nhwc, int bs, float *color, float *mask,
                             lwg_stream_t stream)
{
    int rc = check_ready(g, bs);
    if (rc != LWG_OK) return rc;
    LWG_REQUIRE(feats_nhwc && color && mask, "decode_src: NULL argument");
    const int miss = missing_in(g->src, true);
    if (miss) LWG_FAIL(LWG_ERR_STATE, "%d source-stream weight tensors (decoder / heads) have not been loaded", miss);
    hipStream_t st = as_stream(stream);
    const StreamNet &s = g->src;
    const int is = g->is, cd = g->cd;
    g->split = g->last_split = false;
    for (int l = 0; l < kNDown; ++l) {
        LWG_REQUIRE(feats_nhwc[l], "decode_src: feats_nhwc[%d] is NULL", l);
        const size_t C = (size_t)cd << l, P = (size_t)bs * (is >> l) * (is >> l);
        LWG_HIP(hipMemcpy2DAsync(g->cat[l], 2 * C * sizeof(float), feats_nhwc[l], C * sizeof(float), C * sizeof(float), P,
                                 hipMemcpyDeviceToDevice, st));
    }
    const float *d = feats_nhwc[kNDown + g->repeat];
    LWG_REQUIRE(d, "decode_src: the last residual feature is NULL");
    int dC = cd << kNDown, dH = is >> kNDown;
    for (int i = 0; i < kNDown; ++i) {
// ... 224 lines not shown
```

impersonator_amd/csrc/train.hip:

```cpp
#include <algorithm>
#include <cmath>
#include <cstring>
#include <string>
#include <vector>

#include "conv.h"
#include "split.h"
#include "sample.h"

namespace lwg {
namespace {

typedef float f32x16 __attribute__((ext_vector_type(16)));
constexpr float kLeaky = 0.2f;
constexpr float kEps = 1e-5f;

__device__ __forceinline__ float4 ld4(const float *p) { return *reinterpret_cast<const float4 *>(p); }

constexpr int RS_CH = 16, RS_SL = 16;
__global__ __launch_bounds__(256) void in_stats_kernel(const float *__restrict__ x, int HW, int C, float2 *__restrict__ out)
{
    __shared__ double sh[2][RS_SL][RS_CH];
    const int cl = threadIdx.x & (RS_CH - 1), c = blockIdx.x * RS_CH + cl, slice = threadIdx.x / RS_CH, n = blockIdx.y;
    const float *p = x + (size_t)n * HW * C + c;
// ... 2542 lines not shown
    for (int i = 0; i < 7; ++i) {
        if (wm + 2 * i >= HG_MT) continue;
#pragma unroll
        for (int r = 0; r < 16; ++r) {
            const int m = (wm + 2 * i) * 32 + (r & 3) + 8 * (r >> 2) + 4 * (lane >> 5);
            if (m < HG_M) o[(size_t)m * 64 + c] = acc[i][r];
        }
    }
}

__global__ __launch_bounds__(256) void heads_wgrad_reduce_kernel(const float *__restrict__ part, int S, float *__restrict__ dw)
{
    const int i = blockIdx.x * blockDim.x + threadIdx.x;
    if (i >= HG_M * 64) return;
    float s = 0.f;
    for (int k = 0; k < S; ++k) s += part[(size_t)k * HG_M * 64 + i];
    const int c = i & 63, m = i >> 6, o = m & 7, tap = m >> 3;
    const int ky = 6 - tap / 7, kx = 6 - tap % 7;
    dw[(((size_t)o * 64 + c) * 7 + ky) * 7 + kx] = s;
}

constexpr long kHeadsMaxSlices = 512;
long heads_wgrad_slices(int N, int H, int W, long *steps_per_slice)
{
    const long total = (long)N * H * ceil_div(W, HG_PX);
    long S = kHeadsMaxSlices;
    if (S > total) S = total;
    *steps_per_slice = ceil_div(total, S);
    return ceil_div(total, *steps_per_slice);
}
constexpr size_t kHeadsWFloats = 49 * 64 * 4;

}

size_t lwg_heads_workspace_bytes(int N, int H, int W)
{
    if (N < 1 || H < 1 || W < 1) return 0;
    const size_t fwd = kHeadsWFloats + (size_t)N * 64 * 2, wg = (size_t)kHeadsMaxSlices * HG_M * 64;
    return (fwd > wg ? fwd : wg) * sizeof(float);
}

int lwg_heads_forward(const float *x, int N, int H, int W, const float *w, int w_rows, float *color, float *mask, void *ws,
                      size_t ws_bytes, lwg_stream_t stream)
{
    LWG_REQUIRE(x && w && ws && (color || mask), "heads_forward: NULL argument");
    if (w_rows < 4) LWG_FAIL(LWG_ERR_INVALID_ARG, "heads_forward: the weight tensor needs >= 4 rows (3 colour + 1 mask), got %d", w_rows);
    if (ws_bytes < lwg_heads_workspace_bytes(N, H, W)) LWG_FAIL(LWG_ERR_INVALID_ARG, "heads_forward: workspace too small");
    hipStream_t st = reinterpret_cast<hipStream_t>(stream);
    float *wh = static_cast<float *>(ws);
    float2 *ss = reinterpret_cast<float2 *>(wh + kHeadsWFloats);
    heads_weight_kernel<<<ceil_div((long)kHeadsWFloats, 256), 256, 0, st>>>(w, wh);
    LWG_LAUNCH_CHECK("heads_weight_kernel");
    fill_identity_norm_kernel<<<ceil_div((long)N * 64, 256), 256, 0, st>>>(ss, N * 64);
    LWG_LAUNCH_CHECK("fill_identity_norm_kernel");
    HeadsArgs h = {};
    h.x = x; h.N = N; h.H = H; h.W = W;
    h.scale_shift = ss;
    h.wh = wh;
    h.color = color;
    h.mask = mask;
    return launch_heads(h, st);
}

size_t lwg_heads_inference_workspace_bytes(int N, int H, int W)
{
    if (N < 1 || H < 1 || W < 1) return 0;
    return kHeadsWFloats * sizeof(float) + heads_bf16x3_frag_bytes();
}

int lwg_heads_inference(const float *x, int N, int H, int W, const float *scale_shift, const float *w, int w_rows, int precision,
                        const float *bg, int bg_bs, float *color, float *mask, float *pred, int bands, void *ws, size_t ws_bytes,
                        lwg_stream_t stream)
{
    LWG_REQUIRE(x && scale_shift && w && ws && (color || mask || pred), "heads_inference: NULL argument");
    LWG_REQUIRE(N >= 1 && H >= 1 && W >= 1, "heads_inference: empty tensor (N=%d, H=%d, W=%d)", N, H, W);
    if (w_rows < 4) LWG_FAIL(LWG_ERR_INVALID_ARG, "heads_inference: the weight tensor needs >= 4 rows (3 colour + 1 mask), got %d", w_rows);
    LWG_REQUIRE(precision == 0 || precision == 1, "heads_inference: precision=%d (0: fp32, 1: bf16x3)", precision);
    LWG_REQUIRE(bands >= 0, "heads_inference: bands=%d", bands);
    LWG_REQUIRE(!pred || bg, "heads_inference: pred requested without a background image");
    LWG_REQUIRE(!bg || bg_bs == 1 || bg_bs == N, "heads_inference: bg_bs=%d, must be 1 or the batch size %d", bg_bs, N);
    LWG_REQUIRE(((uintptr_t)x | (uintptr_t)ws) % 16 == 0 && (uintptr_t)scale_shift % 8 == 0,
                "heads_inference: x and the workspace must be 16-byte aligned (scale_shift 8)");
    if ((long)N * H * W > (1l << 24)) LWG_FAIL(LWG_ERR_UNSUPPORTED, "heads_inference: more than 2^24 pixels");
    if (ws_bytes < lwg_heads_inference_workspace_bytes(N, H, W))
        LWG_FAIL(LWG_ERR_WORKSPACE, "heads_inference: workspace of %zu bytes, %zu needed", ws_bytes,
                 lwg_heads_inference_workspace_bytes(N, H, W));
    hipStream_t st = reinterpret_cast<hipStream_t>(stream);
    float *wh = static_cast<float *>(ws);
    void *wfrag = wh + kHeadsWFloats;
    heads_weight_kernel<<<ceil_div((long)kHeadsWFloats, 256), 256, 0, st>>>(w, wh);
    LWG_LAUNCH_CHECK("heads_weight_kernel");
    HeadsArgs h = {};
    h.x = x; h.N = N; h.H = H; h.W = W;
    h.scale_shift = reinterpret_cast<const float2 *>(scale_shift);
    h.wh = wh;
    h.color = color;
    h.mask = mask;
    h.bg = bg;
    h.bg_bs = bg ? bg_bs : 1;
    h.pred = pred;
    if (precision == 0) return launch_heads(h, st);
    const int rc = launch_heads_pack(wh, wfrag, st);
    if (rc != LWG_OK) return rc;
    return launch_heads_bf16x3(h, wfrag, st, bands);
}

namespace {
int norm_conv_tile(const lwg_conv2d_desc *d, int mtiles, int nphase, int *fuse)
{
    *fuse = 0;
    if (d->transposed) {
        if (d->precision == 1 && d->Cout % 128 == 0) return 128;
        *fuse = 1;
        return 64;
    }
    const long tiles128 = (long)mtiles * (d->Cout / 128) * nphase;
    int bn = (d->Cout % 128 == 0 && tiles128 >= 256) ? 128 : 64;
    static const char *bn32_env = getenv("LWG_F32_BN32");
    if (bn == 64 && d->precision == 0 && d->Cin >= kConvBK && d->k * d->k <= 32 && d->Cout % 32 == 0 &&
        (long)mtiles * (d->Cout / 64) * nphase * 2 <= 256 && !(bn32_env && bn32_env[0] == '0'))
        bn = 32;
    return bn;
}
lwg_conv2d_desc norm_conv_ws_desc(const lwg_conv2d_desc *d)
{
    lwg_conv2d_desc w = *d;
    w.precision = 1;
    return w;
}
}

size_t lwg_norm_conv_workspace_bytes(const lwg_conv2d_desc *d)
{
    if (!d) return 0;
    const lwg_conv2d_desc w = norm_conv_ws_desc(d);
    return lwg_conv2d_workspace_bytes(&w);
}

int lwg_norm_conv_forward(const lwg_conv2d_desc *d, const float *x, const float *w, int bn, const float *in_scale_shift,
                          int raw_from, float *y, float *partials, int *variant_host, void *ws, size_t ws_bytes,
                          lwg_stream_t stream)
{
    ConvGeom g;
    int rc = conv_geom(d, &g);
    if (rc != LWG_OK) return rc;
    LWG_REQUIRE(x && w && y && partials && ws, "norm_conv_forward: NULL argument");
    LWG_REQUIRE(d->precision == 0 || d->precision == 1, "norm_conv_forward: precision=%d (0: fp32, 1: bf16x3)", d->precision);
    LWG_REQUIRE(bn == 0 || bn == 32 || bn == 64 || bn == 128, "norm_conv_forward: bn=%d (0: the generator's rule, 32, 64, 128)", bn);
    LWG_REQUIRE(((uintptr_t)x | (uintptr_t)w | (uintptr_t)y) % 16 == 0 && (uintptr_t)partials % 8 == 0,
                "norm_conv_forward: x, w and y must be 16-byte aligned (partials 8)");
    LWG_REQUIRE(!in_scale_shift || (uintptr_t)in_scale_shift % 8 == 0, "norm_conv_forward: in_scale_shift must be 8-byte aligned");
    LWG_REQUIRE((uintptr_t)ws % 16 == 0 && d->pad >= 0, "norm_conv_forward: the workspace must be 16-byte aligned, pad >= 0");
    if (in_scale_shift && d->precision != 1)
        LWG_FAIL(LWG_ERR_UNSUPPORTED, "norm_conv_forward: raw input is taken by the bf16x3 halo kernels only");
    {
        const lwg_conv2d_desc wd = norm_conv_ws_desc(d);
        const size_t need = lwg_conv2d_workspace_bytes(&wd);
        if (ws_bytes < need) LWG_FAIL(LWG_ERR_WORKSPACE, "norm_conv_forward: workspace of %zu bytes, %zu needed", ws_bytes, need);
    }
    hipStream_t st = reinterpret_cast<hipStream_t>(stream);
    const SplitWs sw = carve_split(d, g, ws);
    const bool split = d->precision == 1;
    float *wm = split ? sw.w : static_cast<float *>(ws);

    ConvArgs a = base_args(x, d->Cin, d->N, d->H, d->Cin, wm, y, d->Cout);
    a.W = d->W;
    a.general = 0;
    a.tap_inner = 1;
    a.dil = 1;
    a.zeros = sw.zeros;
    a.partials = reinterpret_cast<float2 *>(partials);
    if (d->transposed) {
        a.Hm = d->H; a.Wm = d->W; a.Ho = 2 * d->H; a.Wo = 2 * d->W;
        a.stride = 1; a.pad = 0; a.os = 2;
        a.nphase = 4;
        long off = 0;
        for (int p = 0; p < 4; ++p) {
            const int py = p >> 1, px = p & 1, nt = (1 + py) * (1 + px);
            a.ph[p] = ConvPhase{1 + py, 1 + px, nt, nt * d->Cin, off, py, px, 0, 0};
            off += (long)d->Cout * nt * d->Cin;
        }
    } else {
        a.Hm = a.Ho = g.Ho; a.Wm = a.Wo = g.Wo;
        a.stride = d->stride; a.pad = d->pad; a.os = 1;
        a.nphase = 1;
        a.ph[0] = ConvPhase{d->k, d->k, d->k * d->k, (int)align_up((size_t)d->k * d->k * d->Cin, kConvBK), 0, 0, 0, 0, 0};
    }
    if (((long)d->N * a.Hm * a.Wm) % kConvBM)
        LWG_FAIL(LWG_ERR_UNSUPPORTED, "norm_conv_forward: %d x %dx%d output pixels are not whole 128-pixel tiles", d->N, a.Hm, a.Wm);
    a.mtiles = d->N * a.Hm * a.Wm / kConvBM;
    int fuse = 0;
    const int bn_rule = norm_conv_tile(d, a.mtiles, a.nphase, &fuse);
    a.fuse_phases = fuse;
    if (bn == 0) bn = bn_rule;
    if (split) {
        if (d->Cin % 32) LWG_FAIL(LWG_ERR_UNSUPPORTED, "norm_conv_forward: the bf16x3 path needs Cin %% 32 == 0, got %d", d->Cin);
        a.x = sw.x;
        a.w_split = sw.w;
        a.precision = 1;
    }
    if (in_scale_shift) {
        a.raw_in = 1;
        a.raw_from = raw_from;
        a.in_ss = reinterpret_cast<const float2 *>(in_scale_shift);
        a.in_ss_ld = d->Cin - raw_from;
    }
    if ((rc = check_conv_igemm(a, bn)) != LWG_OK) return rc;

    const size_t x_floats = (size_t)d->N * d->H * d->W * d->Cin;
    if (d->transposed) {
        if ((rc = relayout(w, wm, 2, d->Cin, d->Cout, 9, (long)g.w_floats, st, 0, split)) != LWG_OK) return rc;
    } else if ((rc = relayout(w, wm, 0, d->Cout, d->Cin, d->k * d->k, (long)g.w_floats, st, a.ph[0].Kpad, split)) != LWG_OK) {
        return rc;
    }
    if (split) {
        if ((rc = split_pack(x, sw.x, x_floats, st, sw.zeros, sw.zero_floats)) != LWG_OK) return rc;
        if (in_scale_shift)
            LWG_HIP(hipMemcpy2DAsync(sw.x + raw_from, (size_t)d->Cin * sizeof(float), x + raw_from, (size_t)d->Cin * sizeof(float),
                                     (size_t)(d->Cin - raw_from) * sizeof(float), (size_t)d->N * d->H * d->W,
                                     hipMemcpyDeviceToDevice, st));
    } else {
        LWG_HIP(hipMemsetAsync(sw.zeros, 0, sw.zero_floats * sizeof(float), st));
    }
    int variant = -1;
    if ((rc = launch_conv_igemm(a, bn, st, &variant)) != LWG_OK) return rc;
    if (variant_host) *variant_host = variant;
    return LWG_OK;
}

int lwg_norm_finalize(const float *partials, int nphase, int mtiles, int N, int C, const float *gamma, const float *beta, float eps,
                      float *scale_shift, lwg_stream_t stream)
{
    LWG_REQUIRE(partials && gamma && beta && scale_shift, "norm_finalize: NULL argument");
    LWG_REQUIRE(nphase >= 1 && nphase <= 4 && mtiles >= 1 && N >= 1 && C >= 1,
                "norm_finalize: bad sizes (nphase=%d, mtiles=%d, N=%d, C=%d)", nphase, mtiles, N, C);
    LWG_REQUIRE(eps >= 0.f, "norm_finalize: eps=%g", (double)eps);
    LWG_REQUIRE(((uintptr_t)partials | (uintptr_t)scale_shift) % 8 == 0 && ((uintptr_t)gamma | (uintptr_t)beta) % 4 == 0,
                "norm_finalize: partials and scale_shift must be 8-byte aligned");
    if (mtiles % N) LWG_FAIL(LWG_ERR_UNSUPPORTED, "norm_finalize: %d tiles do not split over %d images", mtiles, N);
    if (N > 65535) LWG_FAIL(LWG_ERR_UNSUPPORTED, "norm_finalize: N=%d above the grid's 65535", N);
    return launch_in_finalize(reinterpret_cast<const float2 *>(partials), nphase, mtiles, N, C, gamma, beta, eps,
                              reinterpret_cast<float2 *>(scale_shift), reinterpret_cast<hipStream_t>(stream));
}

int lwg_norm_apply(const float *raw, int N, int H, int W, int C, const float *scale_shift, int relu, float *dst, int ld_dst,
                   const float *res, int ld_res, int split, int nwarp, const float *warp_src0, int warp_n0, const float *warp_T0,
                   const float *warp_src1, int warp_n1, const float *warp_T1, int align_corners, int lanes, lwg_stream_t stream)
{
    LWG_REQUIRE(raw && scale_shift && dst, "norm_apply: NULL argument");
    LWG_REQUIRE(N >= 1 && H >= 1 && W >= 1 && C >= 4, "norm_apply: bad sizes (N=%d, H=%d, W=%d, C=%d)", N, H, W, C);
    LWG_REQUIRE(nwarp >= 0 && nwarp <= 2, "norm_apply: nwarp=%d (0..2)", nwarp);
    LWG_REQUIRE(lanes == 0 || lanes == 4 || lanes == 8, "norm_apply: lanes=%d (0: the launcher's choice, 4, 8)", lanes);
    LWG_REQUIRE((split == 0 || split == 1) && (relu == 0 || relu == 1) && (align_corners == 0 || align_corners == 1),
                "norm_apply: split, relu and align_corners are 0 or 1");
    LWG_REQUIRE(ld_dst >= C && (!res || ld_res >= C), "norm_apply: pixel strides below C=%d (ld_dst=%d, ld_res=%d)", C, ld_dst, ld_res);
    const float *wsrc[2] = {warp_src0, warp_src1}, *wT[2] = {warp_T0, warp_T1};
    const int wn[2] = {warp_n0, warp_n1};
    for (int k = 0; k < nwarp; ++k) {
        LWG_REQUIRE(wsrc[k] && wT[k], "norm_apply: NULL warp term %d", k);
        LWG_REQUIRE(wn[k] == 1 || wn[k] == N, "norm_apply: warp_n%d=%d, must be 1 or the batch size %d", k, wn[k], N);
        LWG_REQUIRE((uintptr_t)wsrc[k] % 16 == 0 && (uintptr_t)wT[k] % 8 == 0, "norm_apply: warp term %d is not 16 / 8-byte aligned", k);
    }
    LWG_REQUIRE(((uintptr_t)raw | (uintptr_t)scale_shift | (uintptr_t)dst | (uintptr_t)res) % 16 == 0,
                "norm_apply: raw, scale_shift, dst and res must be 16-byte aligned");
    if ((C & 3) || (ld_dst & 3) || (res && (ld_res & 3)))
        LWG_FAIL(LWG_ERR_UNSUPPORTED, "norm_apply: channel counts / strides must be multiples of 4 (C=%d)", C);
    if (split && ((C & 31) || (ld_dst & 31) || ((uintptr_t)dst & 127) || (res && ((ld_res & 31) || ((uintptr_t)res & 127)))))
        LWG_FAIL(LWG_ERR_UNSUPPORTED, "norm_apply: split-bf16 buffers need 32-channel granularity and 128-byte alignment (C=%d)", C);
    if (lanes == 8 && !split) LWG_FAIL(LWG_ERR_UNSUPPORTED, "norm_apply: eight channels per thread is the split-bf16 kernel");
    if ((long)N * H * W * (C >> 2) > (1l << 31) - 256) LWG_FAIL(LWG_ERR_UNSUPPORTED, "norm_apply: tensor too large for one launch");
    ApplyArgs a = {};
    a.raw = raw; a.C = C; a.N = N; a.H = H; a.W = W;
    a.scale_shift = reinterpret_cast<const float2 *>(scale_shift);
    a.relu = relu;
    a.dst = dst; a.ld_dst = ld_dst;
    a.res = res; a.ld_res = res ? ld_res : 0;
    a.split = split;
    a.nwarp = nwarp;
    for (int k = 0; k < nwarp; ++k) { a.warp_src[k] = wsrc[k]; a.warp_n[k] = wn[k]; a.warp_T[k] = wT[k]; }
    a.align_corners = align_corners;
    return launch_apply(a, reinterpret_cast<hipStream_t>(stream), lanes);
}

int lwg_heads_backward_weight(const float *x, const float *dy8, int N, int H, int W, float *dw, void *ws, size_t ws_bytes,
                              lwg_stream_t stream)
{
    LWG_REQUIRE(x && dy8 && dw && ws, "heads_backward_weight: NULL argument");
    if (N < 1 || H < 1 || W < 1) LWG_FAIL(LWG_ERR_INVALID_ARG, "heads_backward_weight: empty tensor");
    if (ws_bytes < lwg_heads_workspace_bytes(N, H, W)) LWG_FAIL(LWG_ERR_INVALID_ARG, "heads_backward_weight: workspace too small");
    hipStream_t st = reinterpret_cast<hipStream_t>(stream);
    long per = 0;
    const long S = heads_wgrad_slices(N, H, W, &per);
    float *part = static_cast<float *>(ws);
    wgrad_heads_kernel<<<(unsigned)S, 256, 0, st>>>(x, dy8, N, H, W, per, part);
    LWG_LAUNCH_CHECK("wgrad_heads_kernel");
    heads_wgrad_reduce_kernel<<<ceil_div((long)HG_M * 64, 256), 256, 0, st>>>(part, (int)S, dw);
    LWG_LAUNCH_CHECK("heads_wgrad_reduce_kernel");
    return LWG_OK;
}

size_t lwg_instance_norm_scratch_bytes(int N, int HW, int C)
{
    if (N < 1 || HW < 1 || C < RS_CH) return 0;
    const int S4 = C % RS4_CH == 0 ? in_bwd_slabs4(N, C, HW) : 1, S1 = in_slabs(N, C, HW);
    return (size_t)N * (S4 > S1 ? S4 : S1) * C * 2 * sizeof(double) + (size_t)N * C * 2 * sizeof(float);
}

// ... 200 lines not shown
```

Measured before the change: 4200 frames/s.

## Fuse stem instance-norm apply into the 256-row ring bf16x3 conv via raw input

Adds a RAW variant of the 256-row ring bf16x3 implicit-GEMM kernel that loads un-normalised activations, then applies the per-channel scale/shift and ReLU and splits to bf16 hi/lo in LDS ahead of each stage barrier. The generator writes the stem's raw output straight into cat[0] with its own scale/shift buffer, and enc[1] and the last skip conv consume it directly. This removes the separate apply pass and its full-resolution read/write. In exchange it adds conversion work and vmcnt waits inside the pipelined main loop, more LDS, and more complex routing.

```diff
diff --git a/impersonator_amd/csrc/conv.h b/impersonator_amd/csrc/conv.h
--- a/impersonator_amd/csrc/conv.h
+++ b/impersonator_amd/csrc/conv.h
@@ -74,6 +74,7 @@
     const float *x; int N, H, W;
     const void *w;
     float *y;
+    int ldy;
     float2 *partials;
     int dbg;
 };
@@ -82,7 +83,7 @@
 int launch_stem_bf16x3(const StemArgs &a, hipStream_t st, int max_workgroups = 0);
 
 int launch_in_finalize(const float2 *partials, int nphase, int mtiles, int N, int C, const float *gamma,
-                       const float *beta, float eps, float2 *scale_shift, hipStream_t st);
+                       const float *beta, float eps, float2 *scale_shift, hipStream_t st, int ss_ld = 0);
 
 struct ApplyArgs {
     const float *raw; int C;
diff --git a/impersonator_amd/csrc/conv.hip b/impersonator_amd/csrc/conv.hip
--- a/impersonator_amd/csrc/conv.hip
+++ b/impersonator_amd/csrc/conv.hip
@@ -574,8 +574,8 @@
     igemm_dma_body<BN, WM, WN, DBG, NS>(a);
 }
 
-template <int BN, int WM, int WN, int NS = 3, int DBG = 0, int BMT = BM>
-__global__ __launch_bounds__(64 * (BMT / (32 * WM)) * (BN / (32 * WN))) void conv_igemm_bf16x3(const ConvArgs a)
+template <int BN, int WM, int WN, int NS, int DBG, int BMT, bool RAW>
+__device__ __forceinline__ void ring_bf16x3_body(const ConvArgs &a)
 {
     constexpr int WAVES_N = BN / (32 * WN), WAVES_M = BMT / (32 * WM), NW = WAVES_M * WAVES_N;
     static_assert((NW == 4 || NW == 8) && NS >= 3, "wave layout");
@@ -657,6 +657,8 @@
     }
     int s_tap = 0, s_kh = 0, s_kw = 0;
     unsigned s_ci_b = 0, s_w_b = 0;
+    [[maybe_unused]] int tap_new = 0, tap_now = 0;
+    [[maybe_unused]] unsigned ci_new = 0, ci_now = 0;
     auto retap = [&]() {
         const int tapoff = (s_kh * a.W + s_kw) * a.dil * a.ldx;
 #pragma unroll
@@ -667,6 +669,12 @@
     const unsigned wave_b = __builtin_amdgcn_readfirstlane(lds_base + (unsigned)((BMT * BK + wave * B_CH * 8 * BK) * 4));
     auto dma_piece = [&](int p, int kt, int slot) {
         const unsigned slot_byte = (unsigned)(slot * STAGE * 4);
+        if constexpr (RAW) {
+            if (p == 0) {
+                tap_new = s_tap;
+                ci_new = s_ci_b;
+            }
+        }
         if (p < A_CH) {
             dma16(cur[p], x_base + s_ci_b, wave_a + slot_byte + (unsigned)(p * 8 * BK * 4));
         } else {
@@ -701,12 +709,20 @@
 #pragma unroll
             for (int r = 0; r < 16; ++r) acc[i][j][r] = 0.f;
 
-    const int frow = lane & 31, fsw = (frow >> 1) & 7;
-    const int a_row = (wave_m * 32 * WM + frow) * BK;
-    const int b_row = BMT * BK + (wave_n * 32 * WN + frow) * BK;
-    int fcol[4];
-#pragma unroll
-    for (int c = 0; c < 4; ++c) fcol[c] = (((2 * c + (lane >> 5)) ^ fsw) * 4);
+    int a_row, b_row, fcol[4];
+    auto frag_geometry = [&](int l) {
+        const int frow = l & 31, fsw = (frow >> 1) & 7;
+        a_row = (wave_m * 32 * WM + frow) * BK;
+        b_row = BMT * BK + (wave_n * 32 * WN + frow) * BK;
+#pragma unroll
+        for (int c = 0; c < 4; ++c) fcol[c] = (((2 * c + (l >> 5)) ^ fsw) * 4);
+    };
+    frag_geometry(lane);
+    [[maybe_unused]] auto opaque_lane = [&]() {
+        int l = lane;
+        asm volatile("" : "+v"(l));
+        return l;
+    };
     struct Frags { float4 ah[WM], al[WM], bh[WN], bl[WN]; };
     auto load_frags = [&](int slot, int kb, Frags &f) {
         const float *As = smem + slot * STAGE + a_row;
@@ -736,10 +752,59 @@
     constexpr int RPM = (NL + (Q - QB) - 1) / (Q - QB);
     Frags fr;
 
+    static_assert(!RAW || (A_CH % 2 == 0 && NS == 3 && !(DBG & 1024)), "RAW: chunk parity per piece, one stage ahead");
+    constexpr int DUMMY = NS * STAGE;
+    constexpr int SSOFF = DUMMY + 8 * BK;
+    struct Conv { float4 v; uint2 h, l; };
+    [[maybe_unused]] Conv cv;
+    struct CvStage { int rd, hi; float4 sa, sb; };
+    [[maybe_unused]] auto cv_stage = [&](unsigned ci_b) {
+        const int l = opaque_lane(), lr2 = l >> 4, g = (l ^ lr2) & 7;
+        const float *q = reinterpret_cast<const float *>(reinterpret_cast<const char *>(smem + SSOFF) + (ci_b << 1) + g * 32);
+        return CvStage{l << 4, ((l >> 3) << 7) + ((((g >> 1) ^ lr2) & 7) << 4) + ((g & 1) << 3), *reinterpret_cast<const float4 *>(q),
+                       *reinterpret_cast<const float4 *>(q + 4)};
+    };
+    [[maybe_unused]] auto wait_vm = [](int n) {
+        switch (n) {
+#define LWG_WAIT_VM(N) case N: asm volatile("s_waitcnt vmcnt(" #N ")" ::: "memory"); break;
+            LWG_WAIT_VM(1) LWG_WAIT_VM(2) LWG_WAIT_VM(3) LWG_WAIT_VM(4) LWG_WAIT_VM(5) LWG_WAIT_VM(6) LWG_WAIT_VM(7) LWG_WAIT_VM(8)
+            LWG_WAIT_VM(9) LWG_WAIT_VM(10) LWG_WAIT_VM(11) LWG_WAIT_VM(12) LWG_WAIT_VM(13) LWG_WAIT_VM(14) LWG_WAIT_VM(15)
+#undef LWG_WAIT_VM
+            default: asm volatile("s_waitcnt vmcnt(0)" ::: "memory"); break;
+        }
+    };
+    [[maybe_unused]] auto convert_step = [&](const CvStage &ca, int p, int slot, int step, int nyoung, int tap) {
+        const int par64 = (p & 1) << 6;
+        const int chunk = (slot * STAGE + (wave * A_CH + p) * 8 * BK) * 4;
+        char *base = reinterpret_cast<char *>(smem);
+        if (step == 0) {
+            if (nyoung >= 0) wait_vm(nyoung);
+            cv.v = *reinterpret_cast<const float4 *>(base + chunk + (ca.rd ^ par64));
+        } else if (step == 1) {
+            cv.v.x = fmaxf(fmaf(cv.v.x, ca.sa.x, ca.sa.y), 0.f);
+            cv.v.y = fmaxf(fmaf(cv.v.y, ca.sa.z, ca.sa.w), 0.f);
+            cv.v.z = fmaxf(fmaf(cv.v.z, ca.sb.x, ca.sb.y), 0.f);
+            cv.v.w = fmaxf(fmaf(cv.v.w, ca.sb.z, ca.sb.w), 0.f);
+        } else if (step == 2) {
+            split_pair(cv.v.x, cv.v.y, cv.h.x, cv.l.x);
+            split_pair(cv.v.z, cv.v.w, cv.h.y, cv.l.y);
+        } else {
+            const bool live = (amask[p] >> tap) & 1u;
+            const int hi_at = live ? chunk + (ca.hi ^ par64) : DUMMY * 4 + ca.rd;
+            *reinterpret_cast<uint2 *>(base + hi_at) = cv.h;
+            *reinterpret_cast<uint2 *>(base + (live ? hi_at ^ 64 : hi_at + 8)) = cv.l;
+        }
+    };
+    constexpr int NSTEP = 4 * A_CH, QC0 = QB - NSTEP;
+    static_assert(!RAW || QC0 >= 0, "RAW: the conversion of a stage's chunks fits ahead of the stage barrier");
+    [[maybe_unused]] const int nk_raw = ph.Kpad / BK;
+
     auto stage_body = [&](int kt, auto slot_c, auto do_dma) {
         constexpr int slot = decltype(slot_c)::value;
         constexpr int slot1 = (slot + 1) % NS, slot2 = (slot + NS - 1) % NS;
         Frags f1, nx;
+        [[maybe_unused]] CvStage ca = {};
+        if constexpr (RAW) frag_geometry(opaque_lane());
         if (DBG & 256) load_frags(slot, 1, f1);
 #pragma unroll
         for (int q = 0; q < Q; ++q) {
@@ -800,21 +865,62 @@
                     __builtin_amdgcn_sched_barrier(0);
                 }
             }
+            if constexpr (RAW) {
+                if (q >= QC0 && q < QB && (decltype(do_dma)::value || kt + 1 < nk_raw)) {
+                    const int cp = (q - QC0) / 4, issued = decltype(do_dma)::value ? ((q + 1) * LPS) / Q : 0;
+                    __builtin_amdgcn_sched_barrier(0);
+                    if (q == QC0) ca = cv_stage(ci_now);
+                    convert_step(ca, cp, slot1, (q - QC0) % 4, (A_CH - 1 - cp) + B_CH + issued, tap_now);
+                    __builtin_amdgcn_sched_barrier(0);
+                }
+            }
         }
         if (!(DBG & 8)) fr = nx;
+        if constexpr (RAW) {
+            tap_now = tap_new;
+            ci_now = ci_new;
+        }
     };
 
     const int nk = ph.Kpad / BK;
+    if constexpr (RAW) {
+        const float2 *ss = a.in_ss + (size_t)img * a.in_ss_ld;
+        for (int i2 = tid; i2 < a.Cin; i2 += NW * 64) reinterpret_cast<float2 *>(smem + SSOFF)[i2] = ss[i2];
+        asm volatile("s_waitcnt vmcnt(0)" ::: "memory");
+    }
+    [[maybe_unused]] int tap_first = 0;
+    [[maybe_unused]] unsigned ci_first = 0;
 #pragma unroll
     for (int st = 0; st < NS - 1; ++st)
         if (st < nk) {
 #pragma unroll
             for (int p = 0; p < LPS; ++p) dma_piece(p, st, st);
+            if constexpr (RAW) {
+                if (st == 0) {
+                    tap_first = tap_new;
+                    ci_first = ci_new;
+                }
+            }
         }
     if (nk >= NS - 1) {
         asm volatile("s_waitcnt vmcnt(%0)" ::"n"((NS - 2) * LPS) : "memory");
     } else {
         asm volatile("s_waitcnt vmcnt(0)" ::: "memory");
+    }
+    if constexpr (RAW) {
+        asm volatile("s_waitcnt lgkmcnt(0)" ::: "memory");
+        __builtin_amdgcn_s_barrier();
+        asm volatile("" ::: "memory");
+        const CvStage ca = cv_stage(ci_first);
+#pragma unroll
+        for (int p = 0; p < A_CH; ++p) {
+#pragma unroll
+            for (int step = 0; step < 4; ++step) convert_step(ca, p, 0, step, -1, tap_first);
+            __builtin_amdgcn_sched_barrier(0);
+        }
+        asm volatile("s_waitcnt lgkmcnt(0)" ::: "memory");
+        tap_now = tap_new;
+        ci_now = ci_new;
     }
     __builtin_amdgcn_s_barrier();
     asm volatile("" ::: "memory");
@@ -876,6 +982,18 @@
     }
     __syncthreads();
     }
+}
+
+template <int BN, int WM, int WN, int NS = 3, int DBG = 0, int BMT = BM>
+__global__ __launch_bounds__(64 * (BMT / (32 * WM)) * (BN / (32 * WN))) void conv_igemm_bf16x3(const ConvArgs a)
+{
+    ring_bf16x3_body<BN, WM, WN, NS, DBG, BMT, false>(a);
+}
+
+template <int BN, int WM, int WN, int NS = 3, int BMT = 256>
+__global__ __launch_bounds__(64 * (BMT / (32 * WM)) * (BN / (32 * WN))) void conv_igemm_bf16x3_raw(const ConvArgs a)
+{
+    ring_bf16x3_body<BN, WM, WN, NS, 0, BMT, true>(a);
 }
 
 template <int NHW, int B_CH, int Q, int QB, int NS, int HT = 7>
@@ -1347,7 +1465,7 @@
 __global__ __launch_bounds__(256) void in_finalize_kernel(const float2 *__restrict__ partials, int nphase, int mtiles,
                                                           int tiles_per_img, int C, const float *__restrict__ gamma,
                                                           const float *__restrict__ beta, float eps,
-                                                          float2 *__restrict__ scale_shift)
+                                                          float2 *__restrict__ scale_shift, int ss_ld)
 {
     __shared__ double sh[3][FIN_SL][FIN_CH];
     const int cl = threadIdx.x & (FIN_CH - 1);
@@ -1386,7 +1504,7 @@
         const double var = (m2 + BM * between) / (cnt * BM);
         const double inv = 1.0 / sqrt(var + (double)eps);
         const float sc = (float)(gamma[c] * inv);
-        scale_shift[(size_t)n * C + c] = make_float2(sc, (float)(beta[c] - mean * gamma[c] * inv));
+        scale_shift[(size_t)n * ss_ld + c] = make_float2(sc, (float)(beta[c] - mean * gamma[c] * inv));
     }
 }
 
@@ -1675,11 +1793,14 @@
 constexpr int halo3x3_px(int bmt) { return (bmt / 32 + 2) * (32 + 2); }
 constexpr int kHaloCTPx = (4 + 1) * (32 + 1);
 constexpr size_t raw_lds(int channels) { return (size_t)8 * BK * sizeof(float) + (size_t)channels * sizeof(float2); }
+constexpr int kRingRawMaxChannels = 128;
+constexpr int kRingRawMinPixels = 128 * 128;
+constexpr size_t ring_raw_lds(int channels) { return (size_t)8 * BK * sizeof(float) + (size_t)channels * sizeof(float2); }
 
 enum ConvKernelId {
     kF32_64, kF32_128, kF32_Small, kGen_64, kGen_128, kGen_Small, kGenX3_64, kGenX3_128, kGenX3_Small,
     kDma_32, kDma_64, kDma_128,
-    kRing_64, kRing_128_3, kRing_128_4, kRing_128_Traced, kRing_128_Tall,
+    kRing_64, kRing_128_3, kRing_128_4, kRing_128_Traced, kRing_128_Tall, kRingRaw_128_Tall,
     kHalo_64, kHalo_128, kHalo_Tall, kHaloRaw_64, kHaloRaw_128, kHaloRaw_Tall,
     kHaloCT_64, kHaloCT_128, kHaloCTRaw_64, kHaloCTRaw_128,
 #ifdef LWG_EXPERIMENTS
@@ -1705,6 +1826,8 @@
     {&conv_igemm_bf16x3<128, 2, 2, 4>, 256, ring_lds(4, 128), kIgemmBf16x3_128, "conv_igemm_bf16x3"},
     {&conv_igemm_bf16x3<128, 2, 2, 4, 512>, 256, ring_lds(4, 128), kIgemmBf16x3_128, "conv_igemm_bf16x3 (traced)"},
     {&conv_igemm_bf16x3<128, 2, 2, 3, 0, 256>, 512, ring_lds(3, 128, 256), kIgemmBf16x3_128, "conv_igemm_bf16x3 (256-row tiles)"},
+    {&conv_igemm_bf16x3_raw<128, 2, 2>, 512, ring_lds(3, 128, 256) + ring_raw_lds(kRingRawMaxChannels), kIgemmBf16x3_128,
+     "conv_igemm_bf16x3_raw (256-row tiles)"},
     {&conv3x3_halo_bf16x3<64, 1, 2, 3, 32>, 256, halo_lds(halo3x3_px(128), 3, 64), kHaloBf16x3_64, "conv3x3_halo_bf16x3"},
     {&conv3x3_halo_bf16x3<128, 2, 2, 4, 32>, 256, halo_lds(halo3x3_px(128), 4, 128), kHaloBf16x3_128, "conv3x3_halo_bf16x3"},
     {&conv3x3_halo_bf16x3<128, 2, 2, 4, 32, 256>, 512, halo_lds(halo3x3_px(256), 4, 128), kHaloBf16x3_128, "conv3x3_halo_bf16x3"},
@@ -1739,7 +1862,8 @@
 }
 
 struct ConvSwitches {
-    bool halo, halo_tall, ct_wide, ring3, ring_tall, fused_apply;
+    bool halo, halo_tall, ct_wide, ring3, ring_tall, fused_apply, fused_stem;
+    int stem_min_pixels;
     char ring_exp;
 };
 static const ConvSwitches &conv_switches()
@@ -1752,19 +1876,31 @@
                             first("LWG_RING") == '3',
                             first("LWG_RING_TALL") != '0',
                             first("LWG_FUSED_APPLY") != '0',
+                            first("LWG_FUSED_STEM") != '0',
+                            getenv("LWG_FUSED_STEM_MIN_PIXELS") ? atoi(getenv("LWG_FUSED_STEM_MIN_PIXELS")) : kRingRawMinPixels,
                             first("LWG_RING")};
     }();
     return sw;
 }
 
-static bool raw_input_route(const ConvArgs &a, int bn, const ConvSwitches &sw)
-{
-    if (!sw.halo || !sw.fused_apply) return false;
+static bool ring_tall_shape(const ConvArgs &a, int bn, int ncu, const ConvSwitches &sw, bool tracing)
+{
+    return bn == 128 && !a.fuse_phases && a.nphase == 1 && (a.mtiles & 1) == 0 && (a.Hm * a.Wm) % 256 == 0 && !tracing &&
+           (long)(a.mtiles / 2) * (a.Cout / 128) >= ncu && sw.ring_tall;
+}
+
+static bool raw_input_route(const ConvArgs &a, int bn, int ncu, const ConvSwitches &sw, bool tracing)
+{
+    if (!sw.fused_apply) return false;
     if (a.precision != 1 || a.general || !a.w_split || (a.ldx & 31) || (a.Cin & 31) || a.Cin < 32 || (bn != 64 && bn != 128)) return false;
-    if (a.raw_from < 0 || (a.raw_from & 31) || a.raw_from >= a.Cin || a.Cin - a.raw_from > kRawMaxChannels) return false;
-    return halo3x3_shape(a) || haloCT_shape(a);
-}
-bool conv_raw_input_supported(const ConvArgs &a, int bn) { return raw_input_route(a, bn, conv_switches()); }
+    if (a.raw_from < 0 || (a.raw_from & 31) || a.raw_from >= a.Cin) return false;
+    if (sw.halo && (halo3x3_shape(a) || haloCT_shape(a))) return a.Cin - a.raw_from <= kRawMaxChannels;
+    return sw.fused_stem && a.raw_from == 0 && a.Cin <= kRingRawMaxChannels && ring_tall_shape(a, bn, ncu, sw, tracing) && a.Hm * a.Wm >= sw.stem_min_pixels;
+}
+bool conv_raw_input_supported(const ConvArgs &a, int bn)
+{
+    return raw_input_route(a, bn, device_cu_count(), conv_switches(), g_trace.buf != nullptr);
+}
 
 struct ConvLaunch { const ConvKernel *k; dim3 grid; size_t lds; int trace_waves, trace_stages; };
 
@@ -1794,8 +1930,8 @@
             if (a.ph[p].Kpad != a.ph[p].ntaps * a.Cin)
                 LWG_FAIL(LWG_ERR_UNSUPPORTED, "conv: taps-innermost walk needs K=%d == %d taps x %d channels", a.ph[p].Kpad,
                          a.ph[p].ntaps, a.Cin);
-    if (a.raw_in && (!a.in_ss || !raw_input_route(a, bn, sw)))
-        LWG_FAIL(LWG_ERR_UNSUPPORTED, "conv: raw (un-normalised) input is only taken by the halo-resident bf16x3 kernels");
+    if (a.raw_in && (!a.in_ss || !raw_input_route(a, bn, ncu, sw, tracing)))
+        LWG_FAIL(LWG_ERR_UNSUPPORTED, "conv: raw (un-normalised) input is only taken by the halo-resident bf16x3 kernels and the 256-row ring tile");
 
     const bool small_cin = a.Cin < BK;
     const dim3 grid(a.mtiles, a.Cout / bn, a.fuse_phases ? 1 : a.nphase * (a.ksplit > 1 ? a.ksplit : 1));
@@ -1837,9 +1973,8 @@
         if (bn == 64) return choose(kRing_64, grid, ring_lds(3, 64));
         if (tracing && !sw.ring3 && (size_t)grid.x * grid.y * grid.z * 4 * 8 * sizeof(unsigned long long) <= trace_free)
             return choose(kRing_128_Traced, grid, ring_lds(4, 128), 4, a.ph[0].Kpad / BK);
-        if (!a.fuse_phases && a.nphase == 1 && (a.mtiles & 1) == 0 && (a.Hm * a.Wm) % 256 == 0 && !tracing &&
-            (long)(a.mtiles / 2) * (a.Cout / 128) >= ncu && sw.ring_tall)
-            return choose(kRing_128_Tall, dim3(grid.x / 2, grid.y, 1), ring_lds(3, 128, 256));
+        if (a.raw_in) return choose(kRingRaw_128_Tall, dim3(grid.x / 2, grid.y, 1), ring_lds(3, 128, 256) + ring_raw_lds(a.Cin));
+        if (ring_tall_shape(a, bn, ncu, sw, tracing)) return choose(kRing_128_Tall, dim3(grid.x / 2, grid.y, 1), ring_lds(3, 128, 256));
 #ifdef LWG_EXPERIMENTS
         if (sw.ring_exp == 'x') return choose(kRing_128_X, grid, ring_lds(4, 128));
         if (sw.ring_exp == '5') return choose(kRing_128_5, grid, ring_lds(5, 128));
@@ -1953,11 +2088,12 @@
 #endif
 
 int launch_in_finalize(const float2 *partials, int nphase, int mtiles, int N, int C, const float *gamma,
-                       const float *beta, float eps, float2 *scale_shift, hipStream_t st)
-{
+                       const float *beta, float eps, float2 *scale_shift, hipStream_t st, int ss_ld)
+{
+    if (ss_ld != 0 && ss_ld < C) LWG_FAIL(LWG_ERR_INVALID_ARG, "in_finalize: row stride %d below the %d channels", ss_ld, C);
     if (mtiles % N != 0) LWG_FAIL(LWG_ERR_UNSUPPORTED, "in_finalize: %d tiles do not split over %d images", mtiles, N);
     const dim3 grid(ceil_div(C, FIN_CH), N);
-    in_finalize_kernel<<<grid, 256, 0, st>>>(partials, nphase, mtiles, mtiles / N, C, gamma, beta, eps, scale_shift);
+    in_finalize_kernel<<<grid, 256, 0, st>>>(partials, nphase, mtiles, mtiles / N, C, gamma, beta, eps, scale_shift, ss_ld ? ss_ld : C);
     LWG_LAUNCH_CHECK("in_finalize_kernel");
     return LWG_OK;
 }
diff --git a/impersonator_amd/csrc/direct.hip b/impersonator_amd/csrc/direct.hip
--- a/impersonator_amd/csrc/direct.hip
+++ b/impersonator_amd/csrc/direct.hip
@@ -175,7 +175,7 @@
 #pragma unroll
                 for (int r = 0; r < 16; ++r) {
                     const int px = i * 32 + (r & 3) + 8 * (r >> 2) + rsel;
-                    float *yo = a.y + (prow + px) * 64 + col;
+                    float *yo = a.y + (prow + px) * a.ldy + col;
                     yo[0] = acc[i][0][r];
                     yo[32] = acc[i][1][r];
                 }
@@ -258,14 +258,14 @@
     const int want = ceil_div(ntiles, ST_GROUPS);
     int nwg = want < ncu ? want : ncu;
     if (max_workgroups > 0 && nwg > max_workgroups) nwg = max_workgroups;
+    StemArgs b = a;
+    if (b.ldy == 0) b.ldy = 64;
+    if (b.ldy < 64 || (b.ldy & 3)) LWG_FAIL(LWG_ERR_INVALID_ARG, "stem: output pixel stride %d (0: dense, else >= 64 and a multiple of 4)", a.ldy);
 #ifdef LWG_EXPERIMENTS
     static const int dbg = getenv("LWG_STEM_DBG") ? atoi(getenv("LWG_STEM_DBG")) : 0;
-    StemArgs b = a;
     b.dbg = dbg;
+#endif
     stem_bf16x3_kernel<<<nwg, 256 * ST_GROUPS, ST_LDS, st>>>(b);
-#else
-    stem_bf16x3_kernel<<<nwg, 256 * ST_GROUPS, ST_LDS, st>>>(a);
-#endif
     LWG_LAUNCH_CHECK("stem_bf16x3_kernel");
     return LWG_OK;
 }
diff --git a/impersonator_amd/csrc/generator.hip b/impersonator_amd/csrc/generator.hip
--- a/impersonator_amd/csrc/generator.hip
+++ b/impersonator_amd/csrc/generator.hip
@@ -64,6 +64,7 @@
     float *tscale[2][kNDown] = {};
     float2 *partials = nullptr;
     float2 *ss = nullptr;
+    float2 *ss_cat0 = nullptr;
     float *zeros = nullptr;
     size_t cat_floats[kNDown] = {}, trunk_floats = 0, sk_floats[kNDown] = {};
     int trunk_out = 0;
@@ -344,7 +345,7 @@
 }
 
 int conv_args(lwg_generator *g, const Layer &L, const float *x, int ldx, int N, int H, int W, float *raw, int ld_raw, int raw_from,
-              ConvArgs &a, int &bn)
+              ConvArgs &a, int &bn, const float2 *in_ss = nullptr, int in_ss_ld = 0)
 {
     a = ConvArgs{};
     a.x = x;
@@ -372,8 +373,8 @@
     if (raw_from >= 0) {
         a.raw_in = 1;
         a.raw_from = raw_from;
-        a.in_ss = g->ss;
-        a.in_ss_ld = L.cin_pad - raw_from;
+        a.in_ss = in_ss ? in_ss : g->ss;
+        a.in_ss_ld = in_ss ? in_ss_ld : L.cin_pad - raw_from;
     }
     a.nphase = L.nphase;
     a.dil = 1;
@@ -415,12 +416,13 @@
 }
 
 int run_conv(lwg_generator *g, const Layer &L, const float *x, int ldx, int N, int H, int W, float *raw, hipStream_t st,
-             int ld_raw = 0, int raw_from = -1)
+             int ld_raw = 0, int raw_from = -1, const float2 *in_ss = nullptr, int in_ss_ld = 0, float2 *ss_out = nullptr,
+             int ss_out_ld = 0)
 {
     ConvArgs a;
     int bn = 0;
     {
-        const int rc0 = conv_args(g, L, x, ldx, N, H, W, raw, ld_raw, raw_from, a, bn);
+        const int rc0 = conv_args(g, L, x, ldx, N, H, W, raw, ld_raw, raw_from, a, bn, in_ss, in_ss_ld);
         if (rc0 != LWG_OK) return rc0;
     }
 
@@ -436,6 +438,7 @@
         s.x = x; s.N = N; s.H = H; s.W = W;
         s.w = L.w_stem;
         s.y = raw;
+        s.ldy = ld_raw;
         s.partials = a.partials;
         rc = launch_stem_bf16x3(s, st);
         variant = kDirectStemBf16x3;
@@ -452,7 +455,8 @@
         g->ev_variant.push_back(variant);
     }
     if (L.has_norm && !ko(1)) {
-        rc = launch_in_finalize(g->partials, L.nphase, a.mtiles, N, L.cout, L.gamma, L.beta, kInEps, g->ss, st);
+        rc = launch_in_finalize(g->partials, L.nphase, a.mtiles, N, L.cout, L.gamma, L.beta, kInEps, ss_out ? ss_out : g->ss, st,
+                                ss_out ? ss_out_ld : 0);
         if (rc != LWG_OK) return rc;
     }
     return LWG_OK;
@@ -505,11 +509,13 @@
 }
 
 int run_encoder(lwg_generator *g, const StreamNet &s, int lvl, const float *x, int ldx, int N, float *dst, int ld_dst,
-                const Warp *warps, int nwarp, int align, hipStream_t st)
+                const Warp *warps, int nwarp, int align, hipStream_t st, bool x_raw = false)
 {
     const Layer &L = s.enc[lvl];
     const int Hin = lvl == 0 ? g->is : g->is >> (lvl - 1);
-    int rc = (lvl == 0 && &s == &g->tsf && ko(32)) ? LWG_OK : run_conv(g, L, x, ldx, N, Hin, Hin, g->raw, st);
+    int rc = (lvl == 0 && &s == &g->tsf && ko(32)) ? LWG_OK
+             : x_raw ? run_conv(g, L, x, ldx, N, Hin, Hin, g->raw, st, 0, 0, g->ss_cat0, ldx)
+                     : run_conv(g, L, x, ldx, N, Hin, Hin, g->raw, st);
     if (rc != LWG_OK) return rc;
     const int Ho = g->is >> lvl;
     if (&s == &g->tsf && ko(lvl == 0 ? 2 : 4)) return LWG_OK;
@@ -557,7 +563,15 @@
     const float *x0 = nullptr;
     if ((rc = pack_input(g, tsf_inputs, layout, bs, g->tsf_dim, s.enc[0].cin_pad, st, &x0)) != LWG_OK) return rc;
 
-    if ((rc = run_encoder(g, s, 0, x0, s.enc[0].cin_pad, bs, g->cat[0], 2 * cd, nullptr, 0, align, st)) != LWG_OK) return rc;
+    const bool stem_raw = g->split && s.has_skip && !ko(32) && !ko(2) &&
+                          takes_raw_input(g, s.enc[1], g->cat[0], 2 * cd, bs, is, is, 0) &&
+                          takes_raw_input(g, s.skip[kNDown - 1], g->cat[0], 2 * cd, bs, is, is, 0);
+    if (stem_raw) {
+        if ((rc = run_conv(g, s.enc[0], x0, s.enc[0].cin_pad, bs, is, is, g->cat[0], st, 2 * cd, -1, nullptr, 0, g->ss_cat0, 2 * cd)) != LWG_OK)
+            return rc;
+    } else if ((rc = run_encoder(g, s, 0, x0, s.enc[0].cin_pad, bs, g->cat[0], 2 * cd, nullptr, 0, align, st)) != LWG_OK) {
+        return rc;
+    }
     for (int l = 1; l <= kNDown; ++l) {
         Warp w[2];
         for (int k = 0; k < nsets; ++k) {
@@ -569,7 +583,7 @@
         const int ldx = 2 * (cd << (l - 1));
         float *dst = l < kNDown ? g->cat[l] : g->trunk[0];
         const int ld_dst = l < kNDown ? 2 * (cd << l) : (cd << l);
-        if ((rc = run_encoder(g, s, l, xin, ldx, bs, dst, ld_dst, w, nsets, align, st)) != LWG_OK) return rc;
+        if ((rc = run_encoder(g, s, l, xin, ldx, bs, dst, ld_dst, w, nsets, align, st, l == 1 && stem_raw)) != LWG_OK) return rc;
     }
     int cur = 0;
     for (int i = 0; i < g->repeat; ++i) {
@@ -590,9 +604,10 @@
         const int lvl = kNDown - 1 - i, oC = dC / 2, oH = dH * 2;
         const bool last = i + 1 == kNDown;
         const bool skip_takes_raw = takes_raw_input(g, s.skip[i], g->cat[lvl], 2 * oC, bs, oH, oH, oC);
+        const bool both_raw = last && stem_raw;
         if (!(last && ko(128)) &&
             (rc = run_conv(g, s.dec[i], d, dC, bs, dH, dH, skip_takes_raw ? g->cat[lvl] + oC : g->raw, st, skip_takes_raw ? 2 * oC : 0,
-                           d_raw ? 0 : -1)) != LWG_OK)
+                           d_raw ? 0 : -1, nullptr, 0, both_raw ? g->ss_cat0 + oC : nullptr, 2 * oC)) != LWG_OK)
             return rc;
         if (!skip_takes_raw &&
             (rc = run_apply(g, bs, oH, oH, oC, true, g->cat[lvl] + oC, 2 * oC, nullptr, 0, nullptr, 0, align, st)) != LWG_OK)
@@ -600,7 +615,7 @@
         const bool next_takes_raw = !last && takes_raw_input(g, s.dec[i + 1], g->sk[i], oC, bs, oH, oH, 0);
         if (!(last && ko(64)) &&
             (rc = run_conv(g, s.skip[i], g->cat[lvl], 2 * oC, bs, oH, oH, next_takes_raw ? g->sk[i] : g->raw, st, 0,
-                           skip_takes_raw ? oC : -1)) != LWG_OK)
+                           both_raw ? 0 : skip_takes_raw ? oC : -1, both_raw ? g->ss_cat0 : nullptr, 2 * oC)) != LWG_OK)
             return rc;
         if (!last) {
             if (!next_takes_raw &&
@@ -698,6 +713,11 @@
         rc = dev_alloc(&p, B * (size_t)(cd << kNDown) * 2);
         g->ss = reinterpret_cast<float2 *>(p);
     }
+    if (rc == LWG_OK) {
+        float *p = nullptr;
+        rc = dev_alloc(&p, B * (size_t)(2 * cd) * 2);
+        g->ss_cat0 = reinterpret_cast<float2 *>(p);
+    }
     if (rc == LWG_OK) rc = dev_alloc(&g->zeros, 64);
     if (rc == LWG_OK && hipMemset(g->zeros, 0, 64 * sizeof(float)) != hipSuccess) {
         set_error("hipMemset of the zero page failed");
@@ -727,6 +747,7 @@
         for (auto p : k) fr(p);
     fr(g->partials);
     fr(g->ss);
+    fr(g->ss_cat0);
     fr(g->zeros);
     for (auto e : g->ev_pool) (void)hipEventDestroy(e);
     delete g;
diff --git a/impersonator_amd/csrc/train.hip b/impersonator_amd/csrc/train.hip
--- a/impersonator_amd/csrc/train.hip
+++ b/impersonator_amd/csrc/train.hip
@@ -2718,7 +2718,7 @@
     LWG_REQUIRE(!in_scale_shift || (uintptr_t)in_scale_shift % 8 == 0, "norm_conv_forward: in_scale_shift must be 8-byte aligned");
     LWG_REQUIRE((uintptr_t)ws % 16 == 0 && d->pad >= 0, "norm_conv_forward: the workspace must be 16-byte aligned, pad >= 0");
     if (in_scale_shift && d->precision != 1)
-        LWG_FAIL(LWG_ERR_UNSUPPORTED, "norm_conv_forward: raw input is taken by the bf16x3 halo kernels only");
+        LWG_FAIL(LWG_ERR_UNSUPPORTED, "norm_conv_forward: raw input is taken by bf16x3 kernels only");
     {
         const lwg_conv2d_desc wd = norm_conv_ws_desc(d);
         const size_t need = lwg_conv2d_workspace_bytes(&wd);
```

Result: no change. 4175 frames/s (median of 3 runs) (-0.6%).
